# gwlucastrig/gridfour

Measured on NVIDIA B200. Metric: GVRS tile decode GB/s of raw samples (config 3 shard, 180x240 tiles), higher is better.
Workload: dtype int32

## Files before the change

gridfour_b200/csrc/g4_api.cu:

```cuda
#include <cstdio>
#include <cstdlib>
#include <cstring>
#include <string>
#include <algorithm>
#include <vector>
#include "g4_kernels.h"

using namespace g4;

namespace {

constexpr int kMaxChunks = 16;

thread_local std::string tlsError;

int cuda_fail(cudaError_t e, const char* what) {
  tlsError = std::string(what) + ": " + cudaGetErrorString(e);
  return G4_ERR_CUDA;
}
#define CK(call)                                           \
  do {                                                     \
    cudaError_t e_ = (call);                               \
    if (e_ != cudaSuccess) return cuda_fail(e_, #call);    \
  } while (0)

struct DevBuf {
  void* p = nullptr;
  size_t cap = 0;
  cudaError_t ensure(size_t bytes) {
    if (bytes <= cap) return cudaSuccess;
    if (p) cudaFree(p);
    p = nullptr;
    cap = 0;
    size_t want = bytes + bytes / 8 + 256;
    cudaError_t e = cudaMalloc(&p, want);
    if (e == cudaSuccess) cap = want;
    return e;
  }
  void release() {
    if (p) cudaFree(p);
    p = nullptr;
    cap = 0;
  }
  template <class T>
  T* as() const { return static_cast<T*>(p); }
};

size_t round_up(size_t x, size_t a) { return (x + a - 1) / a * a; }

struct DeviceGuard {
  int prev = -1;
  cudaError_t err = cudaSuccess;
  explicit DeviceGuard(int device) {
    if (cudaGetDevice(&prev) != cudaSuccess) prev = -1;
    if (prev != device) err = cudaSetDevice(device);
    else prev = -1;
  }
  ~DeviceGuard() {
    if (prev >= 0) cudaSetDevice(prev);
  }
};
#define ENTER(ctx)                                                     \
  DeviceGuard guard_((ctx)->device);                                  \
  if (guard_.err != cudaSuccess) return cuda_fail(guard_.err, "cudaSetDevice")

}

struct g4_context {
  int device = 0;
  cudaStream_t stream = nullptr;
  bool ownStream = false;
  int smCount = 148;
  uint64_t launches = 0;
  DevBuf slots[G4_MAX_CODECS];
  DevBuf candLens, candPreds, candStatus;
  DevBuf counters;
  DevBuf scratch;
  DevBuf lists, src, total;
  DevBuf encScratch;
  DevBuf region;
  DevBuf coef;
  DevBuf defer;
  DevBuf lsopMeta;
  DevBuf lsopSide, lsopExc, lsopResid, lsopStage, lsopCks;
  DevBuf wide;
  DevBuf jobLen, jobOff, jobOut, jobTotal, streamIn, streamOut, deflateWork;
  DevBuf stSorted, stRank, stTable, stWork, stCounters;
  DevBuf rcPos, rcOff, rcLen, rcCrc, rcStored, rcTotal, rcData, rcOffsets, rcLens, rcIndex, rcStatus, rcOut;
  DevBuf rcChain, rcDesc;
  std::vector<uint64_t> hostOff;
  std::vector<uint32_t> hostLen;
  uint64_t hostTotal = 0;
  int deflateWorkers = 0;
  uint64_t stagedChunkBytes = 2ull << 30;
  const int64_t* curTileOffset = nullptr;
  const int64_t* curTilePitch = nullptr;
  DevBuf tileRefs;
  uint64_t arenaLimit = ~0ull;
  bool lsopDeflate = true;
  DevBuf sGrid, sArena, sOffsets, sLens, sCodec, sPred, sStatus;
  cudaStream_t copyIn = nullptr, copyOut = nullptr;
  cudaEvent_t evIn[16] = {}, evDone[16] = {}, evStart = nullptr, evOrder = nullptr;
  bool timing = false;
  bool asyncDevice = false;
  cudaEvent_t ev[2][G4_CODEC_COUNT + 1][2] = {};
  bool evUsed[2][G4_CODEC_COUNT + 1] = {};
};

namespace {

bool codec_is_float(int id) { return id == G4_CODEC_FLOAT; }

int persistent_ctas(const g4_context* ctx, int nTiles, int perSm) {
  int cap = ctx->smCount * perSm;
  return nTiles < cap ? nTiles : cap;
}

int ensure_jobs(g4_context* ctx, int nStreams) {
  CK(ctx->jobLen.ensure(size_t(nStreams) * 4));
  CK(ctx->jobOff.ensure(size_t(nStreams) * 8));
  CK(ctx->jobOut.ensure(size_t(nStreams) * 4));
  CK(ctx->jobTotal.ensure(8));
  return G4_OK;
}
int prepare_streams(g4_context* ctx, int nStreams) {
  CK(launch_stream_offsets(ctx->jobLen.as<uint32_t>(), ctx->jobOff.as<uint64_t>(), nStreams, ctx->jobTotal.as<uint64_t>(), ctx->stream));
  uint64_t total = 0;
  ctx->hostOff.resize(size_t(nStreams) + 1);
  ctx->hostLen.resize(size_t(nStreams));
  CK(cudaMemcpyAsync(&total, ctx->jobTotal.p, 8, cudaMemcpyDeviceToHost, ctx->stream));
  CK(cudaMemcpyAsync(ctx->hostOff.data(), ctx->jobOff.p, size_t(nStreams) * 8, cudaMemcpyDeviceToHost, ctx->stream));
  CK(cudaMemcpyAsync(ctx->hostLen.data(), ctx->jobLen.p, size_t(nStreams) * 4, cudaMemcpyDeviceToHost, ctx->stream));
  CK(cudaStreamSynchronize(ctx->stream));
  ctx->hostOff[size_t(nStreams)] = total;
  ctx->hostTotal = total;
  CK(ctx->streamIn.ensure(total + 64));
  CK(ctx->streamOut.ensure(total + 112ull * uint64_t(nStreams) + 256));
  ctx->launches++;
  return G4_OK;
}
int run_streams(g4_context* ctx, int nStreams, int capExtra, int level, int* counter) {
  const uint32_t stagedMax = deflate_staged_max();
  int nBig = 0;
  for (int j = 0; j < nStreams; j++) nBig += ctx->hostLen[size_t(j)] > stagedMax;
  if (nBig > 0) {
    int nWorkers = nBig < ctx->deflateWorkers ? nBig : ctx->deflateWorkers;
    nWorkers = (nWorkers + 31) / 32 * 32;
    CK(ctx->deflateWork.ensure(size_t(nWorkers) * deflate_work_bytes()));
    StreamArgs sa{};
    sa.inBuf = ctx->streamIn.as<uint8_t>();
    sa.inOff = ctx->jobOff.as<uint64_t>();
    sa.inLen = ctx->jobLen.as<uint32_t>();
    sa.outBuf = ctx->streamOut.as<uint8_t>();
    sa.outLen = ctx->jobOut.as<uint32_t>();
    sa.nStreams = nStreams;
    sa.capExtra = capExtra;
    sa.level = level;
    sa.work = ctx->deflateWork.p;
    sa.counter = counter;
    sa.bigOnly = 1;
    CK(launch_deflate_streams(sa, nWorkers, ctx->stream));
    ctx->launches++;
  }
  const uint64_t budget = ctx->stagedChunkBytes;
  CK(ctx->stCounters.ensure(4 * sizeof(int)));
  int j0 = 0;
  while (j0 < nStreams) {
    int j1 = j0 + 1;
    while (j1 < nStreams && ctx->hostOff[size_t(j1) + 1] - ctx->hostOff[size_t(j0)] <= budget) j1++;
    const uint64_t base = ctx->hostOff[size_t(j0)];
    const uint64_t span = ctx->hostOff[size_t(j1)] - base;
    const int nChunk = j1 - j0;
    CK(ctx->stSorted.ensure(span * 2 + 64));
    CK(ctx->stRank.ensure(span * 2 + 64));
    CK(ctx->stTable.ensure(span * 8 + 256));
    CK(ctx->stWork.ensure(size_t(nChunk) * deflate_blocks_bytes()));
    CK(cudaMemsetAsync(ctx->stCounters.p, 0, 4 * sizeof(int), ctx->stream));
    StagedArgs st{};
    st.inBuf = ctx->streamIn.as<uint8_t>();
    st.inOff = ctx->jobOff.as<uint64_t>();
    st.inLen = ctx->jobLen.as<uint32_t>();
    st.outBuf = ctx->streamOut.as<uint8_t>();
    st.outLen = ctx->jobOut.as<uint32_t>();
    st.jBegin = j0;
    st.jEnd = j1;
    st.baseOff = base;
    st.sorted = ctx->stSorted.as<uint16_t>();
    st.rank = ctx->stRank.as<uint16_t>();
    st.table = ctx->stTable.as<uint32_t>();
    st.tableQ = ctx->stTable.as<uint32_t>() + (span + 16);
    st.lazy = level >= 9 ? 1 : 0;
    st.maxLen = 0;
    for (int j = j0; j < j1; j++)
      if (ctx->hostLen[size_t(j)] <= stagedMax && ctx->hostLen[size_t(j)] > st.maxLen) st.maxLen = ctx->hostLen[size_t(j)];
    st.blocks = static_cast<DeflateBlocks*>(ctx->stWork.p);
    st.capExtra = capExtra;
    st.level = level;
    st.counters = ctx->stCounters.as<int>();
    CK(launch_deflate_staged(st, ctx->smCount, ctx->stream));
    ctx->launches += st.lazy ? 3 : 4;
    j0 = j1;
  }
  return G4_OK;
}

struct KernelTimer;
int launch_encoder_impl(g4_context* ctx, int codecId, EncodeArgs& a, int nTiles) {
  const int nGrid = persistent_ctas(ctx, nTiles, 8);
  uint32_t* jl = nullptr;
  uint64_t* jo = nullptr;
  uint32_t* jout = nullptr;
  switch (codecId) {
    case G4_CODEC_DEFLATE: {
      const int nStreams = 3 * nTiles;
      int rc = ensure_jobs(ctx, nStreams);
      if (rc != G4_OK) return rc;
      jl = ctx->jobLen.as<uint32_t>(); jo = ctx->jobOff.as<uint64_t>(); jout = ctx->jobOut.as<uint32_t>();
      CK(launch_deflate_m32_size(a, jl, nGrid, ctx->stream));
      if ((rc = prepare_streams(ctx, nStreams)) != G4_OK) return rc;
      CK(launch_deflate_m32_write(a, jl, jo, ctx->streamIn.as<uint8_t>(), nGrid, ctx->stream));
      if ((rc = run_streams(ctx, nStreams, 118, 6, a.counter + 48)) != G4_OK) return rc;
      CK(launch_deflate_pick(a, jl, jo, ctx->streamOut.as<uint8_t>(), jout, nGrid, ctx->stream));
      ctx->launches += 3;
      return G4_OK;
    }
    case G4_CODEC_FLOAT: {
      const int nStreams = 5 * nTiles;
      int rc = ensure_jobs(ctx, nStreams);
      if (rc != G4_OK) return rc;
      jl = ctx->jobLen.as<uint32_t>(); jo = ctx->jobOff.as<uint64_t>(); jout = ctx->jobOut.as<uint32_t>();
      CK(launch_float_plane_size(nTiles, uint32_t(a.band.tile_rows) * uint32_t(a.band.tile_cols), jl, ctx->stream));
      if ((rc = prepare_streams(ctx, nStreams)) != G4_OK) return rc;
      CK(launch_float_plane_write(a, jo, ctx->streamIn.as<uint8_t>(), nGrid, ctx->stream));
      if ((rc = run_streams(ctx, nStreams, 128, 9, a.counter + 48)) != G4_OK) return rc;
      CK(launch_float_pick(a, jo, ctx->streamOut.as<uint8_t>(), jout, nGrid, ctx->stream));
      ctx->launches += 3;
      return G4_OK;
    }
    case G4_CODEC_HUFFMAN: {
      int n = persistent_ctas(ctx, nTiles, 4);
      CK(launch_huffman_encode(a, n, ctx->stream));
      ctx->launches++;
      return G4_OK;
    }
    case G4_CODEC_CANON_HUFFMAN:
    case G4_CODEC_LSOP12: {
      int n = persistent_ctas(ctx, nTiles, 4);
      const size_t stride = 32 * 1024;
      CK(ctx->encScratch.ensure(stride * n));
      a.scratch = ctx->encScratch.as<uint8_t>();
      a.scratchStride = stride;
      if (codecId == G4_CODEC_CANON_HUFFMAN) CK(launch_canon_encode(a, n, ctx->stream));
      else CK(launch_lsop_encode(a, n, ctx->stream));
      ctx->launches++;
      if (codecId == G4_CODEC_LSOP12 && ctx->lsopDeflate) {
        const int nStreams = 2 * nTiles;
        int rc = ensure_jobs(ctx, nStreams);
        if (rc != G4_OK) return rc;
        jl = ctx->jobLen.as<uint32_t>(); jo = ctx->jobOff.as<uint64_t>(); jout = ctx->jobOut.as<uint32_t>();
        CK(launch_lsop_m32_size(a, jl, nGrid, ctx->stream));
        if ((rc = prepare_streams(ctx, nStreams)) != G4_OK) return rc;
        CK(launch_lsop_m32_write(a, jl, jo, ctx->streamIn.as<uint8_t>(), nGrid, ctx->stream));
        if ((rc = run_streams(ctx, nStreams, 128, 6, a.counter + 48)) != G4_OK) return rc;
        CK(launch_lsop_pick(a, jl, jo, ctx->streamOut.as<uint8_t>(), jout, nGrid, ctx->stream));
        ctx->launches += 3;
      }
      return G4_OK;
    }
    default:
      tlsError = "codec not implemented on the GPU yet";
      return G4_ERR_UNSUPPORTED;
  }
}

int decoder_ctas(const g4_context* ctx, int nTiles) { return persistent_ctas(ctx, nTiles, 8); }

struct KernelTimer {
  g4_context* c;
  int dir, kind;
  KernelTimer(g4_context* ctx, int dir_, int kind_) : c(ctx), dir(dir_), kind(kind_) {
    if (c->timing) {
      if (!c->ev[dir][kind][0]) { cudaEventCreate(&c->ev[dir][kind][0]); cudaEventCreate(&c->ev[dir][kind][1]); }
      cudaEventRecord(c->ev[dir][kind][0], c->stream);
    }
  }
  ~KernelTimer() {
    if (c->timing) { cudaEventRecord(c->ev[dir][kind][1], c->stream); c->evUsed[dir][kind] = true; }
  }
};

int launch_decoder(g4_context* ctx, int codecId, DecodeArgs& a, int nCtas) {
  KernelTimer timer(ctx, 0, codecId);
  const int nTiles = a.band.tiles_down * a.band.tiles_across;
  switch (codecId) {
    case G4_CODEC_HUFFMAN: {
      CK(ctx->defer.ensure(size_t(nTiles) * sizeof(int)));
      CK(ctx->lsopStage.ensure(huffman2_spill_bytes(ctx->smCount)));
      CK(ctx->lsopMeta.ensure(huffman2_tree_bytes(nTiles)));
      HuffFusedScratch fused{ctx->lsopStage.as<uint32_t>(), ctx->lsopMeta.as<uint8_t>(), ctx->defer.as<int>(), ctx->counters.as<int>() + 48, ctx->smCount};
      int nLaunch = 0;
      CK(launch_huffman_decode(a, nCtas, ctx->stream, fused, &nLaunch));
      ctx->launches += uint64_t(nLaunch);
      return G4_OK;
    }
    case G4_CODEC_CANON_HUFFMAN:
      CK(launch_canon_decode(a, nCtas, ctx->stream));
      ctx->launches++;
      return G4_OK;
    case G4_CODEC_DEFLATE: {
      const size_t stride = round_up(size_t(a.band.tile_rows) * a.band.tile_cols * 6 + 64, 16);
      CK(ctx->region.ensure(stride * nTiles));
      CK(launch_deflate_decode(a, ctx->region.as<uint8_t>(), stride, nCtas, nTiles, ctx->stream));
      ctx->launches += 2;
      return G4_OK;
    }
    case G4_CODEC_FLOAT: {
      const size_t stride = 5 * round_up(size_t(a.band.tile_rows) * a.band.tile_cols, 16);
      CK(ctx->region.ensure(stride * nTiles));
      CK(launch_float_decode(a, ctx->region.as<uint8_t>(), stride, nCtas, nTiles, ctx->stream));
      ctx->launches += 2;
      return G4_OK;
    }
    case G4_CODEC_LSOP12:
      CK(ctx->coef.ensure(size_t(nTiles) * 12 * sizeof(float)));
      CK(ctx->defer.ensure(size_t(nTiles) * sizeof(int)));
      CK(ctx->lsopMeta.ensure(size_t(nTiles) * lsop_meta_bytes()));
      CK(ctx->lsopCks.ensure(size_t(nTiles) * 8));
      CK(cudaMemsetAsync(ctx->lsopCks.p, 0, size_t(nTiles) * 8, ctx->stream));
      a.lsopCks = ctx->lsopCks.as<uint32_t>();
    {
      int nLaunch = 0;
      LsopFastArgs fast{};
      const bool useFast = lsop_fast_geometry(a.band, a.grid, &fast.g);
      if (useFast) {
        CK(ctx->lsopSide.ensure(lsop_fast_side_bytes(fast.g, nTiles)));
        CK(ctx->lsopExc.ensure(lsop_fast_exc_bytes(nTiles)));
        CK(ctx->lsopResid.ensure(lsop_fast_resid_bytes(fast.g, nTiles)));
        fast.side = ctx->lsopSide.as<int4>();
        fast.exc = ctx->lsopExc.as<uint32_t>();
        fast.resid = ctx->lsopResid.as<uint8_t>();
        if (lsop_fast_stage_bytes(ctx->smCount)) CK(ctx->lsopStage.ensure(lsop_fast_stage_bytes(ctx->smCount)));
        fast.textStage = ctx->lsopStage.as<uint8_t>();
      }
      CK(launch_lsop_decode(a, ctx->coef.as<float>(), ctx->lsopMeta.as<uint8_t>(), ctx->defer.as<int>(), ctx->counters.as<int>() + 56,
                            nCtas, nTiles, ctx->stream, &nLaunch, useFast ? &fast : nullptr, ctx->smCount));
      CK(launch_lsop_value_checksum(a, nTiles, ctx->stream));
      ctx->launches += uint64_t(nLaunch) + 1;
      return G4_OK;
    }
    case G4_CODEC_LSOP08:
      CK(ctx->coef.ensure(size_t(nTiles) * 12 * sizeof(float)));
      CK(launch_lsop08_decode(a, ctx->coef.as<float>(), nCtas, nTiles, ctx->stream));
      ctx->launches += 2;
      return G4_OK;
    default:
      tlsError = "codec not implemented on the GPU yet";
      return G4_ERR_UNSUPPORTED;
  }
}

int launch_encoder(g4_context* ctx, int codecId, EncodeArgs& a, int nTiles) {
  KernelTimer timer(ctx, 1, codecId);
  return launch_encoder_impl(ctx, codecId, a, nTiles);
}

int check_band(const g4_band_desc* b) {
  if (!b) return G4_ERR_ARG;
  if (b->elem_type != G4_ELEM_I32 && b->elem_type != G4_ELEM_F32 && b->elem_type != G4_ELEM_I16) return G4_ERR_ARG;
  if (b->tile_rows < 2 || b->tile_cols < 2) return G4_ERR_UNSUPPORTED;
  if (b->tiles_down < 1 || b->tiles_across < 1) return G4_ERR_ARG;
  if (int64_t(b->tile_rows) * b->tile_cols > (1 << 20)) return G4_ERR_UNSUPPORTED;
  if (b->grid_pitch < int64_t(b->tiles_across) * b->tile_cols) return G4_ERR_ARG;
  if (int64_t(b->tiles_down) * b->tiles_across > (1 << 24)) return G4_ERR_ARG;
  return G4_OK;
}

size_t elem_bytes(const g4_band_desc& b) { return b.elem_type == G4_ELEM_I16 ? 2 : 4; }
uint32_t standard_size(const g4_band_desc& b) {
  const uint32_t n = uint32_t(b.tile_rows) * uint32_t(b.tile_cols);
  return b.elem_type == G4_ELEM_I16 ? ((2u * n + 3u) & ~3u) : 4u * n;
}

size_t band_samples(const g4_band_desc& b) {
  return size_t(int64_t(b.tiles_down) * b.tile_rows - 1) * size_t(b.grid_pitch) + size_t(b.tiles_across) * b.tile_cols;
}

int encode_device_i32(g4_context* ctx, const g4_codec_list* codecs, const g4_band_desc* band, void* grid, uint8_t* arena,
                      uint64_t arenaCap, uint64_t* offsets, uint32_t* lens, uint8_t* codecOut, uint8_t* predOut, int32_t* status,
                      uint64_t* totalHost, size_t slotBytes, const int16_t* raw16, int64_t raw16Pitch) {
  const int nTiles = band->tiles_down * band->tiles_across;
  const int n = band->tile_rows * band->tile_cols;
  const bool isFloat = band->elem_type == G4_ELEM_F32;
  int cand[G4_MAX_CODECS], nCand = 0;
  for (int k = 0; k < codecs->n_codecs; k++) {
    int id = codecs->codec_ids[k];
    if (id < 0 || id >= G4_CODEC_COUNT) return G4_ERR_ARG;
    if (id == G4_CODEC_LSOP08) continue;
    if (codec_is_float(id) == isFloat) cand[nCand++] = k;
  }
  CK(ctx->candLens.ensure(size_t(nCand + 1) * nTiles * 4));
  CK(ctx->candPreds.ensure(size_t(nCand + 1) * nTiles));
  CK(ctx->candStatus.ensure(size_t(nCand + 1) * nTiles * 4));
  CK(ctx->counters.ensure(64 * sizeof(int)));
  CK(ctx->src.ensure(size_t(nTiles) * 4));
  CK(ctx->total.ensure(8));
  CK(cudaMemsetAsync(ctx->counters.p, 0, 64 * sizeof(int), ctx->stream));
  SelectArgs sel{};
  CompactArgs cmp{};
  for (int c = 0; c < nCand; c++) {
    CK(ctx->slots[c].ensure(size_t(nTiles) * slotBytes));
    EncodeArgs a{};
    a.band = *band;
    a.band.tileOffset = ctx->curTileOffset;
    a.band.tilePitch = ctx->curTilePitch;
    a.grid = grid;
    a.slots = ctx->slots[c].as<uint8_t>();
    a.slotBytes = slotBytes;
    a.lens = ctx->candLens.as<uint32_t>() + size_t(c) * nTiles;
    a.preds = ctx->candPreds.as<uint8_t>() + size_t(c) * nTiles;
    a.status = ctx->candStatus.as<int32_t>() + size_t(c) * nTiles;
    a.counter = ctx->counters.as<int>() + c;
    a.codecIndex = cand[c];
    a.scratch = nullptr;
    a.scratchStride = 0;
    int rc = launch_encoder(ctx, codecs->codec_ids[cand[c]], a, nTiles);
    if (rc != G4_OK) return rc;
    sel.candIndex[c] = cand[c];
    cmp.slots[c] = a.slots;
  }
  sel.nTiles = nTiles;
  sel.nCand = nCand;
  sel.rawLen = raw16 ? ((2u * uint32_t(n) + 3u) & ~3u) : uint32_t(n) * 4u;
  sel.candLens = ctx->candLens.as<uint32_t>();
  sel.candPreds = ctx->candPreds.as<uint8_t>();
  sel.candStatus = ctx->candStatus.as<int32_t>();
  sel.lens = lens;
  sel.codecOut = codecOut;
  sel.predOut = predOut;
  sel.src = ctx->src.as<int>();
  sel.status = status;
  CK(launch_select(sel, ctx->stream));
  CK(launch_offsets(lens, offsets, nTiles, ctx->total.as<uint64_t>(), ctx->stream));
  cmp.band = *band;
  cmp.band.tileOffset = ctx->curTileOffset;
  cmp.band.tilePitch = ctx->curTilePitch;
  cmp.grid = grid;
  cmp.slotBytes = slotBytes;
  cmp.lens = lens;
  cmp.offsets = offsets;
  cmp.src = ctx->src.as<int>();
  cmp.arena = arena;
  cmp.arenaCap = arenaCap;
  cmp.status = status;
  cmp.raw16 = raw16;
  cmp.raw16Pitch = raw16Pitch;
  CK(launch_compact(cmp, nTiles, ctx->stream));
  ctx->launches += 3;
  uint64_t total = 0;
  CK(cudaMemcpyAsync(&total, ctx->total.p, 8, cudaMemcpyDeviceToHost, ctx->stream));
  CK(cudaStreamSynchronize(ctx->stream));
  if (totalHost) *totalHost = total;
  return G4_OK;
}

int decode_device_i32(g4_context* ctx, const g4_codec_list* codecs, const g4_band_desc* band, const uint8_t* arena,
                      const uint64_t* offsets, const uint32_t* lens, void* grid, int32_t* status, bool rawShorts) {
  const int nTiles = band->tiles_down * band->tiles_across;
  const int n = band->tile_rows * band->tile_cols;
  const int kinds = G4_CODEC_COUNT + 1;
  CK(ctx->counters.ensure(64 * sizeof(int)));
  CK(ctx->lists.ensure(size_t(kinds) * nTiles * sizeof(int)));
  CK(cudaMemsetAsync(ctx->counters.p, 0, 64 * sizeof(int), ctx->stream));
  ClassifyArgs cl{};
  cl.nTiles = nTiles;
  cl.elemType = band->elem_type;
  cl.rawLen = rawShorts ? ((2u * uint32_t(n) + 3u) & ~3u) : uint32_t(n) * 4u;
  cl.codecs = *codecs;
  cl.arena = arena;
  cl.arenaLen = ctx->arenaLimit;
  cl.offsets = offsets;
  cl.lens = lens;
  cl.lists = ctx->lists.as<int>();
  cl.counts = ctx->counters.as<int>() + 32;
  cl.status = status;
  CK(launch_classify(cl, ctx->stream));
  ctx->launches++;
  const int nCtas = decoder_ctas(ctx, nTiles);
  const size_t stride = round_up(size_t(n) * 6 + 64, 16);
  CK(ctx->scratch.ensure(stride * nCtas));
  bool present[G4_CODEC_COUNT] = {false};
  for (int k = 0; k < codecs->n_codecs; k++) {
    int id = codecs->codec_ids[k];
    if (id < 0 || id >= G4_CODEC_COUNT) return G4_ERR_ARG;
    present[id] = true;
  }
  for (int kind = 0; kind <= G4_CODEC_COUNT; kind++) {
    if (kind < G4_CODEC_COUNT && !present[kind]) continue;
    DecodeArgs a{};
    a.band = *band;
    a.band.tileOffset = ctx->curTileOffset;
    a.band.tilePitch = ctx->curTilePitch;
    a.grid = grid;
    a.arena = arena;
    a.offsets = offsets;
    a.lens = lens;
    a.list = ctx->lists.as<int>() + size_t(kind) * nTiles;
    a.listCount = ctx->counters.as<int>() + 32 + kind;
    a.status = status;
    a.counter = ctx->counters.as<int>() + 16 + kind;
    a.scratch = ctx->scratch.as<uint8_t>();
    a.scratchStride = stride;
    a.rawShorts = rawShorts ? 1 : 0;
    if (kind == G4_CODEC_COUNT) {
      KernelTimer timer(ctx, 0, kind);
      CK(launch_raw_decode(a, nTiles, ctx->stream));
      ctx->launches++;
    } else {
      int rc = launch_decoder(ctx, kind, a, nCtas);
      if (rc != G4_OK) return rc;
    }
  }
  return G4_OK;
}

g4_band_desc widened(const g4_band_desc& b) {
  g4_band_desc w = b;
  w.elem_type = G4_ELEM_I32;
  w.grid_pitch = int64_t(b.tiles_across) * b.tile_cols;
  return w;
}

int encode_device(g4_context* ctx, const g4_codec_list* codecs, const g4_band_desc* band, void* grid, uint8_t* arena,
                  uint64_t arenaCap, uint64_t* offsets, uint32_t* lens, uint8_t* codecOut, uint8_t* predOut, int32_t* status,
                  uint64_t* totalHost, size_t slotBytes) {
  if (band->elem_type != G4_ELEM_I16)
    return encode_device_i32(ctx, codecs, band, grid, arena, arenaCap, offsets, lens, codecOut, predOut, status, totalHost, slotBytes,
                             nullptr, 0);
  const g4_band_desc w = widened(*band);
  const int64_t rows = int64_t(band->tiles_down) * band->tile_rows, cols = w.grid_pitch;
  CK(ctx->wide.ensure(size_t(rows) * size_t(cols) * 4));
  CK(launch_widen_i16(static_cast<const int16_t*>(grid), band->grid_pitch, ctx->wide.as<int32_t>(), rows, cols, band->fill_value,
                      ctx->stream));
  ctx->launches++;
  return encode_device_i32(ctx, codecs, &w, ctx->wide.p, arena, arenaCap, offsets, lens, codecOut, predOut, status, totalHost, slotBytes,
                           static_cast<const int16_t*>(grid), band->grid_pitch);
}

int decode_device(g4_context* ctx, const g4_codec_list* codecs, const g4_band_desc* band, const uint8_t* arena,
                  const uint64_t* offsets, const uint32_t* lens, void* grid, int32_t* status) {
  if (band->elem_type != G4_ELEM_I16) return decode_device_i32(ctx, codecs, band, arena, offsets, lens, grid, status, false);
  const g4_band_desc w = widened(*band);
  const int64_t rows = int64_t(band->tiles_down) * band->tile_rows, cols = w.grid_pitch;
  CK(ctx->wide.ensure(size_t(rows) * size_t(cols) * 4));
  int rc = decode_device_i32(ctx, codecs, &w, arena, offsets, lens, ctx->wide.p, status, true);
  if (rc != G4_OK) return rc;
  CK(launch_narrow_i16(ctx->wide.as<int32_t>(), static_cast<int16_t*>(grid), band->grid_pitch, rows, cols, ctx->stream));
  ctx->launches++;
  return G4_OK;
}

int first_bad_status(const std::vector<int32_t>& st) {
  int32_t note = G4_OK;
  for (int32_t s : st) {
    if (s < 0) return s;
    if (s != G4_OK && note == G4_OK) note = s;
  }
  return note;
}

}

extern "C" {

int g4_abi_version(void) { return G4_ABI_VERSION; }

const char* g4_status_string(int s) {
  switch (s) {
    case G4_OK: return "ok";
    case G4_DECLINED: return "declined (codec returns null for this tile)";
    case G4_ERR_ARG: return "bad argument";
    case G4_ERR_FORMAT: return "malformed packing";
    case G4_ERR_CAPACITY: return "output buffer too small";
    case G4_ERR_CUDA: return "CUDA error";
    case G4_ERR_UNSUPPORTED: return "unsupported";
    default: return "unknown status";
  }
}

const char* g4_last_error(void) { return tlsError.c_str(); }

int g4_device_count(void) {
  int n = 0;
  if (cudaGetDeviceCount(&n) != cudaSuccess) return 0;
  return n;
}

static const char* kCodecNames[G4_CODEC_COUNT] = {"GvrsHuffman", "GvrsDeflate", "GvrsFloat", "GvrsCanonicalHuffman", "LSOP12", "LSOP08"};

int g4_codec_id_from_name(const char* name) {
  if (!name) return -1;
  for (int i = 0; i < G4_CODEC_COUNT; i++)
    if (std::strcmp(name, kCodecNames[i]) == 0) return i;
  return -1;
}
const char* g4_codec_name(int id) { return (id >= 0 && id < G4_CODEC_COUNT) ? kCodecNames[id] : nullptr; }

int g4_context_create(int device, void* cuda_stream, g4_context** out) {
  if (!out) return G4_ERR_ARG;
  *out = nullptr;
  int nDev = 0;
  cudaError_t e = cudaGetDeviceCount(&nDev);
  if (e != cudaSuccess || nDev == 0) {
    tlsError = "no CUDA device available (the codec kernels have no CPU fallback)";
    return G4_ERR_CUDA;
  }
  if (device < 0 || device >= nDev) return G4_ERR_ARG;
  DeviceGuard guard(device);
  if (guard.err != cudaSuccess) return cuda_fail(guard.err, "cudaSetDevice");
  g4_context* ctx = new g4_context();
  ctx->device = device;
  auto fail = [&](cudaError_t err, const char* what) {
    if (ctx->ownStream && ctx->stream) cudaStreamDestroy(ctx->stream);
    delete ctx;
    return cuda_fail(err, what);
  };
  cudaDeviceProp prop;
  if ((e = cudaGetDeviceProperties(&prop, device)) != cudaSuccess) return fail(e, "cudaGetDeviceProperties");
  ctx->smCount = prop.multiProcessorCount;
  ctx->deflateWorkers = ctx->smCount * 256;
  if (const char* ev = std::getenv("G4_DEFLATE_WORKERS")) { int v = std::atoi(ev); if (v >= 32) ctx->deflateWorkers = v; }
  if (const char* ev = std::getenv("G4_STAGED_CHUNK_MB")) { long v = std::atol(ev); if (v >= 1) ctx->stagedChunkBytes = uint64_t(v) << 20; }
  if (cuda_stream) ctx->stream = static_cast<cudaStream_t>(cuda_stream);
  else {
    if ((e = cudaStreamCreateWithFlags(&ctx->stream, cudaStreamNonBlocking)) != cudaSuccess) return fail(e, "cudaStreamCreateWithFlags");
    ctx->ownStream = true;
  }
  if ((e = cudaEventCreateWithFlags(&ctx->evStart, cudaEventDisableTiming)) != cudaSuccess) return fail(e, "cudaEventCreateWithFlags");
  if ((e = cudaEventCreateWithFlags(&ctx->evOrder, cudaEventDisableTiming)) != cudaSuccess) return fail(e, "cudaEventCreateWithFlags");
  *out = ctx;
  return G4_OK;
}

int g4_context_order_stream(g4_context* ctx, void* other_stream, int before) {
  if (!ctx) return G4_ERR_ARG;
  cudaStream_t other = static_cast<cudaStream_t>(other_stream);
  if (other == ctx->stream) return G4_OK;
  ENTER(ctx);
  if (before) {
    CK(cudaEventRecord(ctx->evOrder, other));
    CK(cudaStreamWaitEvent(ctx->stream, ctx->evOrder, 0));
  } else {
    CK(cudaEventRecord(ctx->evOrder, ctx->stream));
    CK(cudaStreamWaitEvent(other, ctx->evOrder, 0));
  }
  return G4_OK;
}

void g4_context_destroy(g4_context* ctx) {
  if (!ctx) return;
  DeviceGuard guard(ctx->device);
  cudaStreamSynchronize(ctx->stream);
  if (ctx->copyIn) {
    cudaStreamSynchronize(ctx->copyIn);
    cudaStreamSynchronize(ctx->copyOut);
    cudaStreamDestroy(ctx->copyIn);
    cudaStreamDestroy(ctx->copyOut);
    for (int k = 0; k < kMaxChunks; k++) { cudaEventDestroy(ctx->evIn[k]); cudaEventDestroy(ctx->evDone[k]); }
  }
  if (ctx->evStart) cudaEventDestroy(ctx->evStart);
  if (ctx->evOrder) cudaEventDestroy(ctx->evOrder);
  for (auto& b : ctx->slots) b.release();
  DevBuf* bufs[] = {&ctx->candLens, &ctx->candPreds, &ctx->candStatus, &ctx->counters, &ctx->scratch, &ctx->lists, &ctx->src,
                    &ctx->total, &ctx->coef, &ctx->defer, &ctx->lsopMeta, &ctx->lsopSide, &ctx->lsopExc, &ctx->lsopResid, &ctx->lsopStage, &ctx->tileRefs, &ctx->lsopCks, &ctx->wide, &ctx->encScratch, &ctx->region, &ctx->jobLen, &ctx->jobOff, &ctx->jobOut, &ctx->jobTotal,
                    &ctx->streamIn, &ctx->streamOut, &ctx->deflateWork, &ctx->stSorted, &ctx->stRank, &ctx->stTable,
                    &ctx->stWork, &ctx->stCounters, &ctx->rcPos, &ctx->rcOff, &ctx->rcLen, &ctx->rcCrc, &ctx->rcStored, &ctx->rcTotal,
                    &ctx->rcData, &ctx->rcOffsets, &ctx->rcLens, &ctx->rcIndex, &ctx->rcStatus, &ctx->rcOut, &ctx->rcChain, &ctx->rcDesc, &ctx->sGrid, &ctx->sArena, &ctx->sOffsets, &ctx->sLens, &ctx->sCodec, &ctx->sPred, &ctx->sStatus};
  for (DevBuf* b : bufs) b->release();
  if (ctx->ownStream) cudaStreamDestroy(ctx->stream);
  delete ctx;
}

int g4_context_synchronize(g4_context* ctx) {
  if (!ctx) return G4_ERR_ARG;
  CK(cudaStreamSynchronize(ctx->stream));
  return G4_OK;
}

uint64_t g4_launch_count(const g4_context* ctx) { return ctx ? ctx->launches : 0; }

int g4_context_set_async(g4_context* ctx, int enabled) {
  if (!ctx) return G4_ERR_ARG;
  ctx->asyncDevice = enabled != 0;
  return G4_OK;
}

int g4_context_set_timing(g4_context* ctx, int enabled) {
  if (!ctx) return G4_ERR_ARG;
  ctx->timing = enabled != 0;
  for (auto& d : ctx->evUsed) for (bool& u : d) u = false;
  return G4_OK;
}

int g4_codec_supported(int codec_id, int direction) {
  switch (codec_id) {
    case G4_CODEC_HUFFMAN: return 1;
    case G4_CODEC_DEFLATE: return 1;
    case G4_CODEC_FLOAT: return 1;
    case G4_CODEC_CANON_HUFFMAN: return 1;
    case G4_CODEC_LSOP12: return 1;
    case G4_CODEC_LSOP08: return direction == 0 ? 1 : 0;
    default: return 0;
  }
}

double g4_kernel_time_ms(g4_context* ctx, int direction, int codec_kind) {
  if (!ctx || direction < 0 || direction > 1 || codec_kind < 0 || codec_kind > G4_CODEC_COUNT) return -1.0;
  if (!ctx->evUsed[direction][codec_kind]) return -1.0;
  float ms = -1.0f;
  if (cudaEventSynchronize(ctx->ev[direction][codec_kind][1]) != cudaSuccess) return -1.0;
  if (cudaEventElapsedTime(&ms, ctx->ev[direction][codec_kind][0], ctx->ev[direction][codec_kind][1]) != cudaSuccess) return -1.0;
  return double(ms);
}

int g4_crc32c(g4_context* ctx, int mem_space, const uint8_t* data, const uint64_t* offsets, const uint32_t* sizes, int n,
              uint32_t* crc_out) {
  if (!ctx || !data || !offsets || !sizes || !crc_out || n < 0) return G4_ERR_ARG;
  if (n == 0) return G4_OK;
  ENTER(ctx);
  if (mem_space == G4_MEM_DEVICE) {
    CK(launch_crc32c(data, offsets, sizes, n, crc_out, 0, ctx->stream));
    ctx->launches++;
    return G4_OK;
  }
  if (mem_space != G4_MEM_HOST) return G4_ERR_ARG;
  uint64_t bytes = 0;
  for (int i = 0; i < n; i++) {
    const uint64_t end = offsets[i] + sizes[i];
    if (end > bytes) bytes = end;
  }
  CK(ctx->rcData.ensure(bytes + 16));
  CK(ctx->rcOff.ensure(size_t(n) * 8));
  CK(ctx->rcLen.ensure(size_t(n) * 4));
  CK(ctx->rcCrc.ensure(size_t(n) * 4));
  CK(cudaMemcpyAsync(ctx->rcData.p, data, bytes, cudaMemcpyHostToDevice, ctx->stream));
  CK(cudaMemcpyAsync(ctx->rcOff.p, offsets, size_t(n) * 8, cudaMemcpyHostToDevice, ctx->stream));
  CK(cudaMemcpyAsync(ctx->rcLen.p, sizes, size_t(n) * 4, cudaMemcpyHostToDevice, ctx->stream));
  CK(launch_crc32c(ctx->rcData.as<uint8_t>(), ctx->rcOff.as<uint64_t>(), ctx->rcLen.as<uint32_t>(), n, ctx->rcCrc.as<uint32_t>(), 0,
                   ctx->stream));
  ctx->launches++;
  CK(cudaMemcpyAsync(crc_out, ctx->rcCrc.p, size_t(n) * 4, cudaMemcpyDeviceToHost, ctx->stream));
  CK(cudaStreamSynchronize(ctx->stream));
  return G4_OK;
}

uint64_t g4_tile_records_bound(int n_tiles, uint64_t payload_bytes) {
  if (n_tiles < 0) return 0;
  return payload_bytes + uint64_t(n_tiles) * 32ull;
}

int g4_pack_tile_records(g4_context* ctx, int mem_space, const uint8_t* arena, const uint64_t* offsets, const uint32_t* lens,
                         const int32_t* tile_index, int first_tile_index, int n_tiles, int checksum, uint64_t base_pos,
                         uint8_t* records, uint64_t records_cap, uint64_t* content_pos, uint64_t* total_bytes) {
  if (!ctx || !arena || !offsets || !lens || !records || !content_pos || !total_bytes || n_tiles < 0 || (base_pos & 7)) return G4_ERR_ARG;
  if (mem_space != G4_MEM_DEVICE && mem_space != G4_MEM_HOST) return G4_ERR_ARG;
  *total_bytes = 0;
  if (n_tiles == 0) return G4_OK;
  ENTER(ctx);
  const int n = n_tiles;
  const uint8_t* dArena = arena;
  const uint64_t* dOffsets = offsets;
  const uint32_t* dLens = lens;
  const int32_t* dIndex = tile_index;
  uint64_t* dPos = content_pos;
  uint8_t* dRecords = records;
  if (mem_space == G4_MEM_HOST) {
    uint64_t arenaBytes = 0;
    for (int t = 0; t < n; t++) {
      const uint64_t end = offsets[t] + lens[t];
      if (end > arenaBytes) arenaBytes = end;
    }
    CK(ctx->rcData.ensure(arenaBytes + 16));
    CK(ctx->rcOffsets.ensure(size_t(n) * 8));
    CK(ctx->rcLens.ensure(size_t(n) * 4));
    CK(ctx->rcPos.ensure(size_t(n) * 8));
    CK(ctx->rcOut.ensure(records_cap + 16));
    CK(cudaMemcpyAsync(ctx->rcData.p, arena, arenaBytes, cudaMemcpyHostToDevice, ctx->stream));
    CK(cudaMemcpyAsync(ctx->rcOffsets.p, offsets, size_t(n) * 8, cudaMemcpyHostToDevice, ctx->stream));
    CK(cudaMemcpyAsync(ctx->rcLens.p, lens, size_t(n) * 4, cudaMemcpyHostToDevice, ctx->stream));
    if (tile_index) {
      CK(ctx->rcIndex.ensure(size_t(n) * 4));
      CK(cudaMemcpyAsync(ctx->rcIndex.p, tile_index, size_t(n) * 4, cudaMemcpyHostToDevice, ctx->stream));
      dIndex = ctx->rcIndex.as<int32_t>();
    }
    dArena = ctx->rcData.as<uint8_t>();
    dOffsets = ctx->rcOffsets.as<uint64_t>();
    dLens = ctx->rcLens.as<uint32_t>();
    dPos = ctx->rcPos.as<uint64_t>();
    dRecords = ctx->rcOut.as<uint8_t>();
  }
  CK(ctx->rcOff.ensure(size_t(n) * 8));
  CK(ctx->rcLen.ensure(size_t(n) * 4));
  CK(ctx->rcTotal.ensure(8));
  CK(launch_record_layout(dLens, n, base_pos, dPos, ctx->rcOff.as<uint64_t>(), ctx->rcLen.as<uint32_t>(), ctx->rcTotal.as<uint64_t>(),
                          ctx->stream));
  uint64_t total = 0;
  CK(cudaMemcpyAsync(&total, ctx->rcTotal.p, 8, cudaMemcpyDeviceToHost, ctx->stream));
  CK(cudaStreamSynchronize(ctx->stream));
  *total_bytes = total;
  if (total > records_cap) return G4_ERR_CAPACITY;
  CK(launch_record_pack(dArena, dOffsets, dLens, dIndex, first_tile_index, n, ctx->rcOff.as<uint64_t>(), ctx->rcLen.as<uint32_t>(), dRecords,
                        persistent_ctas(ctx, n, 8), ctx->stream));
  ctx->launches += 2;
  if (checksum) {
    CK(launch_crc32c(dRecords, ctx->rcOff.as<uint64_t>(), ctx->rcLen.as<uint32_t>(), n, nullptr, 1, ctx->stream));
    ctx->launches++;
  }
  if (mem_space == G4_MEM_HOST) {
    CK(cudaMemcpyAsync(records, dRecords, total, cudaMemcpyDeviceToHost, ctx->stream));
    CK(cudaMemcpyAsync(content_pos, dPos, size_t(n) * 8, cudaMemcpyDeviceToHost, ctx->stream));
    CK(cudaStreamSynchronize(ctx->stream));
  }
  return G4_OK;
}

int g4_unpack_tile_records(g4_context* ctx, int mem_space, const uint8_t* image, uint64_t image_len, const uint64_t* content_pos,
                           int n_tiles, int checksum, uint64_t* payload_offsets, uint32_t* lens, int32_t* status) {
  if (!ctx || !image || !content_pos || !payload_offsets || !lens || !status || n_tiles < 0) return G4_ERR_ARG;
  if (mem_space != G4_MEM_DEVICE && mem_space != G4_MEM_HOST) return G4_ERR_ARG;
  if (n_tiles == 0) return G4_OK;
  ENTER(ctx);
  const int n = n_tiles;
  const uint8_t* dImage = image;
  const uint64_t* dPos = content_pos;
  uint64_t* dPay = payload_offsets;
  uint32_t* dLens = lens;
  int32_t* dStatus = status;
  if (mem_space == G4_MEM_HOST) {
    CK(ctx->rcData.ensure(image_len + 16));
    CK(ctx->rcPos.ensure(size_t(n) * 8));
    CK(ctx->rcOffsets.ensure(size_t(n) * 8));
    CK(ctx->rcLens.ensure(size_t(n) * 4));
    CK(ctx->rcStatus.ensure(size_t(n) * 4));
    CK(cudaMemcpyAsync(ctx->rcData.p, image, image_len, cudaMemcpyHostToDevice, ctx->stream));
    CK(cudaMemcpyAsync(ctx->rcPos.p, content_pos, size_t(n) * 8, cudaMemcpyHostToDevice, ctx->stream));
    dImage = ctx->rcData.as<uint8_t>();
    dPos = ctx->rcPos.as<uint64_t>();
    dPay = ctx->rcOffsets.as<uint64_t>();
    dLens = ctx->rcLens.as<uint32_t>();
    dStatus = ctx->rcStatus.as<int32_t>();
  }
  if (reinterpret_cast<uintptr_t>(dImage) & 7) return G4_ERR_ARG;
  CK(ctx->rcOff.ensure(size_t(n) * 8));
  CK(ctx->rcLen.ensure(size_t(n) * 4));
  CK(ctx->rcCrc.ensure(size_t(n) * 4));
  CK(ctx->rcStored.ensure(size_t(n) * 4));
  CK(launch_record_unpack(dImage, image_len, dPos, n, dPay, dLens, ctx->rcOff.as<uint64_t>(), ctx->rcLen.as<uint32_t>(),
                          ctx->rcStored.as<uint32_t>(), dStatus, ctx->stream));
  ctx->launches++;
  if (checksum) {
    CK(launch_crc32c(dImage, ctx->rcOff.as<uint64_t>(), ctx->rcLen.as<uint32_t>(), n, ctx->rcCrc.as<uint32_t>(), 0, ctx->stream));
    CK(launch_record_verify(ctx->rcCrc.as<uint32_t>(), ctx->rcStored.as<uint32_t>(), n, dStatus, ctx->stream));
    ctx->launches += 2;
  }
  if (mem_space == G4_MEM_HOST) {
    CK(cudaMemcpyAsync(payload_offsets, dPay, size_t(n) * 8, cudaMemcpyDeviceToHost, ctx->stream));
    CK(cudaMemcpyAsync(lens, dLens, size_t(n) * 4, cudaMemcpyDeviceToHost, ctx->stream));
    CK(cudaMemcpyAsync(status, dStatus, size_t(n) * 4, cudaMemcpyDeviceToHost, ctx->stream));
    CK(cudaStreamSynchronize(ctx->stream));
  }
  return G4_OK;
}

uint64_t g4_tile_records_bound_multi(int n_tiles, int n_elements, uint64_t payload_bytes) {
  if (n_tiles < 0 || n_elements < 1 || n_elements > G4_MAX_ELEMENTS) return 0;
  return payload_bytes + uint64_t(n_tiles) * (23ull + 4ull * uint64_t(n_elements));
}

int g4_pack_tile_records_multi(g4_context* ctx, int mem_space, int n_elements, const uint8_t* const* arenas,
                               const uint64_t* const* offsets, const uint32_t* const* lens, const int32_t* tile_index,
                               int first_tile_index, int n_tiles, int checksum, uint64_t base_pos, uint8_t* records,
                               uint64_t records_cap, uint64_t* content_pos, uint64_t* total_bytes) {
  if (!ctx || !arenas || !offsets || !lens || !records || !content_pos || !total_bytes || n_tiles < 0 || (base_pos & 7)) return G4_ERR_ARG;
  if (n_elements < 1 || n_elements > G4_MAX_ELEMENTS) return G4_ERR_UNSUPPORTED;
  if (mem_space != G4_MEM_DEVICE && mem_space != G4_MEM_HOST) return G4_ERR_ARG;
  for (int e = 0; e < n_elements; e++)
    if (!arenas[e] || !offsets[e] || !lens[e]) return G4_ERR_ARG;
  *total_bytes = 0;
  if (n_tiles == 0) return G4_OK;
  ENTER(ctx);
  const int n = n_tiles, E = n_elements;
  std::vector<RecordElement> desc(static_cast<size_t>(E));
  const int32_t* dIndex = tile_index;
  uint64_t* dPos = content_pos;
  uint8_t* dRecords = records;
  if (mem_space == G4_MEM_HOST) {
    std::vector<uint64_t> base(size_t(E) + 1, 0), used(size_t(E), 0);
    for (int e = 0; e < E; e++) {
      for (int t = 0; t < n; t++) {
        const uint64_t end = offsets[e][t] + lens[e][t];
        if (end > used[size_t(e)]) used[size_t(e)] = end;
      }
      base[size_t(e) + 1] = round_up(base[size_t(e)] + used[size_t(e)], 16);
    }
    CK(ctx->rcData.ensure(base[size_t(E)] + 16));
    CK(ctx->rcOffsets.ensure(size_t(E) * n * 8));
    CK(ctx->rcLens.ensure(size_t(E) * n * 4));
    CK(ctx->rcPos.ensure(size_t(n) * 8));
    CK(ctx->rcOut.ensure(records_cap + 16));
    for (int e = 0; e < E; e++) {
      uint8_t* a = ctx->rcData.as<uint8_t>() + base[size_t(e)];
      uint64_t* o = ctx->rcOffsets.as<uint64_t>() + size_t(e) * n;
      uint32_t* l = ctx->rcLens.as<uint32_t>() + size_t(e) * n;
      if (used[size_t(e)]) CK(cudaMemcpyAsync(a, arenas[e], used[size_t(e)], cudaMemcpyHostToDevice, ctx->stream));
      CK(cudaMemcpyAsync(o, offsets[e], size_t(n) * 8, cudaMemcpyHostToDevice, ctx->stream));
      CK(cudaMemcpyAsync(l, lens[e], size_t(n) * 4, cudaMemcpyHostToDevice, ctx->stream));
      desc[size_t(e)] = RecordElement{a, o, l};
    }
    if (tile_index) {
      CK(ctx->rcIndex.ensure(size_t(n) * 4));
      CK(cudaMemcpyAsync(ctx->rcIndex.p, tile_index, size_t(n) * 4, cudaMemcpyHostToDevice, ctx->stream));
      dIndex = ctx->rcIndex.as<int32_t>();
    }
    dPos = ctx->rcPos.as<uint64_t>();
    dRecords = ctx->rcOut.as<uint8_t>();
  } else {
    for (int e = 0; e < E; e++) desc[size_t(e)] = RecordElement{arenas[e], offsets[e], lens[e]};
  }
  CK(ctx->rcDesc.ensure(size_t(E) * sizeof(RecordElement)));
  CK(cudaMemcpyAsync(ctx->rcDesc.p, desc.data(), size_t(E) * sizeof(RecordElement), cudaMemcpyHostToDevice, ctx->stream));
  const RecordElement* dDesc = ctx->rcDesc.as<RecordElement>();
  CK(ctx->rcChain.ensure(size_t(n) * 4));
  CK(ctx->rcOff.ensure(size_t(n) * 8));
  CK(ctx->rcLen.ensure(size_t(n) * 4));
  CK(ctx->rcTotal.ensure(8));
  CK(launch_record_chain_lens(dDesc, E, n, ctx->rcChain.as<uint32_t>(), ctx->stream));
  CK(launch_record_layout(ctx->rcChain.as<uint32_t>(), n, base_pos, dPos, ctx->rcOff.as<uint64_t>(), ctx->rcLen.as<uint32_t>(),
                          ctx->rcTotal.as<uint64_t>(), ctx->stream));
  uint64_t total = 0;
  CK(cudaMemcpyAsync(&total, ctx->rcTotal.p, 8, cudaMemcpyDeviceToHost, ctx->stream));
  CK(cudaStreamSynchronize(ctx->stream));
  ctx->launches += 2;
  *total_bytes = total;
  if (total > records_cap) return G4_ERR_CAPACITY;
  CK(launch_record_pack_multi(dDesc, E, dIndex, first_tile_index, n, ctx->rcOff.as<uint64_t>(), ctx->rcLen.as<uint32_t>(), dRecords,
                              persistent_ctas(ctx, n, 8), ctx->stream));
  ctx->launches++;
  if (checksum) {
    CK(launch_crc32c(dRecords, ctx->rcOff.as<uint64_t>(), ctx->rcLen.as<uint32_t>(), n, nullptr, 1, ctx->stream));
    ctx->launches++;
  }
  if (mem_space == G4_MEM_HOST) {
    CK(cudaMemcpyAsync(records, dRecords, total, cudaMemcpyDeviceToHost, ctx->stream));
    CK(cudaMemcpyAsync(content_pos, dPos, size_t(n) * 8, cudaMemcpyDeviceToHost, ctx->stream));
    CK(cudaStreamSynchronize(ctx->stream));
  }
  return G4_OK;
}

int g4_unpack_tile_records_multi(g4_context* ctx, int mem_space, int n_elements, const uint8_t* image, uint64_t image_len,
                                 const uint64_t* content_pos, int n_tiles, int checksum, uint64_t* payload_offsets,
                                 uint32_t* lens, int32_t* status) {
  if (!ctx || !image || !content_pos || !payload_offsets || !lens || !status || n_tiles < 0) return G4_ERR_ARG;
  if (n_elements < 1 || n_elements > G4_MAX_ELEMENTS) return G4_ERR_UNSUPPORTED;
  if (mem_space != G4_MEM_DEVICE && mem_space != G4_MEM_HOST) return G4_ERR_ARG;
  if (n_tiles == 0) return G4_OK;
  ENTER(ctx);
  const int n = n_tiles, E = n_elements;
  const uint8_t* dImage = image;
  const uint64_t* dPos = content_pos;
  uint64_t* dPay = payload_offsets;
  uint32_t* dLens = lens;
  int32_t* dStatus = status;
  if (mem_space == G4_MEM_HOST) {
    CK(ctx->rcData.ensure(image_len + 16));
    CK(ctx->rcPos.ensure(size_t(n) * 8));
    CK(ctx->rcOffsets.ensure(size_t(E) * n * 8));
// ... 574 lines not shown
```

gridfour_b200/csrc/g4_batch.cu:

```cuda
#include "g4_kernels.h"
#include "g4_device.cuh"
#include "../../include/g4terrain.h"

namespace g4 {

__global__ void fill_terrain_kernel(int elemType, uint64_t seed, int64_t row0, int64_t col0, int64_t nRows, int64_t nCols,
                                    void* out) {
  const int64_t total = nRows * nCols;
  for (int64_t i = blockIdx.x * int64_t(blockDim.x) + threadIdx.x; i < total; i += int64_t(gridDim.x) * blockDim.x) {
    int64_t r = i / nCols, c = i - r * nCols;
    if (elemType == G4_ELEM_I32) static_cast<int32_t*>(out)[i] = g4_terrain_m(seed, row0 + r, col0 + c);
    else static_cast<float*>(out)[i] = float(g4_terrain_dm(seed, row0 + r, col0 + c)) * 0.1f;
  }
}

__global__ void select_kernel(SelectArgs a) {
  int t = blockIdx.x * blockDim.x + threadIdx.x;
  if (t >= a.nTiles) return;
  uint32_t best = 0xffffffffu;
  int bc = -1;
  int st = G4_OK;
  for (int c = 0; c < a.nCand; c++) {
    int s = a.candStatus[size_t(c) * a.nTiles + t];
    uint32_t l = a.candLens[size_t(c) * a.nTiles + t];
    if (s == G4_OK && l > 0 && l < best) { best = l; bc = c; }
    else if (s < 0 && s != G4_ERR_CAPACITY && st == G4_OK) st = s;
  }
  const uint32_t rawLen = a.rawLen;
  if (bc < 0 || best >= rawLen) {
    a.lens[t] = rawLen;
    a.codecOut[t] = G4_CODEC_RAW;
    a.predOut[t] = 0;
    a.src[t] = -1;
  } else {
    a.lens[t] = best;
    a.codecOut[t] = uint8_t(a.candIndex[bc]);
    a.predOut[t] = a.candPreds[size_t(bc) * a.nTiles + t];
    a.src[t] = bc;
  }
  a.status[t] = st;
}

__global__ void __launch_bounds__(kThreads) offsets_kernel(const uint32_t* lens, uint64_t* offsets, int nTiles, uint64_t* total) {
  __shared__ unsigned long long sm[kWarps];
  __shared__ unsigned long long carry;
  const int lane = threadIdx.x & 31, warp = threadIdx.x >> 5;
  if (threadIdx.x == 0) carry = 0;
  __syncthreads();
  for (int t0 = 0; t0 < nTiles; t0 += kThreads) {
    int t = t0 + threadIdx.x;
    unsigned long long x = t < nTiles ? ((unsigned long long)(lens[t]) + 7ull) & ~7ull : 0ull;
    unsigned long long inc = x;
#pragma unroll
    for (int d = 1; d < 32; d <<= 1) {
      unsigned long long y = __shfl_up_sync(0xffffffffu, inc, d);
      if (lane >= d) inc += y;
    }
    if (lane == 31) sm[warp] = inc;
    __syncthreads();
    unsigned long long base = carry;
    for (int w = 0; w < warp; w++) base += sm[w];
    if (t < nTiles) offsets[t] = base + inc - x;
    __syncthreads();
    if (threadIdx.x == kThreads - 1) carry = base + inc;
    __syncthreads();
  }
  if (threadIdx.x == 0) *total = carry;
}

__global__ void __launch_bounds__(kThreads) compact_kernel(CompactArgs a) {
  const int t = blockIdx.x;
  const uint32_t len = a.lens[t];
  const uint64_t off = a.offsets[t];
  if (off + ((uint64_t(len) + 7) & ~7ull) > a.arenaCap) {
    if (threadIdx.x == 0) a.status[t] = G4_ERR_CAPACITY;
    return;
  }
  uint8_t* dst = a.arena + off;
  const int src = a.src[t];
  if (src < 0 && a.raw16) {
    const int R = a.band.tile_rows, C = a.band.tile_cols, n = R * C;
    const int tr = t / a.band.tiles_across, tc = t - tr * a.band.tiles_across;
    const int16_t* base = a.raw16 + int64_t(tr) * R * a.raw16Pitch + int64_t(tc) * C;
    uint32_t* d32 = reinterpret_cast<uint32_t*>(dst);
    const int nWords = int((len + 3u) >> 2);
    for (int i = threadIdx.x; i < ((nWords + 1) & ~1); i += kThreads) {
      uint32_t w = 0;
      for (int h = 0; h < 2; h++) {
        int k = 2 * i + h;
        if (k < n) { int r = k / C, c = k - r * C; w |= uint32_t(uint16_t(base[int64_t(r) * a.raw16Pitch + c])) << (16 * h); }
      }
      d32[i] = w;
    }
  } else if (src < 0) {
    const TileView tv = tile_view(a.band, a.grid, t);
    uint32_t* d32 = reinterpret_cast<uint32_t*>(dst);
    const int n = tv.R * tv.C;
    for (int i = threadIdx.x; i < n; i += kThreads) {
      int r = i / tv.C, c = i - r * tv.C;
      d32[i] = uint32_t(tv.at(r, c));
    }
    if ((n & 1) && threadIdx.x == 0) d32[n] = 0;
  } else {
    const uint32_t* s32 = reinterpret_cast<const uint32_t*>(a.slots[src] + size_t(t) * a.slotBytes);
    uint32_t* d32 = reinterpret_cast<uint32_t*>(dst);
    const uint32_t nWords = ((len + 7u) & ~7u) >> 2;
    for (uint32_t i = threadIdx.x; i < nWords; i += kThreads) {
      uint32_t w = 0;
      if (i * 4u < len) {
        w = s32[i];
        uint32_t valid = len - i * 4u;
        if (valid < 4u) w &= (1u << (8u * valid)) - 1u;
      }
      d32[i] = w;
    }
  }
}

__global__ void classify_kernel(ClassifyArgs a) {
  int t = blockIdx.x * blockDim.x + threadIdx.x;
  if (t >= a.nTiles) return;
  const uint32_t len = a.lens[t];
  int kind;
  int st = G4_OK;
  if (len > a.rawLen || a.offsets[t] > a.arenaLen || uint64_t(len) > a.arenaLen - a.offsets[t]) { kind = -1; st = G4_ERR_FORMAT; }
  else if (len == a.rawLen) kind = G4_CODEC_COUNT;
  else if (len == 0) { kind = -1; st = G4_ERR_FORMAT; }
  else {
    int index = a.arena[a.offsets[t]];
    if (index >= a.codecs.n_codecs) { kind = -1; st = G4_ERR_FORMAT; }
    else {
      kind = a.codecs.codec_ids[index];
      bool isFloatCodec = kind == G4_CODEC_FLOAT;
      if (kind < 0 || kind >= G4_CODEC_COUNT || isFloatCodec != (a.elemType == G4_ELEM_F32)) { kind = -1; st = G4_ERR_FORMAT; }
    }
  }
  a.status[t] = st;
  if (kind >= 0) {
    int pos = atomicAdd(&a.counts[kind], 1);
    a.lists[size_t(kind) * a.nTiles + pos] = t;
  }
}

__global__ void __launch_bounds__(kThreads) raw_decode_kernel(DecodeArgs a) {
  const int li = blockIdx.x;
  if (li >= *a.listCount) return;
  const int t = a.list[li];
  const TileView tv = tile_view(a.band, a.grid, t);
  const uint8_t* src = a.arena + a.offsets[t];
  const int n = tv.R * tv.C;
  if (a.rawShorts) {
    for (int i = threadIdx.x; i < n; i += kThreads) {
      int r = i / tv.C, c = i - r * tv.C;
      tv.at(r, c) = int32_t(int16_t(uint16_t(src[2 * size_t(i)]) | (uint16_t(src[2 * size_t(i) + 1]) << 8)));
    }
    return;
  }
  const bool aligned = (reinterpret_cast<uintptr_t>(src) & 3) == 0;
  for (int i = threadIdx.x; i < n; i += kThreads) {
    int r = i / tv.C, c = i - r * tv.C;
    uint32_t v = aligned ? reinterpret_cast<const uint32_t*>(src)[i] : load_le32(src + 4 * size_t(i));
    tv.at(r, c) = int32_t(v);
  }
}

__global__ void widen_i16_kernel(const int16_t* src, int64_t srcPitch, int32_t* dst, int64_t rows, int64_t cols, int32_t fill) {
  const int64_t total = rows * cols;
  for (int64_t i = blockIdx.x * int64_t(blockDim.x) + threadIdx.x; i < total; i += int64_t(gridDim.x) * blockDim.x) {
    int64_t r = i / cols, c = i - r * cols;
    int32_t v = src[r * srcPitch + c];
    dst[i] = v == fill ? kNull : v;
  }
}
__global__ void narrow_i16_kernel(const int32_t* src, int16_t* dst, int64_t dstPitch, int64_t rows, int64_t cols) {
  const int64_t total = rows * cols;
  for (int64_t i = blockIdx.x * int64_t(blockDim.x) + threadIdx.x; i < total; i += int64_t(gridDim.x) * blockDim.x) {
    int64_t r = i / cols, c = i - r * cols;
    int32_t v = src[i];
    dst[r * dstPitch + c] = v == kNull ? int16_t(-32768) : int16_t(v);
  }
}

cudaError_t launch_fill_terrain(int elemType, uint64_t seed, int64_t row0, int64_t col0, int64_t nRows, int64_t nCols, void* out,
                                cudaStream_t s) {
  fill_terrain_kernel<<<148 * 8, 256, 0, s>>>(elemType, seed, row0, col0, nRows, nCols, out);
  return cudaGetLastError();
}
cudaError_t launch_widen_i16(const int16_t* src, int64_t srcPitch, int32_t* dst, int64_t rows, int64_t cols, int32_t fill, cudaStream_t s) {
  widen_i16_kernel<<<148 * 8, 256, 0, s>>>(src, srcPitch, dst, rows, cols, fill);
  return cudaGetLastError();
}
cudaError_t launch_narrow_i16(const int32_t* src, int16_t* dst, int64_t dstPitch, int64_t rows, int64_t cols, cudaStream_t s) {
  narrow_i16_kernel<<<148 * 8, 256, 0, s>>>(src, dst, dstPitch, rows, cols);
  return cudaGetLastError();
}
cudaError_t launch_select(const SelectArgs& a, cudaStream_t s) {
  select_kernel<<<(a.nTiles + 255) / 256, 256, 0, s>>>(a);
  return cudaGetLastError();
}
cudaError_t launch_offsets(const uint32_t* lens, uint64_t* offsets, int nTiles, uint64_t* total, cudaStream_t s) {
  offsets_kernel<<<1, kThreads, 0, s>>>(lens, offsets, nTiles, total);
  return cudaGetLastError();
}
cudaError_t launch_compact(const CompactArgs& a, int nTiles, cudaStream_t s) {
  compact_kernel<<<nTiles, kThreads, 0, s>>>(a);
  return cudaGetLastError();
}
cudaError_t launch_classify(const ClassifyArgs& a, cudaStream_t s) {
  classify_kernel<<<(a.nTiles + 255) / 256, 256, 0, s>>>(a);
  return cudaGetLastError();
}
cudaError_t launch_raw_decode(const DecodeArgs& a, int nTiles, cudaStream_t s) {
  raw_decode_kernel<<<nTiles, kThreads, 0, s>>>(a);
  return cudaGetLastError();
}

}
```

gridfour_b200/csrc/g4_kernels.h:

```cpp
#pragma once
#include <cstddef>
#include <cstdint>
#include <atomic>
#include <cuda_runtime.h>
#include "../../include/g4codec.h"
#include "g4_device.cuh"

namespace g4 {

template <class Fn>
inline cudaError_t once_per_device(std::atomic<uint64_t>& done, Fn set) {
  int d = 0;
  cudaGetDevice(&d);
  const uint64_t bit = 1ull << (d & 63);
  if (done.load(std::memory_order_acquire) & bit) return cudaSuccess;
  const cudaError_t e = set();
  if (e == cudaSuccess) done.fetch_or(bit, std::memory_order_release);
  return e;
}

struct DeflateBlocks;

struct EncodeArgs {
  BandEx band;
  void* grid;
  uint8_t* slots;
  size_t slotBytes;
  uint32_t* lens;
  uint8_t* preds;
  int32_t* status;
  int* counter;
  int codecIndex;
  uint8_t* scratch;
  size_t scratchStride;
};

struct DecodeArgs {
  BandEx band;
  void* grid;
  const uint8_t* arena;
  const uint64_t* offsets;
  const uint32_t* lens;
  const int* list;
  const int* listCount;
  int32_t* status;
  int* counter;
  uint8_t* scratch;
  size_t scratchStride;
  int rawShorts;
  uint32_t* lsopCks;
};

struct SelectArgs {
  int nTiles, nCand;
  uint32_t rawLen;
  const uint32_t* candLens;
  const uint8_t* candPreds;
  const int32_t* candStatus;
  int candIndex[G4_MAX_CODECS];
  uint32_t* lens;
  uint8_t* codecOut;
  uint8_t* predOut;
  int* src;
  int32_t* status;
};

struct CompactArgs {
  BandEx band;
  void* grid;
  const uint8_t* slots[G4_MAX_CODECS];
  size_t slotBytes;
  const uint32_t* lens;
  const uint64_t* offsets;
  const int* src;
  uint8_t* arena;
  uint64_t arenaCap;
  int32_t* status;
  const int16_t* raw16;
  int64_t raw16Pitch;
};

struct ClassifyArgs {
  int nTiles;
  int elemType;
  uint32_t rawLen;
  g4_codec_list codecs;
  const uint8_t* arena;
  uint64_t arenaLen;
  const uint64_t* offsets;
  const uint32_t* lens;
  int* lists;
  int* counts;
  int32_t* status;
};

struct StreamArgs {
  const uint8_t* inBuf;
  const uint64_t* inOff;
  const uint32_t* inLen;
  uint8_t* outBuf;
  uint32_t* outLen;
  int nStreams;
  int capExtra;
  int level;
  void* work;
  int* counter;
  int bigOnly;
};

struct StagedArgs {
  const uint8_t* inBuf;
  const uint64_t* inOff;
  const uint32_t* inLen;
  uint8_t* outBuf;
  uint32_t* outLen;
  int jBegin, jEnd;
  uint64_t baseOff;
  uint16_t* sorted;
  uint16_t* rank;
  uint32_t* table;
  uint32_t* tableQ;
  uint32_t maxLen;
  int lazy;
  DeflateBlocks* blocks;
  int capExtra, level;
  int* counters;
};

cudaError_t launch_fill_terrain(int elemType, uint64_t seed, int64_t row0, int64_t col0, int64_t nRows, int64_t nCols, void* out,
                                cudaStream_t s);
cudaError_t launch_select(const SelectArgs& a, cudaStream_t s);
cudaError_t launch_offsets(const uint32_t* lens, uint64_t* offsets, int nTiles, uint64_t* total, cudaStream_t s);
cudaError_t launch_compact(const CompactArgs& a, int nTiles, cudaStream_t s);
cudaError_t launch_classify(const ClassifyArgs& a, cudaStream_t s);
cudaError_t launch_raw_decode(const DecodeArgs& a, int nTiles, cudaStream_t s);
cudaError_t launch_widen_i16(const int16_t* src, int64_t srcPitch, int32_t* dst, int64_t rows, int64_t cols, int32_t fill, cudaStream_t s);
cudaError_t launch_narrow_i16(const int32_t* src, int16_t* dst, int64_t dstPitch, int64_t rows, int64_t cols, cudaStream_t s);

cudaError_t launch_huffman_encode(const EncodeArgs& a, int nCtas, cudaStream_t s);
struct HuffFusedScratch {
  uint32_t* spill;
  uint8_t* trees;
  int* defer;
  int* counters;
  int smCount;
};
size_t huffman2_spill_bytes(int smCount);
size_t huffman2_tree_bytes(int nTiles);
cudaError_t launch_huffman_decode(const DecodeArgs& a, int nCtas, cudaStream_t s, const HuffFusedScratch& fused, int* launches);
cudaError_t launch_canon_decode(const DecodeArgs& a, int nCtas, cudaStream_t s);
cudaError_t launch_canon_encode(const EncodeArgs& a, int nCtas, cudaStream_t s);
cudaError_t launch_lsop_encode(const EncodeArgs& a, int nCtas, cudaStream_t s);
cudaError_t launch_deflate_decode(const DecodeArgs& a, uint8_t* region, size_t regionStride, int nCtas, int nTilesUpper,
                                  cudaStream_t s);
cudaError_t launch_float_decode(const DecodeArgs& a, uint8_t* region, size_t regionStride, int nCtas, int nTilesUpper,
                                cudaStream_t s);
size_t lsop_meta_bytes();
cudaError_t launch_lsop08_decode(const DecodeArgs& a, float* coef, int nCtas, int nTilesUpper, cudaStream_t s);


struct LsopFastGeom {
  int R, C;
  int W;
  int logW;
  int nStrips;
  int P;
  int nSteps;
  int chunkRows;
  int nChunks;
  int tileBytes;
  int tilePitch;
  int wide;
};
struct LsopFastArgs {
  DecodeArgs a;
  float* coef;
  uint8_t* meta;
  int4* side;
  uint32_t* exc;
  uint8_t* resid;
  uint8_t* textStage;
  int* defer;
  int* deferCount;
  LsopFastGeom g;
};
bool lsop_fast_geometry(const g4_band_desc& band, const void* grid, LsopFastGeom* out);
size_t lsop_fast_side_bytes(const LsopFastGeom& g, int nTiles);
size_t lsop_fast_exc_bytes(int nTiles);
size_t lsop_fast_stage_bytes(int smCount);
size_t lsop_fast_resid_bytes(const LsopFastGeom& g, int nTiles);
cudaError_t launch_lsop_decode_fast(const LsopFastArgs& A, int nTilesUpper, int smCount, int* textCounter, cudaStream_t s, int* launches);
cudaError_t launch_lsop_decode(const DecodeArgs& a, float* coef, uint8_t* meta, int* defer, int* deferCounters, int nCtas,
                               int nTilesUpper, cudaStream_t s, int* launches, const LsopFastArgs* fast = nullptr, int smCount = 148);

struct AnalyzeArgs {
  int nTiles;
  uint32_t nCells;
  uint32_t rawLen;
  g4_codec_list codecs;
  const uint8_t* arena;
  uint64_t arenaLen;
  const uint64_t* offsets;
  const uint32_t* lens;
  uint8_t* scratch;
  size_t scratchStride;
  g4_tile_stats* stats;
  unsigned long long* pairs;
};
cudaError_t launch_analyze(const AnalyzeArgs& a, int nCtas, cudaStream_t s);

struct PredictorArgs {
  BandEx band;
  void* grid;
  int model;
  int intFlavour;
  uint8_t* slots;
  size_t slotBytes;
  uint32_t* lens;
  int32_t* seeds;
  int32_t* status;
};
cudaError_t launch_predictor(const PredictorArgs& a, int decode, int nCtas, cudaStream_t s);

size_t deflate_work_bytes();
size_t deflate_blocks_bytes();
uint32_t deflate_staged_max();
cudaError_t launch_deflate_staged(const StagedArgs& a, int smCount, cudaStream_t s);
cudaError_t launch_stream_offsets(const uint32_t* inLen, uint64_t* inOff, int nStreams, uint64_t* total, cudaStream_t s);
cudaError_t launch_deflate_streams(const StreamArgs& a, int nWorkers, cudaStream_t s);
cudaError_t launch_deflate_m32_size(const EncodeArgs& a, uint32_t* inLen, int nCtas, cudaStream_t s);
cudaError_t launch_deflate_m32_write(const EncodeArgs& a, const uint32_t* inLen, const uint64_t* inOff, uint8_t* inBuf, int nCtas,
                                     cudaStream_t s);
cudaError_t launch_deflate_pick(const EncodeArgs& a, const uint32_t* inLen, const uint64_t* inOff, const uint8_t* outBuf,
                                const uint32_t* outLen, int nCtas, cudaStream_t s);
cudaError_t launch_float_plane_size(int nTiles, uint32_t n, uint32_t* inLen, cudaStream_t s);
cudaError_t launch_float_plane_write(const EncodeArgs& a, const uint64_t* inOff, uint8_t* inBuf, int nCtas, cudaStream_t s);
cudaError_t launch_float_pick(const EncodeArgs& a, const uint64_t* inOff, const uint8_t* outBuf, const uint32_t* outLen, int nCtas,
                              cudaStream_t s);
cudaError_t launch_lsop_m32_size(const EncodeArgs& a, uint32_t* inLen, int nCtas, cudaStream_t s);
cudaError_t launch_lsop_m32_write(const EncodeArgs& a, const uint32_t* inLen, const uint64_t* inOff, uint8_t* inBuf, int nCtas,
                                  cudaStream_t s);
cudaError_t launch_lsop_pick(const EncodeArgs& a, const uint32_t* inLen, const uint64_t* inOff, const uint8_t* outBuf,
                             const uint32_t* outLen, int nCtas, cudaStream_t s);

cudaError_t launch_crc32c(const uint8_t* data, const uint64_t* offsets, const uint32_t* sizes, int n, uint32_t* out, int storeAtEnd,
                          cudaStream_t s);
cudaError_t launch_record_layout(const uint32_t* lens, int n, uint64_t basePos, uint64_t* contentPos, uint64_t* crcOff, uint32_t* crcLen,
                                 uint64_t* total, cudaStream_t s);
cudaError_t launch_record_pack(const uint8_t* arena, const uint64_t* offsets, const uint32_t* lens, const int32_t* tileIndex,
                               int firstTileIndex, int n, const uint64_t* crcOff, const uint32_t* crcLen, uint8_t* records, int nCtas,
                               cudaStream_t s);
cudaError_t launch_record_unpack(const uint8_t* image, uint64_t imageLen, const uint64_t* contentPos, int n, uint64_t* payloadOff,
                                 uint32_t* lens, uint64_t* crcOff, uint32_t* crcLen, uint32_t* storedCrc, int32_t* status, cudaStream_t s);
cudaError_t launch_lsop_value_checksum(const DecodeArgs& a, int nTilesUpper, cudaStream_t s);
cudaError_t launch_record_verify(const uint32_t* computed, const uint32_t* stored, int n, int32_t* status, cudaStream_t s);
struct RecordElement {
  const uint8_t* arena;
  const uint64_t* offsets;
  const uint32_t* lens;
};
cudaError_t launch_record_chain_lens(const RecordElement* elems, int nElements, int n, uint32_t* chainLens, cudaStream_t s);
cudaError_t launch_record_pack_multi(const RecordElement* elems, int nElements, const int32_t* tileIndex, int firstTileIndex, int n,
                                     const uint64_t* crcOff, const uint32_t* crcLen, uint8_t* records, int nCtas, cudaStream_t s);
cudaError_t launch_record_unpack_multi(const uint8_t* image, uint64_t imageLen, const uint64_t* contentPos, int n, int nElements,
                                       uint64_t* payloadOff, uint32_t* lens, uint64_t* crcOff, uint32_t* crcLen, uint32_t* storedCrc,
                                       int32_t* status, cudaStream_t s);
cudaError_t launch_record_verify_multi(const uint32_t* computed, const uint32_t* stored, int n, int nElements, uint64_t* payloadOff,
                                       uint32_t* lens, int32_t* status, cudaStream_t s);

}
```

gridfour_b200/csrc/g4_lsop.cu:

```cuda
#include <utility>
#include "g4_kernels.h"
#include "g4_predict.cuh"
#include "g4_huffdec.cuh"
#include "g4_canon.cuh"
#include "g4_canon_fast.cuh"
#include "g4_canon_enc.cuh"
#include "g4_inflate.cuh"
#include "g4_m32stream.cuh"
#include "g4_lsop_common.cuh"

namespace g4 {

namespace {

union LsopDecShared {
  HuffDecShared h;
  CanonDecShared c;
  InflateWarpShared inf;
};


struct CellSink {
  TileView t;
  int order;
// ... 193 lines not shown
  if (h.type != 2 || len > stageWords * 4u || (reinterpret_cast<uintptr_t>(packing) & 3) != 0) {
    if (lane == 0) defer[atomicAdd(deferCount, 1)] = tIdx;
    return;
  }
  const uint32_t nInit = uint32_t(4 * R + 2 * C - 9);
  BitSrc src;
  src.init(packing, len);
  canon_warp_parse_header(W, src, h.headerSize * 8u);
  int status = W.error ? G4_ERR_FORMAT : G4_OK;
  uint32_t endBit = 0;
  if (status == G4_OK) {
    uint32_t eb = 0, nv = 0;
    auto emit = [&](uint32_t k, int32_t v) {
      int r, c;
      stream_to_cell(kStreamLsopInit, int(k), R, C, &r, &c);
      t.at(r, c) = v;
    };
    const bool ok = canon_warp_decode_text(W, src, W.textStart, nInit, emit, &eb, &nv) && nv == nInit;
    __syncwarp();
    if (lane == 0) {
      if (!ok) W.error = 1;
      W.textStart = eb;
    }
    __syncwarp();
    if (W.error) status = G4_ERR_FORMAT;
    endBit = W.textStart;
  }
  if (status == G4_OK) {
    canon_warp_parse_header(W, src, endBit);
    if (W.error) status = G4_ERR_FORMAT;
    else {
      for (int i = lane; i < kCanonSymbols; i += 32) m[8 + i] = W.lens[i];
      if (lane == 0) *reinterpret_cast<uint32_t*>(m) = W.textStart;
    }
  }
  if (status == G4_OK) {
    if (lane == 0) t.at(0, 0) = h.seed;
    __syncwarp();
    row_scan_warp(t.row(0), C, 0);
    __syncwarp();
    lsop_warp_column_scan(t, 0, 1, uint32_t(h.seed), false);
    {
      uint32_t carry = uint32_t(t.at(1, 0)) - uint32_t(t.at(0, 0));
      for (int c0 = 1; c0 < C; c0 += 32) {
        int c = c0 + lane;
        uint32_t x = c < C ? uint32_t(t.at(1, c)) : 0u;
        uint32_t inc = warp_inclusive_scan(x);
        if (c < C) t.at(1, c) = int32_t(carry + inc + uint32_t(t.at(0, c)));
        carry += __shfl_sync(0xffffffffu, inc, 31);
      }
    }
    __syncwarp();
    lsop_warp_column_scan(t, 1, 2, uint32_t(t.at(1, 1)) - uint32_t(t.at(1, 0)), true);
  }
  if (lane == 0) a.status[tIdx] = status;
}

template <class InteriorSink>
__global__ void __launch_bounds__(kThreads, 4) lsop_decode_text_kernel(DecodeArgs a, const uint8_t* meta) {
  extern __shared__ __align__(16) unsigned char lsopFastSmem[];
  CanonFastShared& F = *reinterpret_cast<CanonFastShared*>(lsopFastSmem);
  __shared__ int sTile;
  const int tid = threadIdx.x;
  for (;;) {
    __syncthreads();
    if (tid == 0) sTile = atomicAdd(a.counter, 1);
    __syncthreads();
    const int li = sTile;
    if (li >= *a.listCount) break;
    const int tIdx = a.list[li];
    const uint8_t* m = meta + size_t(tIdx) * kLsopMetaBytes;
    const uint32_t T0 = *reinterpret_cast<const uint32_t*>(m);
    if (T0 == 0) continue;
    const TileView t = tile_view(a.band, a.grid, tIdx);
    const uint8_t* packing = a.arena + a.offsets[tIdx];
    const uint32_t len = a.lens[tIdx];
    const uint32_t nInterior = uint32_t(t.R - 2) * uint32_t(t.C - 4);
    canon_fast_stage(F, packing, len);
    for (int i = tid; i < kCanonSymbols; i += kThreads) F.lens[i] = m[8 + i];
    if (tid == 0) F.error = 0;
    __syncthreads();
    canon_fast_tables_cta(F);
    bool ok = F.error == 0;
    if (ok) {
      canon_fast_build_lut(F);
      uint32_t endBit = 0, nv = 0;
      InteriorSink s2{};
      s2.t = t;
      ok = canon_fast_decode_text(F, len * 8u, T0, nInterior, 0u, s2, &endBit, &nv) && nv == nInterior;
    }
    if (!ok && tid == 0) a.status[tIdx] = G4_ERR_FORMAT;
  }
}

__global__ void __launch_bounds__(kThreads) lsop_decode_entropy_kernel(DecodeArgs a, float* coefOut) {
  __shared__ LsopDecShared S;
  __shared__ int sTile;
  const int tid = threadIdx.x, lane = tid & 31, warp = tid >> 5;
  for (;;) {
    __syncthreads();
    if (tid == 0) sTile = atomicAdd(a.counter, 1);
    __syncthreads();
    const int li = sTile;
    if (li >= *a.listCount) break;
    const int tIdx = a.list[li];
    const TileView t = tile_view(a.band, a.grid, tIdx);
    const int R = t.R, C = t.C;
    const uint8_t* packing = a.arena + a.offsets[tIdx];
    const uint32_t len = a.lens[tIdx];
    int status = G4_OK;
    LsHeaderInfo h = parse_ls_header(packing, len, coefOut + size_t(tIdx) * 12, tid == 0);
    if (tid == 0 && a.lsopCks && h.ok && h.hasChecksum) { a.lsopCks[2 * tIdx] = 1u; a.lsopCks[2 * tIdx + 1] = h.valueChecksum; }
    const uint32_t nInit = uint32_t(4 * R + 2 * C - 9);
    const uint32_t nInterior = uint32_t(R - 2) * uint32_t(C - 4);
    if (!h.ok || R < 6 || C < 6) status = G4_ERR_FORMAT;
    if (status == G4_OK) {
      BitSrc src;
      src.init(packing + h.headerSize, len - h.headerSize);
      if (h.type == 2) {
        uint32_t endBit = 0, nv = 0;
        CellSink s1{t, kStreamLsopInit};
        CellSink s2{t, kStreamLsopInterior};
        if (!canon_decode_stream(S.c, src, 0, nInit, 32768u, s1, &endBit, &nv) || nv != nInit) status = G4_ERR_FORMAT;
        else if (!canon_decode_stream(S.c, src, endBit, nInterior, 0u, s2, &endBit, &nv) || nv != nInterior) status = G4_ERR_FORMAT;
      } else {
        if (h.nInitCodes < nInit || h.nInitCodes > 6 * nInit || h.nInteriorCodes < nInterior || h.nInteriorCodes > 6 * nInterior)
          status = G4_ERR_FORMAT;
        else {
          uint8_t* m32a = a.scratch + size_t(blockIdx.x) * a.scratchStride;
          uint8_t* m32b = m32a + ((size_t(h.nInitCodes) + 31) & ~size_t(15));
          uint32_t endBit = 0;
          bool entropyOk;
          if (h.type == 1) {
            __shared__ int sInfOk;
            if (warp == 0) {
              const uint8_t* z = packing + h.headerSize;
              const uint32_t zLen = len - h.headerSize;
              uint32_t produced = 0, consumed = 0;
              int rc = inflate_warp(S.inf, z, zLen, m32a, h.nInitCodes, &produced, &consumed);
              bool ok = rc == kInfOk && produced == h.nInitCodes && consumed <= zLen;
              if (ok) {
                uint32_t c1 = consumed;
                rc = inflate_warp(S.inf, z + c1, zLen - c1, m32b, h.nInteriorCodes, &produced, &consumed);
                ok = rc == kInfOk && produced == h.nInteriorCodes;
              }
              if (lane == 0) sInfOk = ok ? 1 : 0;
            }
            __syncthreads();
            entropyOk = sInfOk != 0;
          } else {
            entropyOk = huffman_decode_stream(S.h, src, 0, h.nInitCodes, m32a, &endBit) &&
                        huffman_decode_stream(S.h, src, endBit, h.nInteriorCodes, m32b, &endBit);
          }
          if (!entropyOk) status = G4_ERR_FORMAT;
          else {
            __syncthreads();
            __shared__ uint32_t scanM[kWarps + 1];
            if (!m32_parse_to_cells(m32a, h.nInitCodes, kStreamLsopInit, t, nInit, scanM)) status = G4_ERR_FORMAT;
            else if (!m32_parse_to_cells(m32b, h.nInteriorCodes, kStreamLsopInterior, t, nInterior, scanM)) status = G4_ERR_FORMAT;
          }
        }
      }
    }
    if (status == G4_OK) lsop_init_scans(t, h.seed);
    __syncthreads();
    if (tid == 0) a.status[tIdx] = status;
  }
}

__global__ void __launch_bounds__(kThreads) lsop08_decode_entropy_kernel(DecodeArgs a, float* coefOut) {
  __shared__ LsopDecShared S;
  __shared__ int sTile;
  __shared__ uint32_t scanM[kWarps + 1];
  __shared__ int sInfOk;
  const int tid = threadIdx.x, lane = tid & 31, warp = tid >> 5;
  for (;;) {
    __syncthreads();
    if (tid == 0) sTile = atomicAdd(a.counter, 1);
    __syncthreads();
    const int li = sTile;
    if (li >= *a.listCount) break;
    const int tIdx = a.list[li];
    const TileView t = tile_view(a.band, a.grid, tIdx);
    const int R = t.R, C = t.C;
    const uint8_t* packing = a.arena + a.offsets[tIdx];
    const uint32_t len = a.lens[tIdx];
    int status = G4_OK;
    LsHeaderInfo h = parse_ls_header(packing, len, coefOut + size_t(tIdx) * 12, tid == 0, 8);
    const uint32_t nInit = uint32_t((C - 1) + C + 2 * (R - 2));
    const uint32_t nInterior = uint32_t(R - 2) * uint32_t(C - 2);
    if (!h.ok || R < 3 || C < 3) status = G4_ERR_FORMAT;
    else if (h.nInitCodes < nInit || h.nInitCodes > 6 * nInit || h.nInteriorCodes < nInterior || h.nInteriorCodes > 6 * nInterior)
      status = G4_ERR_FORMAT;
    if (status == G4_OK) {
      uint8_t* m32a = a.scratch + size_t(blockIdx.x) * a.scratchStride;
      uint8_t* m32b = m32a + ((size_t(h.nInitCodes) + 31) & ~size_t(15));
      bool entropyOk;
      if (h.type != 0) {
        if (warp == 0) {
          const uint8_t* z = packing + h.headerSize;
          const uint32_t zLen = len - h.headerSize;
          uint32_t produced = 0, consumed = 0;
          int rc = inflate_warp(S.inf, z, zLen, m32a, h.nInitCodes, &produced, &consumed);
          bool ok = rc == kInfOk && produced == h.nInitCodes && consumed <= zLen;
          if (ok) {
            const uint32_t c1 = consumed;
            rc = inflate_warp(S.inf, z + c1, zLen - c1, m32b, h.nInteriorCodes, &produced, &consumed);
            ok = rc == kInfOk && produced == h.nInteriorCodes;
          }
          if (lane == 0) sInfOk = ok ? 1 : 0;
        }
        __syncthreads();
        entropyOk = sInfOk != 0;
      } else {
        BitSrc src;
        src.init(packing + h.headerSize, len - h.headerSize);
        uint32_t endBit = 0;
        entropyOk = huffman_decode_stream(S.h, src, 0, h.nInitCodes, m32a, &endBit) &&
                    huffman_decode_stream(S.h, src, endBit, h.nInteriorCodes, m32b, &endBit);
      }
      if (!entropyOk) status = G4_ERR_FORMAT;
      else {
        __syncthreads();
        if (!m32_parse_to_cells(m32a, h.nInitCodes, kStreamLsop8Init, t, nInit, scanM)) status = G4_ERR_FORMAT;
        else if (!m32_parse_to_cells(m32b, h.nInteriorCodes, kStreamLsop8Interior, t, nInterior, scanM)) status = G4_ERR_FORMAT;
      }
    }
    if (status == G4_OK) {
      __syncthreads();
      if (tid == 0) t.at(0, 0) = h.seed;
      __syncthreads();
      if (warp == 0) row_scan_warp(t.row(0), C, 0);
      if (warp == 1) row_scan_warp(t.row(1), C, 0);
      __syncthreads();
      for (int c = tid; c < C; c += kThreads) t.at(1, c) = int32_t(uint32_t(t.at(1, c)) + uint32_t(h.seed));
      __syncthreads();
      uint32_t carry = uint32_t(t.at(1, 0));
      for (int r0 = 2; r0 < R; r0 += kThreads) {
        const int r = r0 + tid;
        const uint32_t x = r < R ? uint32_t(t.at(r, 0)) : 0u;
        uint32_t tot;
        const uint32_t ex = block_exclusive_scan(x, scanM, &tot);
        if (r < R) {
          const uint32_t v0 = carry + ex + x;
          t.at(r, 0) = int32_t(v0);
          t.at(r, 1) = int32_t(v0 + uint32_t(t.at(r, 1)));
        }
        carry += tot;
      }
    }
    __syncthreads();
    if (tid == 0) a.status[tIdx] = status;
  }
}

__global__ void __launch_bounds__(kThreads) lsop08_wavefront_kernel(DecodeArgs a, const float* coef) {
  const int lane = threadIdx.x & 31, warp = threadIdx.x >> 5;
  const int li = blockIdx.x * kWarps + warp;
  if (li >= *a.listCount) return;
  const int tIdx = a.list[li];
  if (a.status[tIdx] != G4_OK) return;
  const TileView t = tile_view(a.band, a.grid, tIdx);
  const int R = t.R, C = t.C;
  float u[8];
#pragma unroll
  for (int i = 0; i < 8; i++) u[i] = coef[size_t(tIdx) * 12 + i];
  for (int r0 = 2; r0 < R; r0 += 32) {
    const int r = r0 + lane;
    const bool active = r < R;
    const int rr = active ? r : R - 1;
    int32_t* rowp = t.row(rr);
    const int32_t* up1 = t.row(rr - 1);
    const int32_t* up2 = t.row(rr - 2);
    float v1 = float(rowp[1]), v2 = float(rowp[0]);
    const int lastLane = (R - 1 - r0) < 31 ? (R - 1 - r0) : 31;
    const int nSteps = (C - 2) + lastLane;
    __syncwarp();
    for (int s = 0; s < nSteps; s++) {
      const int c = 2 + s - lane;
      if (active && c >= 2 && c < C) {
        const float a1 = float(__ldcg(up1 + c - 1)), a0 = float(__ldcg(up1 + c)), a2 = float(__ldcg(up1 + c - 2));
        const float b2 = float(__ldcg(up2 + c - 2)), b1 = float(__ldcg(up2 + c - 1)), b0 = float(__ldcg(up2 + c));
        float p = u[0] * v1;
        p = p + u[1] * a1;
        p = p + u[2] * a0;
        p = p + u[3] * v2;
        p = p + u[4] * a2;
        p = p + u[5] * b2;
        p = p + u[6] * b1;
        p = p + u[7] * b0;
        const int32_t val = int32_t(uint32_t(__float2int_rz(p + 0.5f)) + uint32_t(rowp[c]));
        rowp[c] = val;
        v2 = v1;
        v1 = float(val);
      }
      __threadfence_block();
      __syncwarp();
    }
  }
}

__global__ void __launch_bounds__(kThreads) lsop_wavefront_kernel(DecodeArgs a, const float* coef) {
  const int lane = threadIdx.x & 31, warp = threadIdx.x >> 5;
  const int li = blockIdx.x * kWarps + warp;
  if (li >= *a.listCount) return;
  const int tIdx = a.list[li];
  if (a.status[tIdx] != G4_OK) return;
  const TileView t = tile_view(a.band, a.grid, tIdx);
  const int R = t.R, C = t.C;
  float u[12];
#pragma unroll
  for (int i = 0; i < 12; i++) u[i] = coef[size_t(tIdx) * 12 + i];

  for (int r0 = 2; r0 < R; r0 += 32) {
    const int r = r0 + lane;
    const bool active = r < R;
    const int rr = active ? r : R - 1;
    int32_t* rowp = t.row(rr);
    const int32_t* up1 = t.row(rr - 1);
    const int32_t* up2 = t.row(rr - 2);
    float z1 = float(rowp[1]), z6 = float(rowp[0]);
    int32_t o1 = rowp[1];
    float z7 = 0.f, z2 = 0.f, z3 = 0.f, z4 = float(up1[0]), z5 = float(up1[1]);
    int32_t i2 = 0, i3 = 0, i4 = up1[0], i5 = up1[1];
    float z8 = 0.f, z9 = 0.f, z10 = 0.f, z11 = float(up2[0]), z12 = float(up2[1]);
    float a0 = 0.f, a1 = 0.f, a2 = 0.f;
    int32_t lastOut = 0;
    const int lastLane = (R - 1 - r0) < 31 ? (R - 1 - r0) : 31;
    const int nSteps = C + 3 * lastLane;
    __syncwarp();
    for (int s = 0; s < nSteps; s++) {
      const int c = s - 3 * lane;
      int32_t recvA = __shfl_up_sync(0xffffffffu, lastOut, 1);
      float recvB = __shfl_up_sync(0xffffffffu, a2, 1);
      const bool shifting = c >= 0 && c < C;
      if (lane == 0 && shifting) {
        int cc = c + 2 < C ? c + 2 : C - 1;
        recvA = __ldcg(up1 + cc);
        recvB = float(__ldcg(up2 + cc));
      }
      if (shifting) {
        float fa = float(recvA);
        z7 = z2; z2 = z3; z3 = z4; z4 = z5; z5 = fa;
        i2 = i3; i3 = i4; i4 = i5; i5 = recvA;
        z8 = z9; z9 = z10; z10 = z11; z11 = z12; z12 = recvB;
        a2 = a1; a1 = a0; a0 = fa;
      }
      if (active && c >= 2 && c < C) {
        int32_t res = rowp[c];
        int32_t val;
        if (c < C - 2) {
          float p = u[0] * z1;
          p = p + u[1] * z2;
          p = p + u[2] * z3;
          p = p + u[3] * z4;
          p = p + u[4] * z5;
          p = p + u[5] * z6;
          p = p + u[6] * z7;
          p = p + u[7] * z8;
          p = p + u[8] * z9;
          p = p + u[9] * z10;
          p = p + u[10] * z11;
          p = p + u[11] * z12;
          val = int32_t(uint32_t(java_round(p)) + uint32_t(res));
        } else {
          val = int32_t(uint32_t(res) + ((uint32_t(o1) + uint32_t(i3)) - uint32_t(i2)));
        }
        rowp[c] = val;
        lastOut = val;
        z6 = z1;
        z1 = float(val);
        o1 = val;
      }
    }
    __syncwarp();
    __threadfence_block();
  }
}

__global__ void __launch_bounds__(kThreads, 3) lsop_wavefront4_kernel(DecodeArgs a, const float* coef) {
  const int lane = threadIdx.x & 31, warp = threadIdx.x >> 5;
  const int li = blockIdx.x * kWarps + warp;
  if (li >= *a.listCount) return;
  const int tIdx = a.list[li];
  if (a.status[tIdx] != G4_OK) return;
  const TileView t = tile_view(a.band, a.grid, tIdx);
  const int R = t.R, C = t.C;
  const bool feeder = lane < 2;
  float u[12];
#pragma unroll
  for (int i = 0; i < 12; i++) u[i] = feeder ? 0.f : coef[size_t(tIdx) * 12 + i];
  const int P = C > 136 ? C : 136;
  const int nB = P >> 2, cBlocks = C >> 2;
  const int nGroups = (R - 2 + 29) / 30;
  const int nIter = nGroups * nB + 31;
  const int64_t wrapStep = 30 * t.pitch - 4 * int64_t(nB);
  float av[8], bv[8];
#pragma unroll
  for (int i = 0; i < 8; i++) { av[i] = 0.f; bv[i] = 0.f; }
  float f1 = 0.f, f2 = 0.f;
  float pf0 = 0.f, pf1 = 0.f;
  int32_t h1 = 0;
  int32_t po1 = 0, po2 = 0, po3 = 0;
  int cb = -lane, r = lane;
  int32_t* p = t.base + int64_t(r) * t.pitch + 4 * cb;
  int4 vN = make_int4(0, 0, 0, 0);
  if (cb == 0 && r < R) vN = *reinterpret_cast<const int4*>(p);
  for (int it = 0; it < nIter; it++) {
    const bool act = cb >= 0 && cb < cBlocks && r < R;
    const bool first = cb == 0;
    const bool triangle = cb == cBlocks - 1 && !feeder;
    const int4 v = vN;
    int32_t* const cur = p;
    cb++;
    p += 4;
    if (cb == nB) { cb = 0; r += 30; p += wrapStep; }
    if (cb >= 0 && cb < cBlocks && r < R) vN = *reinterpret_cast<const int4*>(p);
    const float s0 = __shfl_up_sync(0xffffffffu, pf0, 1);
    const float s1 = __shfl_up_sync(0xffffffffu, pf1, 1);
    const float s2 = __shfl_up_sync(0xffffffffu, av[2], 1);
    const float s3 = __shfl_up_sync(0xffffffffu, av[3], 1);
#pragma unroll
    for (int i = 0; i < 4; i++) { av[i] = av[i + 4]; bv[i] = bv[i + 4]; }
    if (first) { av[2] = s0; av[3] = s1; bv[2] = s2; bv[3] = s3; }
    const int32_t upy = __shfl_up_sync(0xffffffffu, po1, 1);
    const int32_t upz = __shfl_up_sync(0xffffffffu, po2, 1);
    const int32_t upw = __shfl_up_sync(0xffffffffu, po3, 1);
    int32_t out[4];
#pragma unroll
    for (int j = 0; j < 4; j++) {
      av[4 + j] = __shfl_up_sync(0xffffffffu, f2, 1);
      bv[4 + j] = __shfl_up_sync(0xffffffffu, av[j], 1);
      const int32_t res = j == 0 ? v.x : j == 1 ? v.y : j == 2 ? v.z : v.w;
      float q = u[0] * f1;
      q = q + u[1] * av[j + 1];
      q = q + u[2] * av[j + 2];
      q = q + u[3] * av[j + 3];
      q = q + u[4] * av[j + 4];
      q = q + u[5] * f2;
      q = q + u[6] * av[j];
      q = q + u[7] * bv[j];
      q = q + u[8] * bv[j + 1];
      q = q + u[9] * bv[j + 2];
      q = q + u[10] * bv[j + 3];
      q = q + u[11] * bv[j + 4];
      uint32_t add = uint32_t(java_round(q));
      if (j < 2) {
        if (first) add = 0u;
      } else {
        const int32_t upc = j == 2 ? upz : upw, upl = j == 2 ? upy : upz;
        if (triangle) add = (uint32_t(h1) + uint32_t(upc)) - uint32_t(upl);
      }
      const int32_t val = int32_t(uint32_t(res) + add);
      out[j] = val;
      h1 = val;
      f2 = f1;
      f1 = float(val);
      if (j == 0) pf0 = f1;
      if (j == 1) pf1 = f1;
    }
    if (act && !feeder) *reinterpret_cast<int4*>(cur) = make_int4(out[0], out[1], out[2], out[3]);
    po1 = out[1]; po2 = out[2]; po3 = out[3];
    __syncwarp();
  }
}

namespace {

constexpr int kMomentQuantities = 104;
constexpr int kMomentPerRole = 26;

__host__ __device__ constexpr int moment_i(int q) {
  int k = q - 13, i = 0;
  while (k >= 13 - i) { k -= 13 - i; i++; }
  return i;
}
__host__ __device__ constexpr int moment_j(int q) {
  int k = q - 13, i = 0;
  while (k >= 13 - i) { k -= 13 - i; i++; }
  return i + k;
}

template <int Q>
__device__ __forceinline__ double moment_term(const double (&z)[13]) {
  if constexpr (Q < 13) return z[Q];
  else {
    constexpr int i = moment_i(Q), j = moment_j(Q);
    return z[i] * z[j];
  }
}
template <int ROLE, int... A>
__device__ __forceinline__ void moment_accumulate_seq(const double (&z)[13], double (&acc)[kMomentPerRole], std::integer_sequence<int, A...>) {
  ((acc[A] += moment_term<A * 4 + ROLE>(z)), ...);
}
template <int ROLE>
__device__ __forceinline__ void moment_accumulate(const double (&z)[13], double (&acc)[kMomentPerRole]) {
  moment_accumulate_seq<ROLE>(z, acc, std::make_integer_sequence<int, kMomentPerRole>{});
}

struct LsopEncShared {
  CanonEncShared E;
  BitWindow W;
  double part[kWarps][kMomentPerRole];
  double sums[kMomentQuantities];
  double M[13][13];
  double rhs[13];
  float u[12];
  int singular;
};

__device__ bool lu_solve13(double (*LU)[13], double* X) {
  const int n = 13;
  int piv[13];
  for (int i = 0; i < n; i++) piv[i] = i;
  double col[13];
  for (int j = 0; j < n; j++) {
    for (int i = 0; i < n; i++) col[i] = LU[i][j];
    for (int i = 0; i < n; i++) {
      int kmax = i < j ? i : j;
      double s = 0.0;
      for (int k = 0; k < kmax; k++) s += LU[i][k] * col[k];
      col[i] -= s;
      LU[i][j] = col[i];
    }
    int p = j;
    for (int i = j + 1; i < n; i++)
      if (fabs(col[i]) > fabs(col[p])) p = i;
    if (p != j) {
      for (int k = 0; k < n; k++) { double t = LU[p][k]; LU[p][k] = LU[j][k]; LU[j][k] = t; }
      int k = piv[p]; piv[p] = piv[j]; piv[j] = k;
    }
    if (LU[j][j] != 0.0)
      for (int i = j + 1; i < n; i++) LU[i][j] /= LU[j][j];
  }
  for (int j = 0; j < n; j++)
    if (LU[j][j] == 0.0) return false;
  double B[13];
  for (int i = 0; i < n; i++) B[i] = X[piv[i]];
  for (int i = 0; i < n; i++) X[i] = B[i];
  for (int k = 0; k < n; k++)
    for (int i = k + 1; i < n; i++) X[i] -= X[k] * LU[i][k];
  for (int k = n - 1; k >= 0; k--) {
    X[k] /= LU[k][k];
    for (int i = 0; i < k; i++) X[i] -= X[k] * LU[i][k];
  }
  return true;
}

struct LsInitGet {
  TileView t;
  __device__ __forceinline__ int32_t operator()(uint32_t k) const {
    int r, c;
    stream_to_cell(kStreamLsopInit, int(k), t.R, t.C, &r, &c);
    return residual_at(G4_PRED_TRIANGLE, t, r, c);
  }
};

struct LsInteriorGet {
  TileView t;
  const float* u;
  __device__ __forceinline__ int32_t operator()(uint32_t k) const {
    const int w = t.C - 4;
    int rr = int(k) / w;
    int r = 2 + rr, c = 2 + int(k) - rr * w;
    const int32_t* row = t.row(r);
    const int32_t* up1 = row - t.pitch;
    const int32_t* up2 = up1 - t.pitch;
    float p = u[0] * float(row[c - 1]);
    p = p + u[1] * float(up1[c - 1]);
    p = p + u[2] * float(up1[c]);
    p = p + u[3] * float(up1[c + 1]);
    p = p + u[4] * float(up1[c + 2]);
    p = p + u[5] * float(row[c - 2]);
    p = p + u[6] * float(up1[c - 2]);
    p = p + u[7] * float(up2[c - 2]);
    p = p + u[8] * float(up2[c - 1]);
    p = p + u[9] * float(up2[c]);
    p = p + u[10] * float(up2[c + 1]);
    p = p + u[11] * float(up2[c + 2]);
    return int32_t(uint32_t(row[c]) - uint32_t(java_round(p)));
  }
};

}

__global__ void __launch_bounds__(kThreads) lsop_encode_kernel(EncodeArgs a) {
  extern __shared__ __align__(16) unsigned char smemRaw[];
  LsopEncShared& S = *reinterpret_cast<LsopEncShared*>(smemRaw);
  __shared__ int sTile;
  __shared__ uint32_t sMaxAbs;
  const int tid = threadIdx.x, lane = tid & 31, warp = tid >> 5;
  const int nTiles = a.band.tiles_down * a.band.tiles_across;
  uint8_t* pm = a.scratch + size_t(blockIdx.x) * a.scratchStride;
  for (;;) {
    __syncthreads();
    if (tid == 0) sTile = atomicAdd(a.counter, 1);
    __syncthreads();
    const int tIdx = sTile;
    if (tIdx >= nTiles) break;
    const TileView t = tile_view(a.band, a.grid, tIdx);
    const int R = t.R, C = t.C;
    uint32_t* outWords = reinterpret_cast<uint32_t*>(a.slots + size_t(tIdx) * a.slotBytes);
    const uint32_t capWords = uint32_t(a.slotBytes / 4);
    if (R < 6 || C < 6) {
      if (tid == 0) { a.lens[tIdx] = 0; a.preds[tIdx] = 0; a.status[tIdx] = G4_DECLINED; }
      continue;
    }
    {
      const int role = warp & 3, group = warp >> 2;
      const int w = C - 4;
      const int nInterior = (R - 2) * w;
      if (tid == 0) sMaxAbs = 0u;
      __syncthreads();
      {
        uint32_t mx = 0u;
        for (int m = tid; m < R * C; m += kThreads) {
          const int rr = m / C;
          const int32_t v = t.row(rr)[m - rr * C];
          const uint32_t av = v < 0 ? 0u - uint32_t(v) : uint32_t(v);
          mx = mx > av ? mx : av;
        }
        mx = __reduce_max_sync(0xffffffffu, mx);
        if (lane == 0) atomicMax(&sMaxAbs, mx);
      }
      double acc[kMomentPerRole];
#pragma unroll
      for (int i = 0; i < kMomentPerRole; i++) acc[i] = 0.0;
      for (int m = group * 32 + lane; m < nInterior; m += 64) {
        int rr = m / w;
        int r = 2 + rr, c = 2 + m - rr * w;
        const int32_t* row = t.row(r);
        const int32_t* up1 = row - t.pitch;
        const int32_t* up2 = up1 - t.pitch;
        double z[13];
        z[0] = row[c]; z[1] = row[c - 1]; z[2] = up1[c - 1]; z[3] = up1[c]; z[4] = up1[c + 1]; z[5] = up1[c + 2];
        z[6] = row[c - 2]; z[7] = up1[c - 2]; z[8] = up2[c - 2]; z[9] = up2[c - 1]; z[10] = up2[c]; z[11] = up2[c + 1];
        z[12] = up2[c + 2];
        switch (role) {
          case 0: moment_accumulate<0>(z, acc); break;
          case 1: moment_accumulate<1>(z, acc); break;
          case 2: moment_accumulate<2>(z, acc); break;
          default: moment_accumulate<3>(z, acc); break;
        }
      }
#pragma unroll
      for (int i = 0; i < kMomentPerRole; i++) {
        double v = acc[i];
#pragma unroll
        for (int d = 16; d >= 1; d >>= 1) v += __shfl_xor_sync(0xffffffffu, v, d);
        if (lane == 0) S.part[warp][i] = v;
      }
      __syncthreads();
      if (tid < kMomentQuantities) S.sums[tid] = S.part[tid & 3][tid >> 2] + S.part[(tid & 3) + 4][tid >> 2];
      const double mag = double(sMaxAbs);
      if (!(double(nInterior) * mag * mag < 9007199254740992.0) && tid < kMomentQuantities) {
        const int dr[13] = {0, 0, -1, -1, -1, -1, 0, -1, -2, -2, -2, -2, -2};
        const int dc[13] = {0, -1, -1, 0, 1, 2, -2, -2, -2, -1, 0, 1, 2};
        const int qi = tid < 13 ? tid : moment_i(tid), qj = tid < 13 ? -1 : moment_j(tid);
        double accq = 0.0;
        for (int r = 2; r < R; r++) {
          const int32_t* ri = t.row(r + dr[qi]) + dc[qi];
          const int32_t* rj = qj >= 0 ? t.row(r + dr[qj]) + dc[qj] : ri;
          if (qj < 0) for (int c = 2; c < C - 2; c++) accq += double(ri[c]);
          else for (int c = 2; c < C - 2; c++) accq += double(ri[c]) * double(rj[c]);
        }
        S.sums[tid] = accq;
      }
      __syncthreads();
    }
    if (tid == 0) {
      double cfull[13][13];
      for (int q = 13; q < kMomentQuantities; q++) {
        int i = moment_i(q), j = moment_j(q);
        cfull[i][j] = S.sums[q];
        cfull[j][i] = S.sums[q];
      }
      for (int i = 0; i < 13; i++) for (int j = 0; j < 13; j++) S.M[i][j] = 0.0;
      for (int i = 1; i < 13; i++) {
        for (int j = 1; j < 13; j++) S.M[i - 1][j - 1] = cfull[i][j];
        S.M[i - 1][12] = S.sums[i];
      }
      for (int j = 1; j < 13; j++) S.M[12][j - 1] = S.sums[j];
      for (int i = 1; i < 13; i++) S.rhs[i - 1] = cfull[0][i];
      S.rhs[12] = S.sums[0];
      bool ok = lu_solve13(S.M, S.rhs);
      S.singular = ok ? 0 : 1;
      if (ok)
        for (int i = 0; i < 12; i++) S.u[i] = __double2float_rn(S.rhs[i]);
    }
    __syncthreads();
    if (S.singular) {
      if (tid == 0) { a.lens[tIdx] = 0; a.preds[tIdx] = 0; a.status[tIdx] = G4_DECLINED; }
      continue;
    }
    const uint32_t nInit = uint32_t(4 * R + 2 * C - 9);
    const uint32_t nInterior = uint32_t(R - 2) * uint32_t(C - 4);
    BitOut o;
    bitwin_reset(S.W, o, outWords, capWords);
    if (tid == 0) {
      WinSink sink{S.W.win, 0};
      sink.put(uint32_t(a.codecIndex) & 0xffu, 8);
      sink.put(0x40u | 2u, 8);
      sink.put(12, 8);
      sink.put(uint32_t(t.at(0, 0)), 32);
      for (int i = 0; i < 12; i++) sink.put(__float_as_uint(S.u[i]), 32);
    }
    o.bitPos = 55u * 8u;
    __syncthreads();
    LsInitGet g1{t};
    LsInteriorGet g2{t, S.u};
    bool bad = false;
    bool clean = canon_histogram(S.E, g1, nInit);
    canon_build_code(S.E, pm);
    if (!clean && !canon_reconcile_escapes(S.E, g1, nInit)) bad = true;
    else {
      canon_emit_stream(S.E, S.W, o, g1, nInit);
      clean = canon_histogram(S.E, g2, nInterior);
      canon_build_code(S.E, pm);
      if (!clean && !canon_reconcile_escapes(S.E, g2, nInterior)) bad = true;
      else canon_emit_stream(S.E, S.W, o, g2, nInterior);
    }
    if (bad) {
      if (tid == 0) { a.lens[tIdx] = 0; a.preds[tIdx] = 0; a.status[tIdx] = G4_DECLINED; }
      continue;
    }
    bitwin_finish(S.W, o);
    if (tid == 0) {
      uint32_t len = (o.bitPos + 7) >> 3;
      a.lens[tIdx] = len;
      a.preds[tIdx] = 2;
      a.status[tIdx] = len <= a.slotBytes ? G4_OK : G4_ERR_CAPACITY;
    }
  }
}

namespace {
__device__ __forceinline__ void load_slot_coefficients(const uint8_t* slot, float* u) {
  if (threadIdx.x < 12) u[threadIdx.x] = __uint_as_float(load_le32(slot + 7 + 4 * threadIdx.x));
  __syncthreads();
}
}

__global__ void __launch_bounds__(kThreads) lsop_m32_size_kernel(EncodeArgs a, uint32_t* inLen) {
  __shared__ uint32_t scan[kWarps + 1];
  __shared__ float u[12];
  const int nTiles = a.band.tiles_down * a.band.tiles_across;
  for (int tIdx = blockIdx.x; tIdx < nTiles; tIdx += gridDim.x) {
    __syncthreads();
    if (a.status[tIdx] != G4_OK || a.lens[tIdx] < 55) {
      if (threadIdx.x == 0) inLen[2 * tIdx] = inLen[2 * tIdx + 1] = 0;
      continue;
    }
    const TileView t = tile_view(a.band, a.grid, tIdx);
    load_slot_coefficients(a.slots + size_t(tIdx) * a.slotBytes, u);
    const uint32_t nInit = uint32_t(4 * t.R + 2 * t.C - 9);
    const uint32_t nInterior = uint32_t(t.R - 2) * uint32_t(t.C - 4);
    uint32_t s0 = m32_stream_size(LsInitGet{t}, nInit, scan);
    uint32_t s1 = m32_stream_size(LsInteriorGet{t, u}, nInterior, scan);
    if (threadIdx.x == 0) { inLen[2 * tIdx] = s0; inLen[2 * tIdx + 1] = s1; }
  }
}

__global__ void __launch_bounds__(kThreads) lsop_m32_write_kernel(EncodeArgs a, const uint32_t* inLen, const uint64_t* inOff,
                                                                  uint8_t* inBuf) {
  __shared__ uint32_t scan[kWarps + 1];
  __shared__ float u[12];
  const int nTiles = a.band.tiles_down * a.band.tiles_across;
  for (int tIdx = blockIdx.x; tIdx < nTiles; tIdx += gridDim.x) {
    __syncthreads();
    if (inLen[2 * tIdx + 1] == 0) continue;
    const TileView t = tile_view(a.band, a.grid, tIdx);
    load_slot_coefficients(a.slots + size_t(tIdx) * a.slotBytes, u);
    const uint32_t nInit = uint32_t(4 * t.R + 2 * t.C - 9);
    const uint32_t nInterior = uint32_t(t.R - 2) * uint32_t(t.C - 4);
    uint8_t* d0 = inBuf + inOff[2 * tIdx];
    uint8_t* d1 = inBuf + inOff[2 * tIdx + 1];
    uint32_t w0 = m32_stream_write(LsInitGet{t}, nInit, d0, scan);
    uint32_t w1 = m32_stream_write(LsInteriorGet{t, u}, nInterior, d1, scan);
    if (threadIdx.x < 16) { d0[w0 + threadIdx.x] = 0; d1[w1 + threadIdx.x] = 0; }
  }
}

__global__ void __launch_bounds__(kThreads) lsop_pick_kernel(EncodeArgs a, const uint32_t* inLen, const uint64_t* inOff,
                                                             const uint8_t* outBuf, const uint32_t* outLen) {
  const int tid = threadIdx.x;
  const int nTiles = a.band.tiles_down * a.band.tiles_across;
  for (int tIdx = blockIdx.x; tIdx < nTiles; tIdx += gridDim.x) {
    if (inLen[2 * tIdx + 1] == 0) continue;
    const uint32_t canonLength = a.lens[tIdx] - 55u;
    const uint32_t initN = outLen[2 * tIdx], insideN = outLen[2 * tIdx + 1];
    if (insideN == 0 || insideN >= canonLength) continue;
    if (initN == 0 || initN + insideN >= canonLength) continue;
    const uint32_t len = 63u + initN + insideN;
    if (len > a.slotBytes) {
      if (tid == 0) a.status[tIdx] = G4_ERR_CAPACITY;
      continue;
    }
    uint8_t* slot = a.slots + size_t(tIdx) * a.slotBytes;
    if (tid == 0) {
      slot[1] = uint8_t(0x40u | 1u);
      const uint32_t n0 = inLen[2 * tIdx], n1 = inLen[2 * tIdx + 1];
      for (int k = 0; k < 4; k++) { slot[55 + k] = uint8_t(n0 >> (8 * k)); slot[59 + k] = uint8_t(n1 >> (8 * k)); }
      a.lens[tIdx] = len;
      a.preds[tIdx] = 1;
    }
    const uint8_t* s0 = outBuf + inOff[2 * tIdx] + 112ull * uint64_t(2 * tIdx);
    const uint8_t* s1 = outBuf + inOff[2 * tIdx + 1] + 112ull * uint64_t(2 * tIdx + 1);
    for (uint32_t i = tid; i < initN; i += kThreads) slot[63 + i] = s0[i];
    for (uint32_t i = tid; i < insideN; i += kThreads) slot[63 + initN + i] = s1[i];
  }
}

cudaError_t launch_lsop_m32_size(const EncodeArgs& a, uint32_t* inLen, int nCtas, cudaStream_t s) {
  lsop_m32_size_kernel<<<nCtas, kThreads, 0, s>>>(a, inLen);
  return cudaGetLastError();
}
cudaError_t launch_lsop_m32_write(const EncodeArgs& a, const uint32_t* inLen, const uint64_t* inOff, uint8_t* inBuf, int nCtas,
                                  cudaStream_t s) {
  lsop_m32_write_kernel<<<nCtas, kThreads, 0, s>>>(a, inLen, inOff, inBuf);
  return cudaGetLastError();
}
cudaError_t launch_lsop_pick(const EncodeArgs& a, const uint32_t* inLen, const uint64_t* inOff, const uint8_t* outBuf,
                             const uint32_t* outLen, int nCtas, cudaStream_t s) {
  lsop_pick_kernel<<<nCtas, kThreads, 0, s>>>(a, inLen, inOff, outBuf, outLen);
  return cudaGetLastError();
}

cudaError_t launch_lsop_encode(const EncodeArgs& a, int nCtas, cudaStream_t s) {
  static std::atomic<uint64_t> attr{0};
  cudaError_t ea = once_per_device(attr, [] {
    return cudaFuncSetAttribute(lsop_encode_kernel, cudaFuncAttributeMaxDynamicSharedMemorySize, int(sizeof(LsopEncShared)));
  });
  if (ea != cudaSuccess) return ea;
  lsop_encode_kernel<<<nCtas, kThreads, sizeof(LsopEncShared), s>>>(a);
  return cudaGetLastError();
}

size_t lsop_meta_bytes() { return kLsopMetaBytes; }

cudaError_t launch_lsop08_decode(const DecodeArgs& a, float* coef, int nCtas, int nTilesUpper, cudaStream_t s) {
  lsop08_decode_entropy_kernel<<<nCtas < 296 ? nCtas : 296, kThreads, 0, s>>>(a, coef);
  cudaError_t e = cudaGetLastError();
  if (e != cudaSuccess) return e;
  lsop08_wavefront_kernel<<<(nTilesUpper + kWarps - 1) / kWarps, kThreads, 0, s>>>(a, coef);
  return cudaGetLastError();
}

cudaError_t launch_lsop_decode(const DecodeArgs& a, float* coef, uint8_t* meta, int* defer, int* deferCounters, int nCtas,
                               int nTilesUpper, cudaStream_t s, int* launches,
                               const LsopFastArgs* fast, int smCount) {
  if (fast) {
    LsopFastArgs A = *fast;
    A.a = a;
    A.coef = coef;
    A.meta = meta;
    A.defer = defer;
    A.deferCount = deferCounters;
    int nLaunch = 0;
    cudaError_t e = launch_lsop_decode_fast(A, nTilesUpper, smCount, deferCounters + 2, s, &nLaunch);
    if (e != cudaSuccess) return e;
    DecodeArgs d = a;
    d.list = defer;
    d.listCount = deferCounters;
    d.counter = deferCounters + 1;
    lsop_decode_entropy_kernel<<<nCtas < 296 ? nCtas : 296, kThreads, 0, s>>>(d, coef);
    if ((e = cudaGetLastError()) != cudaSuccess) return e;
    lsop_wavefront_kernel<<<(nTilesUpper + kWarps - 1) / kWarps, kThreads, 0, s>>>(d, coef);
    if (launches) *launches = nLaunch + 2;
    return cudaGetLastError();
  }
  constexpr uint32_t kMaxStageWords = (192u * 1024u) / 4u;
  uint32_t stageWords = uint32_t((uint64_t(a.band.tile_rows) * uint64_t(a.band.tile_cols) * 5 / 8 + 3) / 4);
  if (stageWords < uint32_t(kFastStageWords)) stageWords = kFastStageWords;
  if (stageWords > kMaxStageWords) stageWords = kMaxStageWords;
  stageWords = (stageWords + 255u) & ~255u;
  const size_t textSmem = canon_fast_smem_bytes(stageWords);
  static std::atomic<uint64_t> attr{0};
  {
    cudaError_t ea = once_per_device(attr, [] {
      const int maxSmem = int(canon_fast_smem_bytes(kMaxStageWords));
      cudaError_t e1 = cudaFuncSetAttribute(lsop_decode_text_kernel<InteriorRunSink>, cudaFuncAttributeMaxDynamicSharedMemorySize, maxSmem);
      if (e1 == cudaSuccess)
        e1 = cudaFuncSetAttribute(lsop_decode_text_kernel<InteriorPackedSink>, cudaFuncAttributeMaxDynamicSharedMemorySize, maxSmem);
      return e1;
    });
    if (ea != cudaSuccess) return ea;
  }
  const bool aligned = (a.band.tile_cols % 4) == 0 && (a.band.grid_pitch % 4) == 0 && a.band.tile_cols >= 8 &&
                       (reinterpret_cast<uintptr_t>(a.grid) & 15) == 0;
  const int nBlocks = (nTilesUpper + kWarps - 1) / kWarps;
  lsop_decode_head_kernel<<<nBlocks, kThreads, 0, s>>>(a, coef, meta, defer, deferCounters, stageWords);
  cudaError_t e = cudaGetLastError();
  if (e != cudaSuccess) return e;
  DecodeArgs t = a;
  t.counter = deferCounters + 2;
  const int ctas = nCtas < nTilesUpper ? nCtas : nTilesUpper;
  if (aligned) lsop_decode_text_kernel<InteriorPackedSink><<<ctas, kThreads, textSmem, s>>>(t, meta);
  else lsop_decode_text_kernel<InteriorRunSink><<<ctas, kThreads, textSmem, s>>>(t, meta);
  if ((e = cudaGetLastError()) != cudaSuccess) return e;
  DecodeArgs d = a;
  d.list = defer;
  d.listCount = deferCounters;
  d.counter = deferCounters + 1;
  lsop_decode_entropy_kernel<<<nCtas < 296 ? nCtas : 296, kThreads, 0, s>>>(d, coef);
  if ((e = cudaGetLastError()) != cudaSuccess) return e;
  if (aligned) lsop_wavefront4_kernel<<<nBlocks, kThreads, 0, s>>>(a, coef);
  else lsop_wavefront_kernel<<<nBlocks, kThreads, 0, s>>>(a, coef);
  if (launches) *launches = 4;
  return cudaGetLastError();
}

}
```

gridfour_b200/csrc/g4_lsop_fast.cu:

```cuda
#include <cuda.h>
#include <cstdio>
#include <type_traits>
#include "g4_kernels.h"
#include "g4_predict.cuh"
#include "g4_lsop_common.cuh"

namespace g4 {

namespace {

constexpr int kTextThreads = 512;
constexpr int kTextThreadsSmall = 256;
constexpr uint32_t kTextSmallTile = 16384;
constexpr uint32_t kTextSubBits = 320;
constexpr int kExcWords = 128;
constexpr int kExcCap = (kExcWords - 2) / 2;
constexpr uint32_t kTextLookback = 96;
constexpr int kStageWordsPerThread = 22;
constexpr int kSpillWords = 8;
constexpr int kResidGuard = 256;
constexpr float kMagicHalf = 6291456.0f;
constexpr float kMagicHalfUp = 6291456.5f;
constexpr float kMagicInt = 12582912.0f;
constexpr float kRange = 2097152.0f;

__device__ __forceinline__ uint32_t smem_u32(const void* p) { return uint32_t(__cvta_generic_to_shared(p)); }
__host__ __device__ constexpr size_t text_fast_bytes(uint32_t stageWords) {
  return (offsetof(CanonFastShared, sw) + size_t(stageWords + 8u) * 4u + 127u) & ~size_t(127);
}
__device__ __forceinline__ void mbar_init(uint32_t bar, uint32_t count) {
  asm volatile("mbarrier.init.shared::cta.b64 [%0], %1;" ::"r"(bar), "r"(count));
}
__device__ __forceinline__ void mbar_expect_tx(uint32_t bar, uint32_t bytes) {
  asm volatile("mbarrier.arrive.expect_tx.shared::cta.b64 _, [%0], %1;" ::"r"(bar), "r"(bytes) : "memory");
}
__device__ __forceinline__ void mbar_wait(uint32_t bar, uint32_t parity) {
  uint32_t done = 0;
  while (!done)
    asm volatile("{ .reg .pred p; mbarrier.try_wait.parity.shared::cta.b64 p, [%1], %2; selp.u32 %0, 1, 0, p; }"
                 : "=r"(done)
                 : "r"(bar), "r"(parity)
                 : "memory");
}

__device__ __forceinline__ uint32_t image_offset(uint32_t w, int logW, uint32_t P, uint32_t k) {
  const uint32_t rr = k / w, pp = k - rr * w;
  return (rr + (pp >> logW)) * P + pp;
}

__device__ inline uint32_t warp_scan_inplace(int32_t* p, int n, uint32_t carry, int stride = 1) {
  const int lane = threadIdx.x & 31;
  for (int i0 = 0; i0 < n; i0 += 32) {
    const int i = i0 + lane;
    const uint32_t x = i < n ? uint32_t(p[i * stride]) : 0u;
    const uint32_t inc = warp_inclusive_scan(x);
    if (i < n) p[i * stride] = int32_t(carry + inc);
    carry += __shfl_sync(0xffffffffu, inc, 31);
  }
  __syncwarp();
  return carry;
}

__global__ void __launch_bounds__(kThreads, 3) lsop2_head_kernel(LsopFastArgs A, uint32_t maxPackBytes, int listBegin, int listEnd) {
  extern __shared__ __align__(16) unsigned char headSmem[];
  const DecodeArgs& a = A.a;
  const int lane = threadIdx.x & 31, warp = threadIdx.x >> 5;
  const int R = A.g.R, C = A.g.C;
  const uint32_t nInit = uint32_t(4 * R + 2 * C - 9);
  const size_t perWarp = ((sizeof(CanonWarpShared) + 15) & ~size_t(15)) + ((size_t(nInit) * 4 + 15) & ~size_t(15));
  CanonWarpShared& W = *reinterpret_cast<CanonWarpShared*>(headSmem + perWarp * warp);
  int32_t* init = reinterpret_cast<int32_t*>(headSmem + perWarp * warp + ((sizeof(CanonWarpShared) + 15) & ~size_t(15)));
  const int li = listBegin + blockIdx.x * kWarps + warp;
  if (li >= listEnd || li >= *a.listCount) return;
  const int tIdx = a.list[li];
  uint8_t* m = A.meta + size_t(tIdx) * kLsopMetaBytes;
  if (lane == 0) {
    *reinterpret_cast<uint32_t*>(m) = 0;
    A.exc[size_t(tIdx) * kExcWords] = 0;
  }
  const TileView t = tile_view(a.band, a.grid, tIdx);
  const uint8_t* packing = a.arena + a.offsets[tIdx];
  const uint32_t len = a.lens[tIdx];
  LsHeaderInfo h = parse_ls_header(packing, len, A.coef + size_t(tIdx) * 12, lane == 0);
  if (lane == 0 && a.lsopCks && h.ok && h.hasChecksum) { a.lsopCks[2 * tIdx] = 1u; a.lsopCks[2 * tIdx + 1] = h.valueChecksum; }
  if (!h.ok) {
    if (lane == 0) a.status[tIdx] = G4_ERR_FORMAT;
    return;
  }
  if (h.type != 2 || len + 96u > maxPackBytes) {
    if (lane == 0) A.defer[atomicAdd(A.deferCount, 1)] = tIdx;
    return;
  }
  BitSrc src;
  src.init(packing, len);
  canon_warp_parse_header(W, src, h.headerSize * 8u);
  int status = W.error ? G4_ERR_FORMAT : G4_OK;
  uint32_t endBit = 0;
  if (status == G4_OK) {
    uint32_t eb = 0, nv = 0;
    auto emit = [&](uint32_t k, int32_t v) { init[k] = v; };
    const bool ok = canon_warp_decode_text(W, src, W.textStart, nInit, emit, &eb, &nv) && nv == nInit;
    __syncwarp();
    if (lane == 0) {
      if (!ok) W.error = 1;
      W.textStart = eb;
    }
    __syncwarp();
    if (W.error) status = G4_ERR_FORMAT;
    endBit = W.textStart;
  }
  if (status == G4_OK) {
    canon_warp_parse_header(W, src, endBit);
    if (W.error) status = G4_ERR_FORMAT;
    else {
      for (int i = lane; i < kCanonSymbols; i += 32) {
        m[8 + i] = W.lens[i];
        reinterpret_cast<uint16_t*>(m + kLsopMetaSorted)[i] = W.sorted[i];
      }
      if (lane < 17) {
        reinterpret_cast<uint16_t*>(m + kLsopMetaFirst)[lane] = W.firstCode[lane];
        reinterpret_cast<uint16_t*>(m + kLsopMetaCount)[lane] = W.count[lane];
        reinterpret_cast<uint16_t*>(m + kLsopMetaOffset)[lane] = W.offset[lane];
      }
      if (lane == 0) *reinterpret_cast<uint32_t*>(m) = W.textStart;
    }
  }
  if (status == G4_OK) {
    int32_t* sA = init;
    int32_t* sB = sA + (C - 1);
    int32_t* sC = sB + (R - 1);
    int32_t* sD = sC + (C - 1);
    int32_t* sE = sD + (R - 2);
    const uint32_t seed = uint32_t(h.seed);
    warp_scan_inplace(sA, C - 1, seed);
    warp_scan_inplace(sB, R - 1, seed);
    warp_scan_inplace(sC, C - 1, uint32_t(sB[0]) - seed);
    for (int i = lane; i < C - 1; i += 32) sC[i] = int32_t(uint32_t(sC[i]) + uint32_t(sA[i]));
    __syncwarp();
    warp_scan_inplace(sD, R - 2, uint32_t(sC[0]) - uint32_t(sB[0]));
    warp_scan_inplace(sE, R - 2, uint32_t(sC[C - 3]) - uint32_t(sC[C - 4]), 2);
    warp_scan_inplace(sE + 1, R - 2, uint32_t(sC[C - 2]) - uint32_t(sC[C - 3]), 2);
    int32_t* row0 = t.row(0);
    int32_t* row1 = t.row(1);
    for (int c = lane; c < C; c += 32) {
      row0[c] = c ? sA[c - 1] : int32_t(seed);
      row1[c] = c ? sC[c - 1] : sB[0];
    }
    int4* side = A.side + size_t(tIdx) * R;
    for (int r = lane; r < R; r += 32) {
      int4 s;
      if (r == 0) s = make_int4(int32_t(seed), sA[0], 0, 0);
      else if (r == 1) s = make_int4(sB[0], sC[0], 0, 0);
      else s = make_int4(sB[r - 1], int32_t(uint32_t(sB[r - 1]) + uint32_t(sD[r - 2])), sE[2 * (r - 2)], sE[2 * (r - 2) + 1]);
      side[r] = s;
    }
  }
  if (lane == 0) a.status[tIdx] = status;
}

struct ByteTileSink {
  static constexpr bool kPacked = true;
  uint8_t* tile;
  uint32_t* exc;
  int w;
  int logW;
  uint32_t P, Wm1;
  uint32_t addr;
  uint32_t rowBase;
  int left;
  int kAddr;
  int head;
  int cnt;
  uint64_t q;
  int excK, excSlot;
  int32_t excV;

  __device__ __forceinline__ void init(uint8_t* img, uint32_t* e, const LsopFastGeom& geom) {
    tile = img;
    exc = e;
    logW = geom.logW;
    w = geom.C - 4;
    P = uint32_t(geom.P);
    Wm1 = uint32_t(geom.W - 1);
  }
  __device__ __forceinline__ void begin(uint32_t k0) {
    const int rr = int(k0) / w, pp = int(k0) - rr * w;
    rowBase = uint32_t(rr) * P;
    const uint32_t a0 = rowBase + (uint32_t(pp) >> logW) * P + uint32_t(pp);
    head = pp & 3;
    addr = a0 & ~3u;
    left = w - (pp & ~3);
    kAddr = int(k0) - head;
    cnt = head;
    q = 0;
    excK = -1;
    excSlot = 0;
    excV = 0;
  }
  __device__ __forceinline__ int cur_k() const { return kAddr + cnt; }
  __device__ __forceinline__ void store_word() {
    if (head) {
      for (int i = head; i < 4; i++) tile[addr + i] = uint8_t(q >> (8 * i));
      head = 0;
    } else *reinterpret_cast<uint32_t*>(tile + addr) = uint32_t(q);
    q >>= 32;
    cnt -= 4;
    kAddr += 4;
    step();
  }
  __device__ __forceinline__ void step() {
    addr += 4;
    left -= 4;
    if ((addr & Wm1) == 0u) {
      addr += P;
      if (left == 0) {
        rowBase += P;
        addr = rowBase;
        left = w;
      }
    } else if (__builtin_expect(left == 0, 0)) {
      rowBase += P;
      addr = rowBase;
      left = w;
    }
  }
  __device__ __forceinline__ void put_word(uint32_t dw, int lo, int hi) {
    if (lo == 0 && hi >= 4) *reinterpret_cast<uint32_t*>(tile + addr) = dw;
    else
      for (int b = lo; b < hi && b < 4; b++) tile[addr + b] = uint8_t(dw >> (8 * b));
    step();
  }
  __device__ __forceinline__ void push(uint32_t bytes, int n) {
    q |= uint64_t(bytes) << (8 * cnt);
    cnt += n;
    if (cnt >= 4) store_word();
  }
  __device__ __forceinline__ int add_exception(int k, int32_t v) {
    const uint32_t slot = atomicAdd(exc, 1u);
    if (slot < uint32_t(kExcCap)) {
      exc[2 + 2 * slot] = uint32_t(k);
      exc[3 + 2 * slot] = uint32_t(v);
    }
    excK = k;
    excV = v;
    excSlot = int(slot);
    return int(slot);
  }
  __device__ __forceinline__ void put_rare(int32_t v) {
    add_exception(cur_k(), v);
    push(0u, 1);
  }
  __device__ __forceinline__ void amend(int nb, uint32_t bits) {
    const int kp = cur_k() - 1;
    if (kp == excK) {
      excV = int32_t((uint32_t(excV) << nb) | bits);
      if (excSlot < kExcCap) exc[3 + 2 * excSlot] = uint32_t(excV);
      return;
    }
    uint32_t b;
    if (cnt > head) {
      const int sh = 8 * (cnt - 1);
      b = uint32_t(q >> sh) & 0xffu;
      q &= ~(0xffull << sh);
    } else {
      const uint32_t o = image_offset(uint32_t(w), logW, P, uint32_t(kp));
      b = tile[o];
      tile[o] = 0;
    }
    add_exception(kp, int32_t(((b - 128u) << nb) | bits));
  }
  __device__ __forceinline__ void end() {
    for (int i = head; i < cnt; i++) tile[addr + i] = uint8_t(q >> (8 * i));
  }
};

constexpr int kSubRare = 4;
constexpr int kSubOverflow = 8;

struct PosCursor {
  uint32_t lo, hi, next, pos;
  __device__ __forceinline__ void init(const uint32_t* sw, uint32_t p) {
    const uint32_t i = p >> 5;
    lo = sw[i];
    hi = sw[i + 1];
    next = i + 2;
    pos = p;
  }
  __device__ __forceinline__ uint32_t peek() const { return __funnelshift_r(lo, hi, pos); }
  __device__ __forceinline__ void skip(const uint32_t* sw, uint32_t n) {
    const uint32_t np = pos + n;
    if ((np ^ pos) & 32u) {
      lo = hi;
      hi = sw[next++];
    }
    pos = np;
  }
};

struct ByteAcc {
  uint32_t acc, qc8, w;
  __device__ __forceinline__ void init() { acc = 0; qc8 = 0; w = 0; }
  __device__ __forceinline__ void append(uint32_t m24, uint32_t n8, uint32_t* slot, uint32_t slotWords, uint32_t* spill) {
    const uint32_t out = __funnelshift_l(acc, m24, qc8);
    acc = __funnelshift_r(acc, m24, n8);
    qc8 += n8;
    if (qc8 >= 32u) {
      if (w < slotWords) slot[w] = out;
      else if (w - slotWords < uint32_t(kSpillWords)) spill[w - slotWords] = out;
      w++;
      qc8 -= 32u;
    }
  }
  __device__ __forceinline__ void finish(uint32_t* slot, uint32_t slotWords, uint32_t* spill) {
    if (qc8) {
      const uint32_t out = acc >> (32u - qc8);
      if (w < slotWords) slot[w] = out;
      else if (w - slotWords < uint32_t(kSpillWords)) spill[w - slotWords] = out;
      w++;
    }
  }
};

__device__ __forceinline__ void text_stage_sub(const CanonFastShared& S, uint32_t nBits, uint32_t start, uint32_t limit, uint32_t* slot,
                                               uint32_t slotWords, uint32_t* spill, uint32_t* endOut, uint32_t* cntOut, int* flagOut) {
  PosCursor cur;
  cur.init(S.sw, start);
  const int lastFull = int(limit) - kFastLutBits;
  uint32_t c = 0, end;
  int flag = 0;
  ByteAcc A;
  A.init();
  for (;;) {
    if (int(cur.pos) <= lastFull) {
      const uint32_t m = S.mlut[cur.peek() & ((1u << kFastLutBits) - 1u)];
      const uint32_t n = m >> 28;
      if (n) {
        cur.skip(S.sw, (m >> 24) & 15u);
        c += n;
        A.append(m & 0xffffffu, (m >> 25) & 0x18u, slot, slotWords, spill);
        continue;
      }
    }
    const uint32_t e = S.lut[cur.peek() & ((1u << kFastLutBits) - 1u)];
    uint32_t byte;
    if (e - 1u < 0x7fffu) {
      if (cur.pos >= limit) { end = cur.pos; break; }
      cur.skip(S.sw, e >> 9);
      byte = e & 0xffu;
    } else {
      const uint32_t p0 = cur.pos;
      uint32_t after;
      const int sym = canon_fast_rare_symbol(S, e, p0, nBits, &after);
      if (sym < 0) { flag = 2; end = p0; break; }
      if (sym == kSymEsc2 || sym == kSymEsc8) {
        after += sym == kSymEsc2 ? 2u : 8u;
        if (after > nBits) { flag = 2; end = p0; break; }
        flag |= kSubRare;
        cur.init(S.sw, after);
        continue;
      }
      if (p0 >= limit) { end = p0; break; }
      if (sym == kSymEot) { flag |= 1; end = after; break; }
      if (sym == kSymNull) { flag |= kSubRare; byte = 0u; }
      else byte = uint32_t(sym);
      cur.init(S.sw, after);
    }
    c++;
    A.append(byte, 8u, slot, slotWords, spill);
  }
  A.finish(slot, slotWords, spill);
  if (A.w > slotWords + uint32_t(kSpillWords)) flag |= kSubOverflow;
  *endOut = end;
  *cntOut = c;
  *flagOut = flag;
}

__device__ __forceinline__ bool text_write_sub(const CanonFastShared& S, uint32_t nBits, uint32_t start, uint32_t limit, uint32_t k0,
                                            ByteTileSink& sink) {
  BitCursor cur;
  cur.init(S, start, limit);
  sink.begin(k0);
  bool have = false, ok = true;
  for (;;) {
    if (cur.rem >= kFastLutBits) {
      const uint32_t m = S.mlut[cur.peek() & ((1u << kFastLutBits) - 1u)];
      const uint32_t n = m >> 28;
      if (n) {
        cur.skip(S, (m >> 24) & 15u);
        sink.push(m & 0xffffffu, int(n));
        have = true;
        continue;
      }
    }
    const uint32_t e = S.lut[cur.peek() & ((1u << kFastLutBits) - 1u)];
    if (e - 1u < 0x7fffu) {
      if (cur.rem <= 0) break;
      cur.skip(S, e >> 9);
      sink.push(e & 0xffu, 1);
      have = true;
      continue;
    }
    const uint32_t p0 = cur.pos(limit);
    uint32_t after;
    const int sym = canon_fast_rare_symbol(S, e, p0, nBits, &after);
    if (sym < 0) { ok = false; break; }
    if (sym == kSymEsc2 || sym == kSymEsc8) {
      const int nb = sym == kSymEsc2 ? 2 : 8;
      if (!have || after + nb > nBits) { ok = false; break; }
      SmemBitSrc src{S.sw, nBits};
      sink.amend(nb, src.bits(after, nb));
      after += nb;
    } else {
      if (p0 >= limit || sym == kSymEot) break;
      if (sym == kSymNull) sink.put_rare(INT32_MIN);
      else sink.push(uint32_t(sym), 1);
      have = true;
    }
    cur.init(S, after, limit);
  }
  sink.end();
  return ok;
}

__device__ __noinline__ void text_exceptions_sub(const CanonFastShared& S, uint32_t nBits, uint32_t start, uint32_t limit, uint32_t k0,
                                                 uint8_t* tile, uint32_t* exc, int w, int logW, uint32_t P) {
  auto image_off = [&](uint32_t k) { return image_offset(uint32_t(w), logW, P, k); };
  auto add = [&](uint32_t k, int32_t v) {
    const uint32_t slot = atomicAdd(exc, 1u);
    if (slot < uint32_t(kExcCap)) {
      exc[2 + 2 * slot] = k;
      exc[3 + 2 * slot] = uint32_t(v);
    }
  };
  SmemBitSrc src{S.sw, nBits};
  uint32_t pos = start, k = k0, pk = 0;
  bool pending = false;
  int32_t pv = 0;
  for (;;) {
    const uint32_t e = S.lut[src.peek32(pos) & ((1u << kFastLutBits) - 1u)];
    int sym;
    uint32_t after;
    if (e - 1u < 0x7fffu) { sym = int(e & 0xffu); after = pos + (e >> 9); }
    else {
      sym = canon_fast_rare_symbol(S, e, pos, nBits, &after);
      if (sym < 0) break;
    }
    if (sym == kSymEsc2 || sym == kSymEsc8) {
      const int nb = sym == kSymEsc2 ? 2 : 8;
      if (after + nb > nBits || k == k0) break;
      if (!pending) {
        pk = k - 1;
        const uint32_t o = image_off(pk);
        pv = int32_t(tile[o]) - 128;
        tile[o] = 0;
        pending = true;
      }
      pv = int32_t((uint32_t(pv) << nb) | src.bits(after, nb));
      after += nb;
    } else {
      if (pending) { add(pk, pv); pending = false; }
      if (pos >= limit || sym == kSymEot) break;
      if (sym == kSymNull) add(k, INT32_MIN);
      k++;
    }
    pos = after;
  }
  if (pending) add(pk, pv);
}

template <int NT>
__device__ int lsop_text_decode(CanonFastShared& S, uint32_t nBits, const uint32_t T0, uint32_t nInterior, uint32_t imageBytes,
                                ByteTileSink sink, uint32_t* spillArea) {
  constexpr int kRounds = kFastMaxSub / NT;
  const int tid = threadIdx.x;
  const uint32_t avail = nBits - T0;
  uint32_t rounds = (avail / kTextSubBits + NT - 1) / NT;
  if (rounds < 1u) rounds = 1u;
  if (rounds > uint32_t(kRounds)) rounds = kRounds;
  uint32_t B = (avail + rounds * NT - 1) / (rounds * NT);
  if (B < 96u) B = 96u;
  const int nSub = int((avail + B - 1) / B);
  uint32_t slotWords = (imageBytes / uint32_t(nSub)) >> 2;
  if (slotWords > uint32_t(kStageWordsPerThread) / rounds) slotWords = uint32_t(kStageWordsPerThread) / rounds;
  if (uint64_t(slotWords + uint32_t(kSpillWords)) * 4u * uint64_t(nSub) * 3u < uint64_t(nInterior) * 4u) return 2;
  uint32_t* const image32 = reinterpret_cast<uint32_t*>(sink.tile);
  if (tid == 0) S.firstEot = nSub;
#pragma unroll 1
  for (int i = tid; i < nSub; i += NT) {
    uint32_t limit = T0 + uint32_t(i + 1) * B;
    if (limit > nBits) limit = nBits;
    uint32_t from = T0 + uint32_t(i) * B;
    if (limit - from > kTextLookback) from = limit - kTextLookback;
    uint32_t e, c;
    int f;
    canon_fast_count(S, nBits, from, limit, &e, &c, &f);
    S.endpos[i] = e;
    S.startv[i] = 0xffffffffu;
  }
  volatile uint32_t* vend = S.endpos;
  __syncthreads();
  for (int pass = 0; pass <= nSub; pass++) {
    bool any = false;
#pragma unroll 1
    for (int i = tid; i < nSub; i += NT) {
      const uint32_t ns = i ? vend[i - 1] : T0;
      if (ns != S.startv[i]) {
        S.startv[i] = ns;
        uint32_t limit = T0 + uint32_t(i + 1) * B;
        if (limit > nBits) limit = nBits;
        uint32_t e, c;
        int f;
        text_stage_sub(S, nBits, ns, limit, image32 + size_t(i) * slotWords, slotWords, spillArea + size_t(i) * kSpillWords, &e, &c, &f);
        vend[i] = e;
        S.cnt[i] = uint16_t(c);
        S.eot[i] = uint8_t(f);
        any = true;
      }
    }
    if (!__syncthreads_or(any ? 1 : 0)) break;
  }
#pragma unroll 1
  for (int i = tid; i < nSub; i += NT)
    if (S.eot[i] & 3) atomicMin(&S.firstEot, i);
  __syncthreads();
  const int fe = S.firstEot;
  if (fe == nSub || (S.eot[fe] & 3) == 2) return 1;
  uint32_t mySum = 0;
#pragma unroll
  for (int j = 0; j < kRounds; j++) {
    const int i = tid * kRounds + j;
    mySum += (i <= fe && i < nSub) ? S.cnt[i] : 0u;
  }
  uint32_t total;
  const uint32_t ex = block_exclusive_scan<NT>(mySum, S.scan, &total);
  if (total != nInterior) return 1;
  uint32_t* offv = S.endpos;
  {
    uint32_t run = ex;
#pragma unroll
    for (int j = 0; j < kRounds; j++) {
      const int i = tid * kRounds + j;
      if (i < nSub) {
        offv[i] = run;
        run += (i <= fe) ? S.cnt[i] : 0u;
      }
    }
  }
  uint32_t r[kStageWordsPerThread];
#pragma unroll
  for (int j = 0; j < kStageWordsPerThread; j++) r[j] = 0;
  {
    const uint32_t perSub = uint32_t(kStageWordsPerThread) / rounds;
    for (uint32_t s = 0; s < rounds; s++) {
      const int i = tid + int(s) * NT;
      if (i <= fe && !(S.eot[i] & kSubOverflow)) {
        const uint32_t* slot = image32 + size_t(i) * slotWords;
#pragma unroll
        for (int j = 0; j < kStageWordsPerThread; j++)
          if (uint32_t(j) >= s * perSub && uint32_t(j) < s * perSub + slotWords) r[j] = slot[uint32_t(j) - s * perSub];
      }
    }
  }
  __syncthreads();
  bool bad = false;
  {
    const uint32_t perSub = uint32_t(kStageWordsPerThread) / rounds;
    for (uint32_t s = 0; s < rounds; s++) {
      const int i = tid + int(s) * NT;
      if (i > fe) continue;
      const uint32_t n = S.cnt[i];
      const int flags = S.eot[i];
      uint32_t limit = T0 + uint32_t(i + 1) * B;
      if (limit > nBits) limit = nBits;
      if (flags & kSubOverflow) {
        if (!text_write_sub(S, nBits, S.startv[i], limit, offv[i], sink)) bad = true;
        continue;
      }
      if (n == 0) continue;
      sink.begin(offv[i]);
      if (rounds == 1u) {
        const int head = sink.head;
        const uint32_t sh = 8u * uint32_t(head);
        const int nD = int((n + uint32_t(head) + 3u) >> 2);
        const uint32_t* sp = spillArea + size_t(i) * kSpillWords;
        uint32_t prev = 0;
#pragma unroll
        for (int d = 0; d < kStageWordsPerThread + kSpillWords + 1; d++) {
          if (d >= nD) break;
          uint32_t cur = 0;
          if (d < kStageWordsPerThread && uint32_t(d) < slotWords) cur = r[d];
          else if (uint32_t(d) >= slotWords && uint32_t(d) - slotWords < uint32_t(kSpillWords) && 4u * uint32_t(d) < n) cur = sp[uint32_t(d) - slotWords];
          sink.put_word(__funnelshift_l(prev, cur, sh), d == 0 ? head : 0, int(n) + head - 4 * d);
          prev = cur;
        }
        if (flags & kSubRare) text_exceptions_sub(S, nBits, S.startv[i], limit, offv[i], sink.tile, sink.exc, sink.w, sink.logW, sink.P);
        continue;
      }
#pragma unroll
      for (int j = 0; j < kStageWordsPerThread; j++) {
        const uint32_t at = (uint32_t(j) - s * perSub) * 4u;
        if (uint32_t(j) >= s * perSub && uint32_t(j) < s * perSub + slotWords && at < n) {
          const uint32_t m = n - at;
          sink.push(m >= 4u ? r[j] : (r[j] & ((1u << (8 * m)) - 1u)), m >= 4u ? 4 : int(m));
        }
      }
      if (n > slotWords * 4u) {
        const uint32_t* sp = spillArea + size_t(i) * kSpillWords;
        for (uint32_t at = slotWords * 4u; at < n; at += 4u) {
          const uint32_t wv = *sp++, m = n - at;
          sink.push(m >= 4u ? wv : (wv & ((1u << (8 * m)) - 1u)), m >= 4u ? 4 : int(m));
        }
      }
      sink.end();
      if (flags & kSubRare) text_exceptions_sub(S, nBits, S.startv[i], limit, offv[i], sink.tile, sink.exc, sink.w, sink.logW, sink.P);
    }
  }
  return __syncthreads_or(bad ? 1 : 0) ? 1 : 0;
}

template <int NT>
__global__ void __launch_bounds__(NT, NT == 512 ? 2 : 4) lsop2_text_kernel(LsopFastArgs A, uint32_t stageWords, int listBegin, int listEnd) {
  extern __shared__ __align__(128) unsigned char textSmem[];
  CanonFastShared& F = *reinterpret_cast<CanonFastShared*>(textSmem);
  uint8_t* tileImg = textSmem + text_fast_bytes(stageWords);
  __shared__ int sTile[2];
  __shared__ __align__(8) uint64_t sBar;
  const DecodeArgs& a = A.a;
  const int tid = threadIdx.x;
  const uint32_t bar = smem_u32(&sBar);
  if (tid == 0) {
    mbar_init(bar, 1);
    asm volatile("fence.mbarrier_init.release.cluster;");
    sTile[0] = listBegin + atomicAdd(a.counter, 1);
  }
  __syncthreads();
  uint32_t parity = 0;
  for (int phase = 0;; phase ^= 1) {
    const int li = sTile[phase];
    if (li >= listEnd || li >= *a.listCount) break;
    if (tid == 0) sTile[phase ^ 1] = listBegin + atomicAdd(a.counter, 1);
    const int tIdx = a.list[li];
    const uint8_t* m = A.meta + size_t(tIdx) * kLsopMetaBytes;
    const uint32_t T0 = *reinterpret_cast<const uint32_t*>(m);
    if (T0 == 0) { __syncthreads(); continue; }
    const uint8_t* packing = a.arena + a.offsets[tIdx];
    const uint32_t len = a.lens[tIdx];
    const uint32_t delta = uint32_t(reinterpret_cast<uintptr_t>(packing) & 15u);
    const uint8_t* src16 = packing - delta;
    const uint32_t span = len + delta, nBulk = span & ~15u;
    if (tid == 0 && nBulk) {
      mbar_expect_tx(bar, nBulk);
      asm volatile("cp.async.bulk.shared::cluster.global.mbarrier::complete_tx::bytes [%0], [%1], %2, [%3];" ::"r"(smem_u32(F.sw)), "l"(src16),
                   "r"(nBulk), "r"(bar)
                   : "memory");
    }
    if (tid < 64) {
      const uint32_t i = nBulk + uint32_t(tid);
      reinterpret_cast<uint8_t*>(F.sw)[i] = i < span ? src16[i] : uint8_t(0);
    }
    for (int i = tid; i < kCanonSymbols; i += NT) F.sorted[i] = reinterpret_cast<const uint16_t*>(m + kLsopMetaSorted)[i];
    if (tid < 17) {
      F.firstCode[tid] = reinterpret_cast<const uint16_t*>(m + kLsopMetaFirst)[tid];
      F.count[tid] = reinterpret_cast<const uint16_t*>(m + kLsopMetaCount)[tid];
      F.offset[tid] = reinterpret_cast<const uint16_t*>(m + kLsopMetaOffset)[tid];
    }
    if (tid == 0) F.error = 0;
    __syncthreads();
    bool ok = true;
    canon_fast_build_lut<NT>(F);
    if (nBulk) mbar_wait(bar, parity);
    parity ^= nBulk ? 1u : 0u;
    __syncthreads();
    int rc = ok ? 0 : 1;
    if (ok) {
      const uint32_t nInterior = uint32_t(A.g.R - 2) * uint32_t(A.g.C - 4);
      ByteTileSink sink;
      sink.init(tileImg, A.exc + size_t(tIdx) * kExcWords, A.g);
      if (tid == 0) asm volatile("cp.async.bulk.wait_group.read 0;" ::: "memory");
      rc = lsop_text_decode<NT>(F, span * 8u, T0 + 8u * delta, nInterior, uint32_t(A.g.tileBytes), sink,
                                reinterpret_cast<uint32_t*>(A.textStage) + size_t(blockIdx.x) * (kFastMaxSub * kSpillWords));
      if (rc == 2) {
        uint32_t endBit = 0, nv = 0;
        rc = (canon_fast_decode_text<ByteTileSink, NT, kTextSubBits>(F, span * 8u, T0 + 8u * delta, nInterior, 0u, sink, &endBit, &nv) &&
              nv == nInterior) ? 0 : 1;
      }
      ok = rc == 0;
    }
    __syncthreads();
    if (tid == 0) {
      if (rc == 1) a.status[tIdx] = G4_ERR_FORMAT;
      else if (A.exc[size_t(tIdx) * kExcWords] > uint32_t(kExcCap)) {
        A.exc[size_t(tIdx) * kExcWords] = uint32_t(kExcCap) + 1u;
        A.defer[atomicAdd(A.deferCount, 1)] = tIdx;
      }
      else {
        asm volatile("fence.proxy.async.shared::cta;" ::: "memory");
        uint8_t* dst = A.resid + kResidGuard + size_t(tIdx) * size_t(A.g.tilePitch);
        asm volatile("cp.async.bulk.global.shared::cta.bulk_group [%0], [%1], %2;" ::"l"(dst), "r"(smem_u32(tileImg)), "r"(uint32_t(A.g.tileBytes))
                     : "memory");
        asm volatile("cp.async.bulk.commit_group;" ::: "memory");
      }
    }
  }
  if (tid == 0) asm volatile("cp.async.bulk.wait_group 0;" ::: "memory");
}

#ifndef G4_WAVE_CTAS
#define G4_WAVE_CTAS 2
#endif
#ifndef G4_WAVE_WARPS
#define G4_WAVE_WARPS 8
#endif
constexpr int kWaveWarps = G4_WAVE_WARPS;
constexpr int kWaveChunkBytes = 4096;

__device__ __noinline__ int32_t wave_exception(const uint32_t* exc, int n, int k) {
  for (int i = 0; i < n; i++)
    if (int(exc[2 + 2 * i]) == k) return int32_t(exc[3 + 2 * i]);
  return -128;
}

__device__ __forceinline__ int wave_rowbuf_floats(int C) { return (C + 4 + 3) & ~3; }

template <int W, bool WIDE>
__global__ void __launch_bounds__(32 * kWaveWarps, G4_WAVE_CTAS) lsop3_wave_kernel(LsopFastArgs A, int* tileCounter, int listBegin, int listEnd) {
  extern __shared__ __align__(128) unsigned char waveSmem[];
  constexpr int CR = 128 / W;
  constexpr int NW = W / 4;
  constexpr int E = W - 4;
  const DecodeArgs& a = A.a;
  const int lane = threadIdx.x & 31, warp = threadIdx.x >> 5;
  const LsopFastGeom& G = A.g;
  const int R = G.R, C = G.C, nS = G.nStrips, P = G.P;
  const int rbFloats = wave_rowbuf_floats(C);
  unsigned char* ring = waveSmem + size_t(warp) * (2 * kWaveChunkBytes);
  float* rowbuf = reinterpret_cast<float*>(waveSmem + size_t(kWaveWarps) * (2 * kWaveChunkBytes)) + size_t(warp) * (2 * rbFloats);
  uint64_t* bars = reinterpret_cast<uint64_t*>(waveSmem + size_t(kWaveWarps) * (2 * kWaveChunkBytes) + size_t(kWaveWarps) * (2 * rbFloats) * sizeof(float)) + 2 * warp;
  const uint32_t bar0 = smem_u32(bars), ring0 = smem_u32(ring);
  const bool active = lane < nS, isFirst = lane == 0, isLast = lane == nS - 1;
  if (lane == 0) {
    mbar_init(bar0, 1);
    mbar_init(bar0 + 8, 1);
    asm volatile("fence.mbarrier_init.release.cluster;");
  }
  __syncwarp();
  uint32_t gchunk = 0;
  for (;;) {
  int li = 0;
  if (lane == 0) li = listBegin + atomicAdd(tileCounter, 1);
  li = __shfl_sync(0xffffffffu, li, 0);
  if (li >= listEnd || li >= *a.listCount) break;
  const int tIdx = a.list[li];
  if (a.status[tIdx] != G4_OK) continue;
  if (*reinterpret_cast<const uint32_t*>(A.meta + size_t(tIdx) * kLsopMetaBytes) == 0u) continue;
  const uint32_t* exc = A.exc + size_t(tIdx) * kExcWords;
  const int nExc = int(exc[0]);
  if (nExc > kExcCap) continue;
  const TileView t = tile_view(a.band, a.grid, tIdx);
  const uint8_t* img = A.resid + kResidGuard + size_t(tIdx) * size_t(G.tilePitch);
  const uint32_t chunkBytes = uint32_t(CR * P);
  const int nChunks = G.nChunks;
  auto issue = [&](int chunk) {
    const uint32_t g = gchunk + uint32_t(chunk);
    const uint32_t bar = bar0 + 8u * (g & 1u), dst = ring0 + uint32_t(kWaveChunkBytes) * (g & 1u);
    mbar_expect_tx(bar, chunkBytes);
    asm volatile("cp.async.bulk.shared::cluster.global.mbarrier::complete_tx::bytes [%0], [%1], %2, [%3];" ::"r"(dst),
                 "l"(img + size_t(chunk) * chunkBytes), "r"(chunkBytes), "r"(bar)
                 : "memory");
  };
  if (lane == 0) issue(0);

  float u[12];
#pragma unroll
  for (int i = 0; i < 12; i++) u[i] = active ? A.coef[size_t(tIdx) * 12 + i] : 0.f;
  for (int c = lane; c < rbFloats; c += 32) {
    rowbuf[c] = c < C ? float(t.row(0)[c]) : 0.f;
    rowbuf[rbFloats + c] = c < C ? float(t.row(1)[c]) : 0.f;
  }
  const int4* side = A.side + size_t(tIdx) * R;
  const bool needSide = active && (isFirst || isLast);
  uint32_t rr = active ? uint32_t(-lane) : 0x40000000u;
  const uint32_t nRowsIn = uint32_t(R - 2);
  int4 sideCur = make_int4(0, 0, 0, 0), sideNext = make_int4(0, 0, 0, 0);
  if (needSide && rr < nRowsIn) sideNext = side[2 + rr];
  const int4* sideAt = side + 3 - lane;
  char* rowp = reinterpret_cast<char*>(t.base + int64_t(2 - lane) * t.pitch + lane * W);
  const int64_t rowStep = int64_t(t.pitch) * 4;
  const uint32_t ringLane = ring0 + uint32_t(lane * W);
  uint32_t ringAt = ringLane;
  const uint32_t rb0 = smem_u32(rowbuf) + uint32_t(lane * W) * 4u, rb1 = rb0 + uint32_t(rbFloats) * 4u;
  const int wInterior = C - 4;
  uint32_t badBits = 0;
  float a0[W + 4], a1[W + 4], a2[W + 4];
#pragma unroll
  for (int i = 0; i < W + 4; i++) { a0[i] = 0.f; a1[i] = 0.f; a2[i] = 0.f; }
  int32_t pa = 0, pb = 0;
  float h0 = 0.f, h1 = 0.f;
  __syncwarp();

  auto step = [&](float (&am2)[W + 4], float (&am1)[W + 4], float (&cur)[W + 4], const int s) {
    if ((s & (CR - 1)) == 0) {
      const int chunk = s / CR;
      if (chunk < nChunks) {
        if (lane == 0 && chunk + 1 < nChunks) issue(chunk + 1);
        const uint32_t g = gchunk + uint32_t(chunk);
        mbar_wait(bar0 + 8u * (g & 1u), (g >> 1) & 1u);
      }
      ringAt = ringLane + uint32_t(kWaveChunkBytes) * ((gchunk + uint32_t(chunk)) & 1u);
    }
    const bool valid = rr < nRowsIn;
    const bool first = rr == 0u;
    if (s < nS) {
     if (first) {
#pragma unroll
      for (int i = 0; i < W + 4; i += 4) {
        float4 x, y;
        asm volatile("ld.shared.v4.f32 {%0, %1, %2, %3}, [%4];" : "=f"(x.x), "=f"(x.y), "=f"(x.z), "=f"(x.w) : "r"(rb0 + 4u * i));
        asm volatile("ld.shared.v4.f32 {%0, %1, %2, %3}, [%4];" : "=f"(y.x), "=f"(y.y), "=f"(y.z), "=f"(y.w) : "r"(rb1 + 4u * i));
        am2[i] = x.x; am2[i + 1] = x.y; am2[i + 2] = x.z; am2[i + 3] = x.w;
        am1[i] = y.x; am1[i + 1] = y.y; am1[i + 2] = y.z; am1[i + 3] = y.w;
      }
      h0 = am1[W + 2];
      h1 = am1[W + 3];
     }
    }
    sideCur = sideNext;
    if (needSide && rr + 1u < nRowsIn) sideNext = *sideAt;
    sideAt++;
    uint32_t rw[NW];
    {
      const uint32_t at = ringAt;
      ringAt += uint32_t(P);
      if constexpr (NW == 1) asm volatile("ld.shared.b32 %0, [%1];" : "=r"(rw[0]) : "r"(at));
      else if constexpr (NW == 2) asm volatile("ld.shared.v2.b32 {%0, %1}, [%2];" : "=r"(rw[0]), "=r"(rw[1]) : "r"(at));
      else asm volatile("ld.shared.v4.b32 {%0, %1, %2, %3}, [%4];" : "=r"(rw[0]), "=r"(rw[1]), "=r"(rw[2]), "=r"(rw[3]) : "r"(at));
    }
    float l2 = __shfl_up_sync(0xffffffffu, am1[W], 1), l1 = __shfl_up_sync(0xffffffffu, am1[W + 1], 1);
    int32_t li2 = __shfl_up_sync(0xffffffffu, pa, 1), li1 = __shfl_up_sync(0xffffffffu, pb, 1);
    if (isFirst) { li2 = sideCur.x; li1 = sideCur.y; l2 = float(li2); l1 = float(li1); }
    cur[0] = l2;
    cur[1] = l1;
    bool general = false;
    if (nExc > 0) {
      bool z = false;
#pragma unroll
      for (int i = 0; i < NW; i++) z = z || ((rw[i] - 0x01010101u) & ~rw[i] & 0x80808080u) != 0u;
      general = __any_sync(0xffffffffu, z && valid);
    }
    int32_t oi[W];
    uint32_t accLo = 0, accHi = 0;
    auto cells = [&](auto genTag) {
      constexpr bool GEN = decltype(genTag)::value;
#pragma unroll
      for (int j = 0; j < W; j++) {
        constexpr int dummy = 0;
        (void)dummy;
        const int c = j + 2;
        if (j == 2) {
          const float s0 = __shfl_down_sync(0xffffffffu, cur[2], 1), s1 = __shfl_down_sync(0xffffffffu, cur[3], 1);
          am1[W + 2] = first ? h0 : s0;
          am1[W + 3] = first ? h1 : s1;
        }
        float p = u[0] * cur[c - 1];
        p = p + u[1] * am1[c - 1];
        p = p + u[2] * am1[c];
        p = p + u[3] * am1[c + 1];
        p = p + u[4] * am1[c + 2];
        p = p + u[5] * cur[c - 2];
        p = p + u[6] * am1[c - 2];
        p = p + u[7] * am2[c - 2];
        p = p + u[8] * am2[c - 1];
        p = p + u[9] * am2[c];
        p = p + u[10] * am2[c + 1];
        p = p + u[11] * am2[c + 2];
        const float t1 = __fadd_rd(p, kMagicHalf);
        if (j < E) accLo |= __float_as_uint(t1) ^ 0x4A800000u;
        else accHi |= __float_as_uint(t1) ^ 0x4A800000u;
        const float t2 = __fadd_rd(t1, kMagicHalfUp);
        const uint32_t word = rw[j >> 2];
        const float xj = __uint_as_float(__byte_perm(word, 0x4B400000u, 0x7640 + (j & 3)));
        float fv = t2 + (xj - (2.f * kMagicInt + 128.f));
        int32_t iv;
        if constexpr (GEN) {
          const uint32_t byte = (word >> (8 * (j & 3))) & 0xffu;
          int32_t ex = int32_t(byte) - 128;
          if (byte == 0u && valid) ex = wave_exception(exc, nExc, int(rr) * wInterior + lane * W + j);
          iv = int32_t(uint32_t(__float_as_int(t2)) - 0x4B400000u + uint32_t(ex));
          fv = float(iv);
        } else iv = int32_t(uint32_t(__float_as_int(t2)) + __float_as_uint(xj) - 0x96800080u);
        if (j == E || j == E + 1) {
          const int32_t prev = j == 0 ? li1 : oi[j > 0 ? j - 1 : 0];
          const int32_t sv = int32_t(uint32_t(prev) + uint32_t(j == E ? sideCur.z : sideCur.w));
          if (isLast) { iv = sv; fv = float(sv); }
        }
        oi[j] = iv;
        cur[c] = fv;
      }
    };
    if (general) cells(std::true_type{});
    else cells(std::false_type{});
    if (valid) badBits |= (accLo | (isLast ? 0u : accHi)) & 0xFF800000u;
    if (valid) {
      if constexpr (W == 4) *reinterpret_cast<int4*>(rowp) = make_int4(li2, li1, oi[0], oi[1]);
      else {
        if (WIDE) {
          asm volatile("st.global.v8.b32 [%0], {%1,%2,%3,%4,%5,%6,%7,%8};" ::"l"(rowp), "r"(li2), "r"(li1), "r"(oi[0]), "r"(oi[1]), "r"(oi[2]),
                       "r"(oi[3]), "r"(oi[4]), "r"(oi[5])
                       : "memory");
          if constexpr (W == 16)
            asm volatile("st.global.v8.b32 [%0], {%1,%2,%3,%4,%5,%6,%7,%8};" ::"l"(rowp + 32), "r"(oi[6]), "r"(oi[7]), "r"(oi[8]), "r"(oi[9]),
                         "r"(oi[10]), "r"(oi[11]), "r"(oi[12]), "r"(oi[13])
                         : "memory");
        } else {
          *reinterpret_cast<int4*>(rowp) = make_int4(li2, li1, oi[0], oi[1]);
          *reinterpret_cast<int4*>(rowp + 16) = make_int4(oi[2], oi[3], oi[4], oi[5]);
          if constexpr (W == 16) {
            *reinterpret_cast<int4*>(rowp + 32) = make_int4(oi[6], oi[7], oi[8], oi[9]);
            *reinterpret_cast<int4*>(rowp + 48) = make_int4(oi[10], oi[11], oi[12], oi[13]);
          }
        }
      }
    }
    pa = oi[W - 2];
    pb = oi[W - 1];
    rr++;
    rowp += rowStep;
    __syncwarp();
  };

  const int nSteps = G.nSteps;
#pragma unroll 1
  for (int s = 0; s < nSteps; s += 3) {
    step(a0, a1, a2, s);
    step(a1, a2, a0, s + 1);
    step(a2, a0, a1, s + 2);
  }
  if (__any_sync(0xffffffffu, badBits != 0u)) {
    if (lane == 0) A.defer[atomicAdd(A.deferCount, 1)] = tIdx;
  }
  gchunk += uint32_t(nChunks);
  }
}

size_t head_smem_bytes(const LsopFastGeom& g) {
  const size_t nInit = size_t(4 * g.R + 2 * g.C - 9);
  return size_t(kWarps) * (((sizeof(CanonWarpShared) + 15) & ~size_t(15)) + ((nInit * 4 + 15) & ~size_t(15))) + 16;
}
uint32_t text_stage_words(const LsopFastGeom& g) {
  uint32_t w = uint32_t((uint64_t(g.R) * uint64_t(g.C) * 5 / 8 + 3) / 4) + 128u;
  if (w < 512u) w = 512u;
  return (w + 255u) & ~255u;
}
size_t text_smem_bytes(const LsopFastGeom& g) { return text_fast_bytes(text_stage_words(g)) + size_t(g.tileBytes); }
bool text_small(const LsopFastGeom& g) { return uint32_t(g.R) * uint32_t(g.C) <= kTextSmallTile; }
size_t wave_smem_bytes(const LsopFastGeom& g) {
  const size_t rbFloats = size_t((g.C + 4 + 3) & ~3);
  return size_t(kWaveWarps) * (2 * kWaveChunkBytes) + size_t(kWaveWarps) * (2 * rbFloats) * sizeof(float) + size_t(kWaveWarps) * 16;
}

template <int W>
cudaError_t launch_wave(const LsopFastArgs& A, int nCtas, int nTilesUpper, int* tileCounter, cudaStream_t s) {
  const size_t smem = wave_smem_bytes(A.g);
  cudaError_t e;
  if (A.g.wide) {
    if ((e = cudaFuncSetAttribute(lsop3_wave_kernel<W, true>, cudaFuncAttributeMaxDynamicSharedMemorySize, int(smem))) != cudaSuccess) return e;
    lsop3_wave_kernel<W, true><<<nCtas, 32 * kWaveWarps, smem, s>>>(A, tileCounter, 0, nTilesUpper);
  } else {
    if ((e = cudaFuncSetAttribute(lsop3_wave_kernel<W, false>, cudaFuncAttributeMaxDynamicSharedMemorySize, int(smem))) != cudaSuccess) return e;
    lsop3_wave_kernel<W, false><<<nCtas, 32 * kWaveWarps, smem, s>>>(A, tileCounter, 0, nTilesUpper);
  }
  return cudaGetLastError();
}

}

bool lsop_fast_geometry(const g4_band_desc& band, const void* grid, LsopFastGeom* out) {
  LsopFastGeom g{};
  g.R = band.tile_rows;
  g.C = band.tile_cols;
  if (g.R < 6 || g.C < 16 || (g.C & 3) != 0 || (band.grid_pitch & 3) != 0 || (reinterpret_cast<uintptr_t>(grid) & 15) != 0) return false;
  if (g.C <= 128) g.W = 4;
  else if (g.C <= 256 && (g.C & 7) == 0) g.W = 8;
  else if (g.C <= 512 && (g.C & 15) == 0) g.W = 16;
  else return false;
  g.logW = g.W == 4 ? 2 : g.W == 8 ? 3 : 4;
  g.nStrips = (g.C - 2 + g.W - 1) / g.W;
  g.P = g.nStrips * g.W;
  g.nSteps = g.R - 2 + g.nStrips - 1;
  g.chunkRows = 128 / g.W;
  g.nChunks = (g.nSteps + g.chunkRows - 1) / g.chunkRows;
  g.tileBytes = g.nChunks * g.chunkRows * g.P;
  g.tilePitch = g.tileBytes;
  g.wide = ((band.grid_pitch & 7) == 0 && (reinterpret_cast<uintptr_t>(grid) & 31) == 0) ? 1 : 0;
  if (text_smem_bytes(g) > 224u * 1024u || head_smem_bytes(g) > 224u * 1024u || wave_smem_bytes(g) > 224u * 1024u) return false;
  *out = g;
  return true;
}
size_t lsop_fast_side_bytes(const LsopFastGeom& g, int nTiles) { return size_t(nTiles) * size_t(g.R) * sizeof(int4); }
size_t lsop_fast_exc_bytes(int nTiles) { return size_t(nTiles) * kExcWords * sizeof(uint32_t); }
size_t lsop_fast_stage_bytes(int smCount) { return size_t(smCount) * 4 * kFastMaxSub * kSpillWords * sizeof(uint32_t); }
size_t lsop_fast_resid_bytes(const LsopFastGeom& g, int nTiles) { return size_t(kResidGuard) + size_t(nTiles) * size_t(g.tilePitch) + 4096; }

cudaError_t launch_lsop_decode_fast(const LsopFastArgs& A, int nTilesUpper, int smCount, int* textCounter, cudaStream_t s, int* launches) {
  const LsopFastGeom& g = A.g;
  {
    cudaError_t e = cudaFuncSetAttribute(lsop2_head_kernel, cudaFuncAttributeMaxDynamicSharedMemorySize, int(head_smem_bytes(g)));
    if (e == cudaSuccess)
      e = text_small(g) ? cudaFuncSetAttribute(lsop2_text_kernel<kTextThreadsSmall>, cudaFuncAttributeMaxDynamicSharedMemorySize, int(text_smem_bytes(g)))
                        : cudaFuncSetAttribute(lsop2_text_kernel<kTextThreads>, cudaFuncAttributeMaxDynamicSharedMemorySize, int(text_smem_bytes(g)));
    if (e != cudaSuccess) return e;
  }
  const uint32_t stageWords = text_stage_words(g);
  const int nCtasWarp = (nTilesUpper + kWarps - 1) / kWarps;
  lsop2_head_kernel<<<nCtasWarp, kThreads, head_smem_bytes(g), s>>>(A, stageWords * 4u, 0, nTilesUpper);
  cudaError_t e = cudaGetLastError();
  if (e != cudaSuccess) return e;
  LsopFastArgs T = A;
  T.a.counter = textCounter;
  const size_t textSmem = text_smem_bytes(g);
  int perSm = int((227u * 1024u) / (textSmem + 1024));
  const int perSmCap = text_small(g) ? 4 : 2;
  if (perSm < 1) perSm = 1;
  if (perSm > perSmCap) perSm = perSmCap;
  int ctas = smCount * perSm;
  if (ctas > nTilesUpper) ctas = nTilesUpper;
  if (text_small(g)) lsop2_text_kernel<kTextThreadsSmall><<<ctas, kTextThreadsSmall, textSmem, s>>>(T, stageWords, 0, nTilesUpper);
  else lsop2_text_kernel<kTextThreads><<<ctas, kTextThreads, textSmem, s>>>(T, stageWords, 0, nTilesUpper);
  if ((e = cudaGetLastError()) != cudaSuccess) return e;
  int nCtasWave = (nTilesUpper + kWaveWarps - 1) / kWaveWarps;
  if (nCtasWave > smCount * G4_WAVE_CTAS) nCtasWave = smCount * G4_WAVE_CTAS;
  int* waveCounter = textCounter + 1;
  e = g.W == 4 ? launch_wave<4>(A, nCtasWave, nTilesUpper, waveCounter, s) : g.W == 8 ? launch_wave<8>(A, nCtasWave, nTilesUpper, waveCounter, s)
                                                                                          : launch_wave<16>(A, nCtasWave, nTilesUpper, waveCounter, s);
  if (e != cudaSuccess) return e;
  if (launches) *launches += 3;
  return cudaSuccess;
}

}
```

Baseline: 877.8.

## Overlap LSOP head, text and wave kernels with PDL and per-tile ready flags

Launches the LSOP fast-path text and wave kernels with programmatic dependent launch so they can start while the previous kernel is still running. Per-tile epoch-stamped ready flags, written with release stores and polled with acquire loads, let each tile proceed as soon as its producer finishes instead of waiting for a whole-kernel boundary. The raw and legacy wavefront decoders also become grid-stride loops with a capped CTA count. This trades kernel-boundary idle time for spin-polling overhead, more complex memory-ordering code, and the risk of deadlock or timeout if consumer CTAs occupy SMs that producers still need.

```diff
diff --git a/gridfour_b200/csrc/g4_api.cu b/gridfour_b200/csrc/g4_api.cu
--- a/gridfour_b200/csrc/g4_api.cu
+++ b/gridfour_b200/csrc/g4_api.cu
@@ -83,6 +83,8 @@
   DevBuf defer;
   DevBuf lsopMeta;
   DevBuf lsopSide, lsopExc, lsopResid, lsopStage, lsopCks;
+  DevBuf lsopReady;
+  uint32_t lsopEpoch = 0;
   DevBuf wide;
   DevBuf jobLen, jobOff, jobOut, jobTotal, streamIn, streamOut, deflateWork;
   DevBuf stSorted, stRank, stTable, stWork, stCounters;
@@ -341,6 +343,12 @@
         fast.resid = ctx->lsopResid.as<uint8_t>();
         if (lsop_fast_stage_bytes(ctx->smCount)) CK(ctx->lsopStage.ensure(lsop_fast_stage_bytes(ctx->smCount)));
         fast.textStage = ctx->lsopStage.as<uint8_t>();
+        const size_t oldReady = ctx->lsopReady.cap;
+        CK(ctx->lsopReady.ensure(lsop_fast_ready_bytes(nTiles)));
+        if (ctx->lsopReady.cap != oldReady) CK(cudaMemsetAsync(ctx->lsopReady.p, 0, ctx->lsopReady.cap, ctx->stream));
+        if (++ctx->lsopEpoch == 0) ctx->lsopEpoch = 1;
+        fast.ready = ctx->lsopReady.as<uint32_t>();
+        fast.epoch = ctx->lsopEpoch;
       }
       CK(launch_lsop_decode(a, ctx->coef.as<float>(), ctx->lsopMeta.as<uint8_t>(), ctx->defer.as<int>(), ctx->counters.as<int>() + 56,
                             nCtas, nTiles, ctx->stream, &nLaunch, useFast ? &fast : nullptr, ctx->smCount));
@@ -513,7 +521,7 @@
     a.rawShorts = rawShorts ? 1 : 0;
     if (kind == G4_CODEC_COUNT) {
       KernelTimer timer(ctx, 0, kind);
-      CK(launch_raw_decode(a, nTiles, ctx->stream));
+      CK(launch_raw_decode(a, nTiles, ctx->smCount * 8, ctx->stream));
       ctx->launches++;
     } else {
       int rc = launch_decoder(ctx, kind, a, nCtas);
@@ -671,7 +679,7 @@
   if (ctx->evOrder) cudaEventDestroy(ctx->evOrder);
   for (auto& b : ctx->slots) b.release();
   DevBuf* bufs[] = {&ctx->candLens, &ctx->candPreds, &ctx->candStatus, &ctx->counters, &ctx->scratch, &ctx->lists, &ctx->src,
-                    &ctx->total, &ctx->coef, &ctx->defer, &ctx->lsopMeta, &ctx->lsopSide, &ctx->lsopExc, &ctx->lsopResid, &ctx->lsopStage, &ctx->tileRefs, &ctx->lsopCks, &ctx->wide, &ctx->encScratch, &ctx->region, &ctx->jobLen, &ctx->jobOff, &ctx->jobOut, &ctx->jobTotal,
+                    &ctx->total, &ctx->coef, &ctx->defer, &ctx->lsopMeta, &ctx->lsopSide, &ctx->lsopExc, &ctx->lsopResid, &ctx->lsopStage, &ctx->tileRefs, &ctx->lsopCks, &ctx->lsopReady, &ctx->wide, &ctx->encScratch, &ctx->region, &ctx->jobLen, &ctx->jobOff, &ctx->jobOut, &ctx->jobTotal,
                     &ctx->streamIn, &ctx->streamOut, &ctx->deflateWork, &ctx->stSorted, &ctx->stRank, &ctx->stTable,
                     &ctx->stWork, &ctx->stCounters, &ctx->rcPos, &ctx->rcOff, &ctx->rcLen, &ctx->rcCrc, &ctx->rcStored, &ctx->rcTotal,
                     &ctx->rcData, &ctx->rcOffsets, &ctx->rcLens, &ctx->rcIndex, &ctx->rcStatus, &ctx->rcOut, &ctx->rcChain, &ctx->rcDesc, &ctx->sGrid, &ctx->sArena, &ctx->sOffsets, &ctx->sLens, &ctx->sCodec, &ctx->sPred, &ctx->sStatus};
diff --git a/gridfour_b200/csrc/g4_batch.cu b/gridfour_b200/csrc/g4_batch.cu
--- a/gridfour_b200/csrc/g4_batch.cu
+++ b/gridfour_b200/csrc/g4_batch.cu
@@ -143,24 +143,25 @@
 }
 
 __global__ void __launch_bounds__(kThreads) raw_decode_kernel(DecodeArgs a) {
-  const int li = blockIdx.x;
-  if (li >= *a.listCount) return;
-  const int t = a.list[li];
-  const TileView tv = tile_view(a.band, a.grid, t);
-  const uint8_t* src = a.arena + a.offsets[t];
-  const int n = tv.R * tv.C;
-  if (a.rawShorts) {
+  const int nList = *a.listCount;
+  for (int li = blockIdx.x; li < nList; li += gridDim.x) {
+    const int t = a.list[li];
+    const TileView tv = tile_view(a.band, a.grid, t);
+    const uint8_t* src = a.arena + a.offsets[t];
+    const int n = tv.R * tv.C;
+    if (a.rawShorts) {
+      for (int i = threadIdx.x; i < n; i += kThreads) {
+        int r = i / tv.C, c = i - r * tv.C;
+        tv.at(r, c) = int32_t(int16_t(uint16_t(src[2 * size_t(i)]) | (uint16_t(src[2 * size_t(i) + 1]) << 8)));
+      }
+      continue;
+    }
+    const bool aligned = (reinterpret_cast<uintptr_t>(src) & 3) == 0;
     for (int i = threadIdx.x; i < n; i += kThreads) {
       int r = i / tv.C, c = i - r * tv.C;
-      tv.at(r, c) = int32_t(int16_t(uint16_t(src[2 * size_t(i)]) | (uint16_t(src[2 * size_t(i) + 1]) << 8)));
-    }
-    return;
-  }
-  const bool aligned = (reinterpret_cast<uintptr_t>(src) & 3) == 0;
-  for (int i = threadIdx.x; i < n; i += kThreads) {
-    int r = i / tv.C, c = i - r * tv.C;
-    uint32_t v = aligned ? reinterpret_cast<const uint32_t*>(src)[i] : load_le32(src + 4 * size_t(i));
-    tv.at(r, c) = int32_t(v);
+      uint32_t v = aligned ? reinterpret_cast<const uint32_t*>(src)[i] : load_le32(src + 4 * size_t(i));
+      tv.at(r, c) = int32_t(v);
+    }
   }
 }
 
@@ -210,9 +211,9 @@
   classify_kernel<<<(a.nTiles + 255) / 256, 256, 0, s>>>(a);
   return cudaGetLastError();
 }
-cudaError_t launch_raw_decode(const DecodeArgs& a, int nTiles, cudaStream_t s) {
-  raw_decode_kernel<<<nTiles, kThreads, 0, s>>>(a);
-  return cudaGetLastError();
-}
-
-}
+cudaError_t launch_raw_decode(const DecodeArgs& a, int nTiles, int maxCtas, cudaStream_t s) {
+  raw_decode_kernel<<<nTiles < maxCtas ? nTiles : maxCtas, kThreads, 0, s>>>(a);
+  return cudaGetLastError();
+}
+
+}
diff --git a/gridfour_b200/csrc/g4_kernels.h b/gridfour_b200/csrc/g4_kernels.h
--- a/gridfour_b200/csrc/g4_kernels.h
+++ b/gridfour_b200/csrc/g4_kernels.h
@@ -133,7 +133,7 @@
 cudaError_t launch_offsets(const uint32_t* lens, uint64_t* offsets, int nTiles, uint64_t* total, cudaStream_t s);
 cudaError_t launch_compact(const CompactArgs& a, int nTiles, cudaStream_t s);
 cudaError_t launch_classify(const ClassifyArgs& a, cudaStream_t s);
-cudaError_t launch_raw_decode(const DecodeArgs& a, int nTiles, cudaStream_t s);
+cudaError_t launch_raw_decode(const DecodeArgs& a, int nTiles, int maxCtas, cudaStream_t s);
 cudaError_t launch_widen_i16(const int16_t* src, int64_t srcPitch, int32_t* dst, int64_t rows, int64_t cols, int32_t fill, cudaStream_t s);
 cudaError_t launch_narrow_i16(const int32_t* src, int16_t* dst, int64_t dstPitch, int64_t rows, int64_t cols, cudaStream_t s);
 
@@ -182,6 +182,8 @@
   uint8_t* textStage;
   int* defer;
   int* deferCount;
+  uint32_t* ready;
+  uint32_t epoch;
   LsopFastGeom g;
 };
 bool lsop_fast_geometry(const g4_band_desc& band, const void* grid, LsopFastGeom* out);
@@ -189,6 +191,7 @@
 size_t lsop_fast_exc_bytes(int nTiles);
 size_t lsop_fast_stage_bytes(int smCount);
 size_t lsop_fast_resid_bytes(const LsopFastGeom& g, int nTiles);
+size_t lsop_fast_ready_bytes(int nTiles);
 cudaError_t launch_lsop_decode_fast(const LsopFastArgs& A, int nTilesUpper, int smCount, int* textCounter, cudaStream_t s, int* launches);
 cudaError_t launch_lsop_decode(const DecodeArgs& a, float* coef, uint8_t* meta, int* defer, int* deferCounters, int nCtas,
                                int nTilesUpper, cudaStream_t s, int* launches, const LsopFastArgs* fast = nullptr, int smCount = 148);
diff --git a/gridfour_b200/csrc/g4_lsop.cu b/gridfour_b200/csrc/g4_lsop.cu
--- a/gridfour_b200/csrc/g4_lsop.cu
+++ b/gridfour_b200/csrc/g4_lsop.cu
@@ -519,10 +519,10 @@
 
 __global__ void __launch_bounds__(kThreads) lsop_wavefront_kernel(DecodeArgs a, const float* coef) {
   const int lane = threadIdx.x & 31, warp = threadIdx.x >> 5;
-  const int li = blockIdx.x * kWarps + warp;
-  if (li >= *a.listCount) return;
+  const int nList = *a.listCount;
+  for (int li = blockIdx.x * kWarps + warp; li < nList; li += gridDim.x * kWarps) {
   const int tIdx = a.list[li];
-  if (a.status[tIdx] != G4_OK) return;
+  if (a.status[tIdx] != G4_OK) continue;
   const TileView t = tile_view(a.band, a.grid, tIdx);
   const int R = t.R, C = t.C;
   float u[12];
@@ -592,6 +592,7 @@
     }
     __syncwarp();
     __threadfence_block();
+  }
   }
 }
 
@@ -1082,7 +1083,9 @@
     d.counter = deferCounters + 1;
     lsop_decode_entropy_kernel<<<nCtas < 296 ? nCtas : 296, kThreads, 0, s>>>(d, coef);
     if ((e = cudaGetLastError()) != cudaSuccess) return e;
-    lsop_wavefront_kernel<<<(nTilesUpper + kWarps - 1) / kWarps, kThreads, 0, s>>>(d, coef);
+    int nCtasWave = (nTilesUpper + kWarps - 1) / kWarps;
+    if (nCtasWave > smCount * 8) nCtasWave = smCount * 8;
+    lsop_wavefront_kernel<<<nCtasWave, kThreads, 0, s>>>(d, coef);
     if (launches) *launches = nLaunch + 2;
     return cudaGetLastError();
   }
diff --git a/gridfour_b200/csrc/g4_lsop_fast.cu b/gridfour_b200/csrc/g4_lsop_fast.cu
--- a/gridfour_b200/csrc/g4_lsop_fast.cu
+++ b/gridfour_b200/csrc/g4_lsop_fast.cu
@@ -43,6 +43,29 @@
                  : "memory");
 }
 
+constexpr uint32_t kReadySleepNs = 1000;
+constexpr uint32_t kReadyPolls = 4000000;
+
+__device__ __forceinline__ void pdl_launch_dependents() { asm volatile("griddepcontrol.launch_dependents;" ::: "memory"); }
+__device__ __forceinline__ void pdl_wait_producers() { asm volatile("griddepcontrol.wait;" ::: "memory"); }
+__device__ __forceinline__ void ready_publish(uint32_t* w, uint32_t epoch) {
+  asm volatile("st.release.gpu.global.u32 [%0], %1;" ::"l"(w), "r"(epoch) : "memory");
+}
+__device__ __forceinline__ uint32_t ready_load(const uint32_t* w) {
+  uint32_t v;
+  asm volatile("ld.acquire.gpu.global.u32 %0, [%1];" : "=r"(v) : "l"(w) : "memory");
+  return v;
+}
+__device__ __forceinline__ bool ready_poll(const uint32_t* w, uint32_t epoch) {
+#pragma unroll 1
+  for (uint32_t i = 0; i < kReadyPolls; i++) {
+    __nanosleep(kReadySleepNs);
+    if (ready_load(w) == epoch) return true;
+  }
+  return false;
+}
+__device__ __forceinline__ bool ready_wait(const uint32_t* w, uint32_t epoch) { return ready_load(w) == epoch || ready_poll(w, epoch); }
+
 __device__ __forceinline__ uint32_t image_offset(uint32_t w, int logW, uint32_t P, uint32_t k) {
   const uint32_t rr = k / w, pp = k - rr * w;
   return (rr + (pp >> logW)) * P + pp;
@@ -61,7 +84,7 @@
   return carry;
 }
 
-__global__ void __launch_bounds__(kThreads, 3) lsop2_head_kernel(LsopFastArgs A, uint32_t maxPackBytes, int listBegin, int listEnd) {
+__device__ __forceinline__ void lsop2_head_tile(const LsopFastArgs& A, uint32_t maxPackBytes, int tIdx) {
   extern __shared__ __align__(16) unsigned char headSmem[];
   const DecodeArgs& a = A.a;
   const int lane = threadIdx.x & 31, warp = threadIdx.x >> 5;
@@ -70,9 +93,6 @@
   const size_t perWarp = ((sizeof(CanonWarpShared) + 15) & ~size_t(15)) + ((size_t(nInit) * 4 + 15) & ~size_t(15));
   CanonWarpShared& W = *reinterpret_cast<CanonWarpShared*>(headSmem + perWarp * warp);
   int32_t* init = reinterpret_cast<int32_t*>(headSmem + perWarp * warp + ((sizeof(CanonWarpShared) + 15) & ~size_t(15)));
-  const int li = listBegin + blockIdx.x * kWarps + warp;
-  if (li >= listEnd || li >= *a.listCount) return;
-  const int tIdx = a.list[li];
   uint8_t* m = A.meta + size_t(tIdx) * kLsopMetaBytes;
   if (lane == 0) {
     *reinterpret_cast<uint32_t*>(m) = 0;
@@ -156,6 +176,17 @@
     }
   }
   if (lane == 0) a.status[tIdx] = status;
+}
+
+__global__ void __launch_bounds__(kThreads, 3) lsop2_head_kernel(LsopFastArgs A, uint32_t maxPackBytes, int listBegin, int listEnd) {
+  pdl_launch_dependents();
+  const int li = listBegin + blockIdx.x * kWarps + int(threadIdx.x >> 5);
+  if (li >= listEnd || li >= *A.a.listCount) return;
+  const int tIdx = A.a.list[li];
+  lsop2_head_tile(A, maxPackBytes, tIdx);
+  __syncwarp();
+  __threadfence();
+  if ((threadIdx.x & 31) == 0) ready_publish(A.ready + 2 * size_t(tIdx), A.epoch);
 }
 
 struct ByteTileSink {
@@ -618,20 +649,44 @@
   return __syncthreads_or(bad ? 1 : 0) ? 1 : 0;
 }
 
+__device__ __forceinline__ int text_acquire(const LsopFastArgs& A, int li, int listEnd, bool block) {
+  if (li >= listEnd || li >= *A.a.listCount) return 1;
+  const int tIdx = A.a.list[li];
+  const uint32_t* w = A.ready + 2 * size_t(tIdx);
+  if (ready_load(w) == A.epoch) return 1;
+  if (!block) return 2;
+  if (ready_poll(w, A.epoch)) return 1;
+  A.a.status[tIdx] = G4_ERR_CUDA;
+  ready_publish(A.ready + 2 * size_t(tIdx) + 1, A.epoch);
+  return 0;
+}
+__device__ __forceinline__ void text_publish_image(const LsopFastArgs& A, int pend) {
+  asm volatile("cp.async.bulk.wait_group 0;" ::: "memory");
+  if (pend >= 0) {
+    asm volatile("fence.proxy.async.global;" ::: "memory");
+    ready_publish(A.ready + 2 * size_t(pend) + 1, A.epoch);
+  }
+}
+
 template <int NT>
 __global__ void __launch_bounds__(NT, NT == 512 ? 2 : 4) lsop2_text_kernel(LsopFastArgs A, uint32_t stageWords, int listBegin, int listEnd) {
   extern __shared__ __align__(128) unsigned char textSmem[];
   CanonFastShared& F = *reinterpret_cast<CanonFastShared*>(textSmem);
   uint8_t* tileImg = textSmem + text_fast_bytes(stageWords);
   __shared__ int sTile[2];
+  __shared__ int sHeld[2];
+  __shared__ int sPend;
   __shared__ __align__(8) uint64_t sBar;
   const DecodeArgs& a = A.a;
   const int tid = threadIdx.x;
   const uint32_t bar = smem_u32(&sBar);
+  pdl_launch_dependents();
   if (tid == 0) {
     mbar_init(bar, 1);
     asm volatile("fence.mbarrier_init.release.cluster;");
     sTile[0] = listBegin + atomicAdd(a.counter, 1);
+    sHeld[0] = text_acquire(A, sTile[0], listEnd, true);
+    sPend = -1;
   }
   __syncthreads();
   uint32_t parity = 0;
@@ -641,8 +696,15 @@
     if (tid == 0) sTile[phase ^ 1] = listBegin + atomicAdd(a.counter, 1);
     const int tIdx = a.list[li];
     const uint8_t* m = A.meta + size_t(tIdx) * kLsopMetaBytes;
-    const uint32_t T0 = *reinterpret_cast<const uint32_t*>(m);
-    if (T0 == 0) { __syncthreads(); continue; }
+    const uint32_t T0 = sHeld[phase] ? *reinterpret_cast<const uint32_t*>(m) : 0u;
+    if (T0 == 0) {
+      if (tid == 0) {
+        ready_publish(A.ready + 2 * size_t(tIdx) + 1, A.epoch);
+        sHeld[phase ^ 1] = text_acquire(A, sTile[phase ^ 1], listEnd, true);
+      }
+      __syncthreads();
+      continue;
+    }
     const uint8_t* packing = a.arena + a.offsets[tIdx];
     const uint32_t len = a.lens[tIdx];
     const uint32_t delta = uint32_t(reinterpret_cast<uintptr_t>(packing) & 15u);
@@ -676,7 +738,11 @@
       const uint32_t nInterior = uint32_t(A.g.R - 2) * uint32_t(A.g.C - 4);
       ByteTileSink sink;
       sink.init(tileImg, A.exc + size_t(tIdx) * kExcWords, A.g);
-      if (tid == 0) asm volatile("cp.async.bulk.wait_group.read 0;" ::: "memory");
+      if (tid == 0) {
+        text_publish_image(A, sPend);
+        sPend = -1;
+        sHeld[phase ^ 1] = text_acquire(A, sTile[phase ^ 1], listEnd, false);
+      }
       rc = lsop_text_decode<NT>(F, span * 8u, T0 + 8u * delta, nInterior, uint32_t(A.g.tileBytes), sink,
                                 reinterpret_cast<uint32_t*>(A.textStage) + size_t(blockIdx.x) * (kFastMaxSub * kSpillWords));
       if (rc == 2) {
@@ -686,23 +752,28 @@
       }
       ok = rc == 0;
     }
+    if (tid == 0 && sHeld[phase ^ 1] == 2) sHeld[phase ^ 1] = text_acquire(A, sTile[phase ^ 1], listEnd, true);
     __syncthreads();
     if (tid == 0) {
-      if (rc == 1) a.status[tIdx] = G4_ERR_FORMAT;
-      else if (A.exc[size_t(tIdx) * kExcWords] > uint32_t(kExcCap)) {
+      if (rc == 1) {
+        a.status[tIdx] = G4_ERR_FORMAT;
+        ready_publish(A.ready + 2 * size_t(tIdx) + 1, A.epoch);
+      } else if (A.exc[size_t(tIdx) * kExcWords] > uint32_t(kExcCap)) {
         A.exc[size_t(tIdx) * kExcWords] = uint32_t(kExcCap) + 1u;
         A.defer[atomicAdd(A.deferCount, 1)] = tIdx;
-      }
-      else {
+        ready_publish(A.ready + 2 * size_t(tIdx) + 1, A.epoch);
+      } else {
         asm volatile("fence.proxy.async.shared::cta;" ::: "memory");
         uint8_t* dst = A.resid + kResidGuard + size_t(tIdx) * size_t(A.g.tilePitch);
         asm volatile("cp.async.bulk.global.shared::cta.bulk_group [%0], [%1], %2;" ::"l"(dst), "r"(smem_u32(tileImg)), "r"(uint32_t(A.g.tileBytes))
                      : "memory");
         asm volatile("cp.async.bulk.commit_group;" ::: "memory");
-      }
-    }
-  }
-  if (tid == 0) asm volatile("cp.async.bulk.wait_group 0;" ::: "memory");
+        sPend = tIdx;
+      }
+    }
+  }
+  if (tid == 0) text_publish_image(A, sPend);
+  pdl_wait_producers();
 }
 
 #ifndef G4_WAVE_CTAS
@@ -751,6 +822,11 @@
   li = __shfl_sync(0xffffffffu, li, 0);
   if (li >= listEnd || li >= *a.listCount) break;
   const int tIdx = a.list[li];
+  if (lane == 0) {
+    if (ready_wait(A.ready + 2 * size_t(tIdx) + 1, A.epoch)) asm volatile("fence.proxy.async.global;" ::: "memory");
+    else a.status[tIdx] = G4_ERR_CUDA;
+  }
+  __syncwarp();
   if (a.status[tIdx] != G4_OK) continue;
   if (*reinterpret_cast<const uint32_t*>(A.meta + size_t(tIdx) * kLsopMetaBytes) == 0u) continue;
   const uint32_t* exc = A.exc + size_t(tIdx) * kExcWords;
@@ -940,6 +1016,7 @@
   }
   gchunk += uint32_t(nChunks);
   }
+  pdl_wait_producers();
 }
 
 size_t head_smem_bytes(const LsopFastGeom& g) {
@@ -956,6 +1033,21 @@
 size_t wave_smem_bytes(const LsopFastGeom& g) {
   const size_t rbFloats = size_t((g.C + 4 + 3) & ~3);
   return size_t(kWaveWarps) * (2 * kWaveChunkBytes) + size_t(kWaveWarps) * (2 * rbFloats) * sizeof(float) + size_t(kWaveWarps) * 16;
+}
+
+template <typename... Params, typename... Args>
+cudaError_t launch_overlapped(void (*kernel)(Params...), int nCtas, int nThreads, size_t smem, cudaStream_t s, Args... args) {
+  cudaLaunchConfig_t cfg{};
+  cfg.gridDim = dim3(unsigned(nCtas));
+  cfg.blockDim = dim3(unsigned(nThreads));
+  cfg.dynamicSmemBytes = smem;
+  cfg.stream = s;
+  cudaLaunchAttribute attr[1];
+  attr[0].id = cudaLaunchAttributeProgrammaticStreamSerialization;
+  attr[0].val.programmaticStreamSerializationAllowed = 1;
+  cfg.attrs = attr;
+  cfg.numAttrs = 1;
+  return cudaLaunchKernelEx(&cfg, kernel, Params(args)...);
 }
 
 template <int W>
@@ -964,12 +1056,11 @@
   cudaError_t e;
   if (A.g.wide) {
     if ((e = cudaFuncSetAttribute(lsop3_wave_kernel<W, true>, cudaFuncAttributeMaxDynamicSharedMemorySize, int(smem))) != cudaSuccess) return e;
-    lsop3_wave_kernel<W, true><<<nCtas, 32 * kWaveWarps, smem, s>>>(A, tileCounter, 0, nTilesUpper);
+    return launch_overlapped(lsop3_wave_kernel<W, true>, nCtas, 32 * kWaveWarps, smem, s, A, tileCounter, 0, nTilesUpper);
   } else {
     if ((e = cudaFuncSetAttribute(lsop3_wave_kernel<W, false>, cudaFuncAttributeMaxDynamicSharedMemorySize, int(smem))) != cudaSuccess) return e;
-    lsop3_wave_kernel<W, false><<<nCtas, 32 * kWaveWarps, smem, s>>>(A, tileCounter, 0, nTilesUpper);
-  }
-  return cudaGetLastError();
+    return launch_overlapped(lsop3_wave_kernel<W, false>, nCtas, 32 * kWaveWarps, smem, s, A, tileCounter, 0, nTilesUpper);
+  }
 }
 
 }
@@ -1000,6 +1091,7 @@
 size_t lsop_fast_exc_bytes(int nTiles) { return size_t(nTiles) * kExcWords * sizeof(uint32_t); }
 size_t lsop_fast_stage_bytes(int smCount) { return size_t(smCount) * 4 * kFastMaxSub * kSpillWords * sizeof(uint32_t); }
 size_t lsop_fast_resid_bytes(const LsopFastGeom& g, int nTiles) { return size_t(kResidGuard) + size_t(nTiles) * size_t(g.tilePitch) + 4096; }
+size_t lsop_fast_ready_bytes(int nTiles) { return size_t(nTiles) * 2 * sizeof(uint32_t); }
 
 cudaError_t launch_lsop_decode_fast(const LsopFastArgs& A, int nTilesUpper, int smCount, int* textCounter, cudaStream_t s, int* launches) {
   const LsopFastGeom& g = A.g;
@@ -1024,9 +1116,9 @@
   if (perSm > perSmCap) perSm = perSmCap;
   int ctas = smCount * perSm;
   if (ctas > nTilesUpper) ctas = nTilesUpper;
-  if (text_small(g)) lsop2_text_kernel<kTextThreadsSmall><<<ctas, kTextThreadsSmall, textSmem, s>>>(T, stageWords, 0, nTilesUpper);
-  else lsop2_text_kernel<kTextThreads><<<ctas, kTextThreads, textSmem, s>>>(T, stageWords, 0, nTilesUpper);
-  if ((e = cudaGetLastError()) != cudaSuccess) return e;
+  e = text_small(g) ? launch_overlapped(lsop2_text_kernel<kTextThreadsSmall>, ctas, kTextThreadsSmall, textSmem, s, T, stageWords, 0, nTilesUpper)
+                    : launch_overlapped(lsop2_text_kernel<kTextThreads>, ctas, kTextThreads, textSmem, s, T, stageWords, 0, nTilesUpper);
+  if (e != cudaSuccess) return e;
   int nCtasWave = (nTilesUpper + kWaveWarps - 1) / kWaveWarps;
   if (nCtasWave > smCount * G4_WAVE_CTAS) nCtasWave = smCount * G4_WAVE_CTAS;
   int* waveCounter = textCounter + 1;
diff --git a/probes/trace_decode_step.py b/probes/trace_decode_step.py
--- /dev/null
+++ b/probes/trace_decode_step.py
@@ -0,0 +1,125 @@
+import argparse
+import json
+import os
+import subprocess
+import sys
+import tempfile
+
+import numpy as np
+
+ROOT = os.path.dirname(os.path.dirname(os.path.abspath(__file__)))
+sys.path.insert(0, ROOT)
+sys.dont_write_bytecode = True
+
+
+def gpu_info(index):
+    q = subprocess.run(["nvidia-smi", "-i", str(index), "--query-gpu=name,power.limit,clocks.max.sm", "--format=csv,noheader"],
+                       capture_output=True, text=True, timeout=30)
+    name, power, clock = [x.strip() for x in q.stdout.strip().split(",")]
+    return {"name": name, "power_limit": power, "max_sm_clock": clock}
+
+
+def short(name):
+    n = name.split("(")[0]
+    for p in ("void ", "g4::", "(anonymous namespace)::"):
+        n = n.replace(p, "")
+    return n
+
+
+def main():
+    ap = argparse.ArgumentParser()
+    ap.add_argument("--steps", type=int, default=6)
+    ap.add_argument("--warmup", type=int, default=3)
+    ap.add_argument("--out", default=None, help="also write the JSON result to this file")
+    args = ap.parse_args()
+    if args.steps < 3:
+        raise SystemExit("--steps must be at least 3")
+
+    import torch
+    from torch.profiler import ProfilerActivity, profile
+
+    import gridfour_b200 as g4
+
+    dev = torch.device("cuda", 0)
+    torch.cuda.set_device(dev)
+    info = gpu_info(0)
+    stream = torch.cuda.Stream(dev)
+    torch.cuda.set_stream(stream)
+    ctx = g4.Context(0, stream.cuda_stream)
+    spec = g4.CodecSpecification(default=False)
+    spec.addCompressionCodec("GvrsHuffman", g4.CodecHuffman)
+    spec.addCompressionCodec("GvrsDeflate", g4.CodecDeflate)
+    spec.addCompressionCodec("LSOP12", g4.LsEncoder12, g4.LsDecoder12)
+    master = g4.CodecMaster(spec, ctx)
+    tr, tc, rows, cols = 180, 240, 5400, 86400
+    grid = torch.empty((rows, cols), dtype=torch.int32, device=dev)
+    ctx.fill_terrain(grid.data_ptr(), 0, 0, 0, rows, cols)
+    batch = master.encodeTiles(grid, tr, tc)
+    out = torch.zeros_like(grid)
+    for _ in range(args.warmup):
+        master.decodeTiles(batch, out=out)
+    torch.cuda.synchronize(dev)
+    assert torch.equal(out, grid)
+
+    with profile(activities=[ProfilerActivity.CUDA]) as prof:
+        ctx.set_async(True)
+        for _ in range(args.steps):
+            master.decodeTiles(batch, out=out)
+        ctx.synchronize()
+        torch.cuda.synchronize(dev)
+        ctx.set_async(False)
+    assert int((master.lastStatus != 0).sum()) == 0 and torch.equal(out, grid)
+    with tempfile.TemporaryDirectory() as tmp:
+        path = os.path.join(tmp, "trace.json")
+        prof.export_chrome_trace(path)
+        with open(path) as f:
+            trace = json.load(f)
+    acts = sorted((e for e in trace["traceEvents"] if e.get("ph") == "X" and e.get("cat") in ("kernel", "gpu_memset", "gpu_memcpy")),
+                  key=lambda e: e["ts"])
+    starts = [i for i, e in enumerate(acts) if short(e["name"]) == "classify_kernel"]
+    assert len(starts) == args.steps, "expected one classify_kernel per step, found %d" % len(starts)
+    steps = []
+    for s, i0 in enumerate(starts[1:], 1):
+        i1 = starts[s + 1] if s + 1 < len(starts) else len(acts)
+        t0 = acts[i0]["ts"]
+        rows_, prev_end = [], None
+        for e in acts[i0:i1]:
+            b, d = e["ts"] - t0, e["dur"]
+            rows_.append({"name": short(e["name"]), "start_us": round(b, 2), "end_us": round(b + d, 2), "dur_us": round(d, 2),
+                          "gap_us": None if prev_end is None else round(b - prev_end, 2)})
+            prev_end = b + d if prev_end is None else max(prev_end, b + d)
+        step_us = (acts[i1]["ts"] - t0) if i1 < len(acts) else None
+        steps.append({"step_us": step_us, "activities": rows_})
+    n_act = len(steps[0]["activities"])
+    assert all(len(s["activities"]) == n_act for s in steps), "steps differ in their activities"
+    mean = []
+    for k in range(n_act):
+        col = [s["activities"][k] for s in steps]
+        m = {"name": col[0]["name"]}
+        for f in ("start_us", "end_us", "dur_us", "gap_us"):
+            v = [c[f] for c in col if c[f] is not None]
+            m[f] = round(float(np.mean(v)), 2) if v else None
+        mean.append(m)
+    full = [s["step_us"] for s in steps if s["step_us"] is not None]
+    last_end = float(np.mean([s["activities"][-1]["end_us"] for s in steps]))
+    result = {
+        "what": "device timeline of the config-3 decode step (10,800 tiles of 180x240 int32; GvrsHuffman+GvrsDeflate+LSOP12), "
+                "pipelined steps, torch.profiler CUDA activities; times relative to the start of classify_kernel",
+        "gpu": info, "steps_traced": args.steps, "steps_reported": len(steps),
+        "step_us_mean": round(float(np.mean(full)), 2) if full else None, "last_activity_end_us_mean": round(last_end, 2),
+        "mean": mean, "last_step": steps[-1]["activities"],
+    }
+    print("%-48s %10s %10s %10s %10s" % ("activity (mean over steps)", "start us", "end us", "dur us", "gap us"))
+    for m in mean:
+        print("%-48s %10.2f %10.2f %10.2f %10s" % (m["name"][:48], m["start_us"], m["end_us"], m["dur_us"],
+                                                   "" if m["gap_us"] is None else "%.2f" % m["gap_us"]))
+    print("step (classify to classify): %s us; last activity ends at %.2f us" % (result["step_us_mean"], last_end))
+    print(json.dumps(result))
+    if args.out:
+        os.makedirs(os.path.dirname(os.path.abspath(args.out)), exist_ok=True)
+        with open(args.out, "w") as f:
+            f.write(json.dumps(result, indent=1) + "\n")
+
+
+if __name__ == "__main__":
+    main()
```

Result: faster. 895.6 (median of 6 runs) (+2.0%).
